# pascalPost/turbomesh

Hardware: AMD Instinct MI355X
Metric: nodes smoothed/sec (elliptic sweeps, 4096^2 blocks) + achieved HBM GB/s (higher is better)
Workload: dtype f64

## Files before the change

include/tm_hip.h:

```cpp
#ifndef TM_HIP_H
#define TM_HIP_H

#include <stdint.h>

#ifdef __cplusplus
extern "C" {
#endif

#define TM_HIP_ABI_VERSION 1

typedef enum tm_error {
    TM_OK = 0,
    TM_W_NOT_CONVERGED = 1,
    TM_E_SIZE = -1,
    TM_E_TOPOLOGY = -2,
    TM_E_MISMATCH = -3,
    TM_E_OVERFLOW = -4,
    TM_E_UNSUPPORTED = -5,
    TM_E_ARG = -6,
    TM_E_MEMORY = -7,
    TM_E_HIP = -8,
    TM_E_COMM = -9
} tm_error;

// ... 49 lines not shown
} tm_control_fn;

enum { TM_SOLVER_GMRES = 0, TM_SOLVER_BICGSTAB = 1, TM_SOLVER_UMFPACK = 2, TM_SOLVER_PETSC = 3, TM_SOLVER_HIP = 4 };
enum {
    TM_INNER_BICGSTAB = 0,
    TM_INNER_RELAX = 1,
    TM_INNER_MG_BICGSTAB = 2,
    TM_INNER_GMRES = 4,
    TM_INNER_REFERENCE_GMRES = 5,
    TM_INNER_AUTO = 3
};
enum {
    TM_OPT_SINGLE_SWEEP = 1,
    TM_OPT_EAGER_SCALARS = 2,
    TM_OPT_PRECOND_ILU0 = 8,
    TM_OPT_REFINE = 16,
    TM_OPT_RTOL_INITIAL = 4
};
typedef struct tm_solver_opt {
    int32_t tag;
    int32_t inner;
    double rtol;
    double atol;
    uint64_t max_inner;
    uint32_t check_every;
    uint32_t flags;
    double omega;
} tm_solver_opt;

typedef struct tm_stats {
    uint64_t outer_iterations;
    uint64_t inner_iterations;
    uint64_t operator_sweeps;
    double last_residual;
    double last_dx2, last_dy2;
    double scaled_residual_rms;
    double seconds;
    int32_t not_converged;
    int32_t _pad;
} tm_stats;

int tm_tfi_block(double* xy_out, uint64_t ni, uint64_t nj,
                 const double* x_i_min, const double* x_i_max,
                 const double* x_j_min, const double* x_j_max,
                 const double* s1, const double* s2, const double* t1, const double* t2);

int tm_tfi_linear2d(double* xy_out, uint64_t ni, uint64_t nj,
                    const double* e_i_min, const double* e_i_max, const double* e_j_min, const double* e_j_max);

int tm_smooth_mesh(const tm_mesh_desc* mesh, uint64_t iterations, const tm_solver_opt* opt,
                   const tm_control_fn* cf, tm_stats* stats );

int tm_csr_solve(uint64_t n, const int32_t* Ap, const int32_t* Ai, const double* Ax_x, const double* Ax_y ,
                 const double* bx, const double* by, double* x , double* y, const tm_solver_opt* opt ,
                 tm_stats* stats );

int tm_csr_residual(uint64_t n, const int32_t* Ap, const int32_t* Ai, const double* Ax_x, const double* Ax_y ,
                    const double* bx, const double* by, const double* x, const double* y, double* rx, double* ry);

typedef struct tm_smoother tm_smoother;

typedef struct tm_comm_hooks {
    void* ctx;
    int32_t rank, nranks;
    const int32_t* owner;
    int (*exchange)(void* ctx, const double* send_buf, double* recv_buf, void* stream);
    int (*allreduce_sum)(void* ctx, double* buf, int32_t n, void* stream);
    int (*exchange_wait)(void* ctx, void* stream);
    void* workspace;
    uint64_t workspace_bytes;
} tm_comm_hooks;
int tm_smoother_workspace_bytes(const tm_mesh_desc* mesh, const tm_solver_opt* opt, const tm_control_fn* cf,
                                const tm_comm_hooks* hooks, uint64_t* bytes);

int tm_smoother_create(const tm_mesh_desc* mesh, const tm_solver_opt* opt, const tm_control_fn* cf,
                       const tm_comm_hooks* hooks , void* stream ,
                       tm_smoother** out);
int tm_smoother_iterate(tm_smoother* s, uint64_t iterations, tm_stats* stats);
int tm_smoother_iterate_until(tm_smoother* s, uint64_t max_iterations, double scaled_residual_tol, tm_stats* stats);
int tm_smoother_iterate_until_update(tm_smoother* s, uint64_t max_iterations, double update_rms_tol, tm_stats* stats);
int tm_smoother_download(tm_smoother* s, const tm_mesh_desc* mesh);
int tm_smoother_upload(tm_smoother* s, const tm_mesh_desc* mesh);
void tm_smoother_destroy(tm_smoother* s);

typedef struct tm_rccl_comm tm_rccl_comm;
#define TM_RCCL_ID_BYTES 128
int tm_rccl_unique_id(const char* librccl_path, void* id_out );
int tm_rccl_comm_create(const char* librccl_path, const void* id, int32_t rank, int32_t nranks, tm_rccl_comm** out);
void tm_rccl_comm_destroy(tm_rccl_comm* comm);
int tm_rccl_hooks(tm_rccl_comm* comm, const tm_mesh_desc* mesh, const int32_t* owner , tm_comm_hooks* hooks);
int tm_rccl_hooks_for(tm_rccl_comm* comm, const tm_mesh_desc* mesh, const int32_t* owner, const tm_solver_opt* opt, const tm_control_fn* cf ,
                      tm_comm_hooks* hooks);

typedef struct tm_rccl_peer_table {
    int32_t npeers, direct_send;
    int64_t send_rows, recv_rows;
    int32_t* peer;
    int64_t *send_off, *send_cnt, *recv_off, *recv_cnt;
} tm_rccl_peer_table;
int tm_rccl_peer_table_build(const tm_mesh_desc* mesh, const int32_t* owner, int32_t rank, int32_t nranks, tm_rccl_peer_table* out);
void tm_rccl_peer_table_free(tm_rccl_peer_table* table);

int tm_smoother_exchange_plan(const tm_smoother* s, int32_t* npeers, const int32_t** peer_rank,
                              const int64_t** send_offset, const int64_t** send_count,
                              const int64_t** recv_offset, const int64_t** recv_count);

int tm_smoother_apply(tm_smoother* s, const double* in_xy, double* out_xy, int scaled);
int tm_smoother_assemble_csr(tm_smoother* s, int32_t* Ap, int32_t* Ai, double* Ax_x, double* Ax_y, uint64_t nnz_capacity, uint64_t* nnz);
int tm_smoother_apply_reference_order(tm_smoother* s, const double* in_xy, double* out_xy);
int tm_smoother_rhs(tm_smoother* s, double* rhs_xy);
int tm_smoother_residual(tm_smoother* s, const double* xy , double* r_xy);
int tm_smoother_refine_report(const tm_smoother* s, uint32_t* steps_x_y ,
                              double* last_update_rel ,
                              uint64_t* correction_iterations );
int tm_smoother_row_kinds(const tm_smoother* s, int32_t* kinds );
uint64_t tm_smoother_dof(const tm_smoother* s);
int tm_smoother_inner(const tm_smoother* s);
int tm_smoother_inner_counts(const tm_smoother* s, uint64_t* x_iterations, uint64_t* y_iterations);
int tm_smoother_control_function(tm_smoother* s, double* pq);

int tm_export_soa(const double* xy , uint64_t ni, uint64_t nj, double* x_out , double* y_out );
int tm_smoother_export_soa(tm_smoother* s, uint64_t block, double* x, double* y, double* p, double* q);

typedef struct tm_quality {
    uint64_t cells, inverted, degenerate;
    int32_t  orientation, _pad;
    double   min_scaled_jacobian;
    uint64_t worst_block, worst_i, worst_j;
    double   min_angle_deg, max_angle_deg;
    double   max_aspect, max_growth_i, max_growth_j;
    double   min_area, max_area, total_area;
    uint64_t hist[10];
} tm_quality;

int tm_mesh_quality(const tm_mesh_desc* mesh, tm_quality* per_block , tm_quality* total );
int tm_mesh_quality_host(const tm_mesh_desc* mesh, tm_quality* per_block, tm_quality* total);
int tm_smoother_quality(tm_smoother* s, tm_quality* per_block, tm_quality* total);
int tm_smoother_quality_field(tm_smoother* s, uint64_t block, double* min_scaled_jacobian );

typedef struct tm_plan_rows {
    uint64_t nrows;
    int64_t* row;
    int32_t* kind;
    int32_t* ncols;
    int64_t* cols;
    double* coef_x;
    double* coef_y;
    double* rhs;
    int32_t* slot;
} tm_plan_rows;
int tm_plan_build(const tm_mesh_desc* mesh, tm_plan_rows* out);
void tm_plan_free(tm_plan_rows* rows);

typedef struct tm_plan_local_info {
    int64_t n_owned, n_ghost, n_send;
    int32_t npeers, nowned_blocks;
    int64_t* owned_blocks;
    int64_t* local_start;
    int64_t* ghost_gid;
    int32_t* send_ids;
    int64_t* send_gid;
    int32_t* peer_rank;
    int64_t* send_offset;
    int64_t* send_count;
    int64_t* recv_offset;
    int64_t* recv_count;
    int64_t* send_first;
    int32_t direct_send;
    int32_t _pad;
    int64_t n_ghost_rows;
    int64_t* ghost_row_gid;
    int32_t* ghost_row_kind;
    int64_t* ghost_row_cols;
} tm_plan_local_info;
int tm_plan_local(const tm_mesh_desc* mesh, const int32_t* owner, int32_t rank, int32_t nranks, tm_plan_local_info* out);
void tm_plan_local_free(tm_plan_local_info* info);

int tm_dev_tfi_block(double* d_xy, uint64_t ni, uint64_t nj,
                     const double* d_x_i_min, const double* d_x_i_max, const double* d_x_j_min, const double* d_x_j_max,
                     const double* d_s1, const double* d_s2, const double* d_t1, const double* d_t2, void* stream);
int tm_dev_relax_sweep(const double* d_in, double* d_out, uint64_t ni, uint64_t nj, double omega,
                       double* d_partials, uint64_t partials_capacity, uint64_t* nwg, void* stream);
uint64_t tm_dev_relax_partials_needed(uint64_t ni, uint64_t nj);

#ifdef __cplusplus
}
#endif
#endif
```

turbomesh_amd/_capi.py:

```python
from __future__ import annotations

import ctypes as C
import os

import numpy as np

_HERE = os.path.dirname(os.path.abspath(__file__))
LIB_PATH = os.environ.get("TM_HIP_LIB") or os.path.join(_HERE, "libtm_hip.so")
DBG_LIB_PATH = os.path.join(_HERE, "libtm_hip_dbg.so")

TM_OK, TM_W_NOT_CONVERGED = 0, 1
TM_E_SIZE, TM_E_TOPOLOGY, TM_E_MISMATCH, TM_E_OVERFLOW, TM_E_UNSUPPORTED, TM_E_ARG, TM_E_MEMORY, TM_E_HIP, TM_E_COMM = -1, -2, -3, -4, -5, -6, -7, -8, -9
_ERR_NAMES = {-1: "InconsistentSize", -2: "Topology", -3: "Mismatch", -4: "Overflow", -5: "ExternalSolverNotEnabled", -6: "Argument",
              -7: "OutOfMemory", -8: "Hip", -9: "Comm"}
TM_SOLVER_GMRES, TM_SOLVER_BICGSTAB, TM_SOLVER_UMFPACK, TM_SOLVER_PETSC, TM_SOLVER_HIP = 0, 1, 2, 3, 4
TM_INNER_BICGSTAB, TM_INNER_RELAX, TM_INNER_MG_BICGSTAB, TM_INNER_AUTO, TM_INNER_GMRES, TM_INNER_REFERENCE_GMRES = 0, 1, 2, 3, 4, 5
TM_CF_LAPLACE, TM_CF_WHITE = 0, 1
TM_OPT_REFINE = 16


class TmError(RuntimeError):

    def __init__(self, code, msg):
        super().__init__(f"error.{_ERR_NAMES.get(code, 'Unknown')} ({code}): {msg}")
        self.code = code
        self.name = _ERR_NAMES.get(code, "Unknown")


class tm_range(C.Structure):
    _fields_ = [("block", C.c_uint64), ("side", C.c_uint32), ("_pad", C.c_uint32), ("start", C.c_uint64), ("end", C.c_uint64)]


class tm_connection(C.Structure):
    _fields_ = [("r", tm_range * 2), ("has_periodicity", C.c_int32), ("_pad", C.c_int32), ("periodicity", C.c_double * 2)]


class tm_condition(C.Structure):
    _fields_ = [("range", tm_range), ("kind", C.c_uint32), ("_pad", C.c_uint32)]


class tm_block(C.Structure):
    _fields_ = [("xy", C.POINTER(C.c_double)), ("ni", C.c_uint64), ("nj", C.c_uint64)]


class tm_mesh_desc(C.Structure):
    _fields_ = [("blocks", C.POINTER(tm_block)), ("nblocks", C.c_uint64), ("conns", C.POINTER(tm_connection)), ("nconns", C.c_uint64),
                ("bcs", C.POINTER(tm_condition)), ("nbcs", C.c_uint64)]


class tm_control_fn(C.Structure):
    _fields_ = [("kind", C.c_int32), ("_pad", C.c_int32), ("ds_target", C.c_double), ("theta_target", C.c_double)]


class tm_solver_opt(C.Structure):
    _fields_ = [("tag", C.c_int32), ("inner", C.c_int32), ("rtol", C.c_double), ("atol", C.c_double), ("max_inner", C.c_uint64),
                ("check_every", C.c_uint32), ("flags", C.c_uint32), ("omega", C.c_double)]


class tm_stats(C.Structure):
    _fields_ = [("outer_iterations", C.c_uint64), ("inner_iterations", C.c_uint64), ("operator_sweeps", C.c_uint64),
                ("last_residual", C.c_double), ("last_dx2", C.c_double), ("last_dy2", C.c_double), ("scaled_residual_rms", C.c_double),
                ("seconds", C.c_double), ("not_converged", C.c_int32), ("_pad", C.c_int32)]

    def as_dict(self):
        return {k: getattr(self, k) for k, _ in self._fields_ if not k.startswith("_")}


EXCHANGE_FN = C.CFUNCTYPE(C.c_int, C.c_void_p, C.c_void_p, C.c_void_p, C.c_void_p)
ALLREDUCE_FN = C.CFUNCTYPE(C.c_int, C.c_void_p, C.c_void_p, C.c_int32, C.c_void_p)
EXCHANGE_WAIT_FN = C.CFUNCTYPE(C.c_int, C.c_void_p, C.c_void_p)


LOG_FN = C.CFUNCTYPE(None, C.c_void_p, C.c_int32, C.c_uint64, C.c_double)


class tm_comm_hooks(C.Structure):
    _fields_ = [("ctx", C.c_void_p), ("rank", C.c_int32), ("nranks", C.c_int32), ("owner", C.POINTER(C.c_int32)),
                ("exchange", EXCHANGE_FN), ("allreduce_sum", ALLREDUCE_FN), ("exchange_wait", EXCHANGE_WAIT_FN), ("workspace", C.c_void_p),
                ("workspace_bytes", C.c_uint64)]


class tm_plan_rows(C.Structure):
    _fields_ = [("nrows", C.c_uint64), ("row", C.POINTER(C.c_int64)), ("kind", C.POINTER(C.c_int32)), ("ncols", C.POINTER(C.c_int32)),
                ("cols", C.POINTER(C.c_int64)), ("coef_x", C.POINTER(C.c_double)), ("coef_y", C.POINTER(C.c_double)),
                ("rhs", C.POINTER(C.c_double)), ("slot", C.POINTER(C.c_int32))]


class tm_plan_local_info(C.Structure):
    _fields_ = [("n_owned", C.c_int64), ("n_ghost", C.c_int64), ("n_send", C.c_int64), ("npeers", C.c_int32), ("nowned_blocks", C.c_int32),
                ("owned_blocks", C.POINTER(C.c_int64)), ("local_start", C.POINTER(C.c_int64)), ("ghost_gid", C.POINTER(C.c_int64)),
                ("send_ids", C.POINTER(C.c_int32)), ("send_gid", C.POINTER(C.c_int64)), ("peer_rank", C.POINTER(C.c_int32)),
                ("send_offset", C.POINTER(C.c_int64)), ("send_count", C.POINTER(C.c_int64)), ("recv_offset", C.POINTER(C.c_int64)),
                ("recv_count", C.POINTER(C.c_int64)), ("send_first", C.POINTER(C.c_int64)), ("direct_send", C.c_int32), ("_pad", C.c_int32),
                ("n_ghost_rows", C.c_int64), ("ghost_row_gid", C.POINTER(C.c_int64)), ("ghost_row_kind", C.POINTER(C.c_int32)),
                ("ghost_row_cols", C.POINTER(C.c_int64))]


class tm_rccl_peer_table(C.Structure):
    _fields_ = [("npeers", C.c_int32), ("direct_send", C.c_int32), ("send_rows", C.c_int64), ("recv_rows", C.c_int64),
                ("peer", C.POINTER(C.c_int32)), ("send_off", C.POINTER(C.c_int64)), ("send_cnt", C.POINTER(C.c_int64)),
                ("recv_off", C.POINTER(C.c_int64)), ("recv_cnt", C.POINTER(C.c_int64))]


_i32p = C.POINTER(C.c_int32)


class tm_edge_tables_info(C.Structure):
    _fields_ = ([("nrows", C.c_int64), ("nruns", C.c_int64), ("nwg", C.c_int64)] +
                [(k, _i32p) for k in ("first", "count", "row0", "row_stride", "col0", "col_stride", "met0", "met_stride", "kind", "ncols", "self", "flags",
                                     "wg_run", "wg_k0")] +
                [("gid", C.POINTER(C.c_int64)), ("nstrips", C.c_int64), ("ntasks", C.c_int64), ("strip_off", _i32p), ("task", _i32p)])


class tm_quality(C.Structure):
    _fields_ = [("cells", C.c_uint64), ("inverted", C.c_uint64), ("degenerate", C.c_uint64), ("orientation", C.c_int32), ("_pad", C.c_int32),
                ("min_scaled_jacobian", C.c_double), ("worst_block", C.c_uint64), ("worst_i", C.c_uint64), ("worst_j", C.c_uint64),
                ("min_angle_deg", C.c_double), ("max_angle_deg", C.c_double), ("max_aspect", C.c_double), ("max_growth_i", C.c_double),
                ("max_growth_j", C.c_double), ("min_area", C.c_double), ("max_area", C.c_double), ("total_area", C.c_double),
                ("hist", C.c_uint64 * 10)]


EXPORTS = [
    "tm_last_error", "tm_abi_version", "tm_set_log", "tm_csr_solve", "tm_tfi_block", "tm_tfi_linear2d", "tm_smooth_mesh", "tm_smoother_create",
    "tm_smoother_workspace_bytes", "tm_smoother_iterate", "tm_smoother_iterate_until", "tm_smoother_iterate_until_update", "tm_smoother_download", "tm_smoother_upload", "tm_smoother_destroy",
    "tm_smoother_exchange_plan", "tm_smoother_apply", "tm_smoother_rhs", "tm_smoother_row_kinds", "tm_smoother_dof",
    "tm_smoother_control_function", "tm_smoother_profile", "tm_smoother_profile_read", "tm_plan_build", "tm_plan_free", "tm_plan_local", "tm_plan_local_free", "tm_dev_tfi_block", "tm_dev_relax_sweep",
    "tm_dev_relax_partials_needed", "tm_export_soa", "tm_smoother_export_soa", "tm_rccl_unique_id", "tm_rccl_comm_create", "tm_rccl_comm_destroy", "tm_rccl_hooks",
    "tm_rccl_peer_table_build", "tm_rccl_peer_table_free", "tm_white_math_probe", "tm_stream_probe", "tm_smoother_queue_ordering", "tm_smoother_inner", "tm_csr_ilu0_probe", "tm_rccl_hooks_for", "tm_smoother_assemble_csr", "tm_smoother_apply_reference_order",
    "tm_smoother_inner_counts", "tm_mesh_quality", "tm_mesh_quality_host", "tm_smoother_quality", "tm_smoother_quality_field",
    "tm_csr_residual", "tm_smoother_residual", "tm_smoother_refine_report",
    "tm_mg_transfer_probe", "tm_smoother_mg_levels", "tm_smoother_precondition_probe", "tm_edge_tables_probe", "tm_edge_tables_free",
]

_lib = None
_dp = C.POINTER(C.c_double)


def _share_hip_runtime():
    import importlib.util
    import sys

    if "torch" in sys.modules:
        return
    try:
        spec = importlib.util.find_spec("torch")
    except (ImportError, ValueError):
        spec = None
    if spec is None or not spec.origin:
        return
    rt = os.path.join(os.path.dirname(spec.origin), "lib", "libamdhip64.so")
    if os.path.exists(rt):
        try:
            C.CDLL(rt, mode=C.RTLD_GLOBAL)
        except OSError:
            pass


def lib():
    global _lib
    if _lib is None:
        if not os.path.exists(LIB_PATH):
            raise OSError(f"{LIB_PATH} is missing: build it with `python -c 'import __graft_entry__ as g; g.build()'` "
                          "or `make -C turbomesh_amd/csrc`; turbomesh_amd has no CPU fallback")
        _share_hip_runtime()
        L = C.CDLL(LIB_PATH)
        L.tm_last_error.restype = C.c_char_p
        L.tm_csr_solve.argtypes = [C.c_uint64, C.POINTER(C.c_int32), C.POINTER(C.c_int32), _dp, _dp, _dp, _dp, _dp, _dp, C.POINTER(tm_solver_opt),
                                   C.POINTER(tm_stats)]
        L.tm_csr_residual.argtypes = [C.c_uint64, C.POINTER(C.c_int32), C.POINTER(C.c_int32)] + [_dp] * 8
        L.tm_set_log.argtypes = [LOG_FN, C.c_void_p]
        L.tm_set_log.restype = None
        L.tm_smoother_dof.restype = C.c_uint64
        L.tm_smoother_dof.argtypes = [C.c_void_p]
        L.tm_dev_relax_partials_needed.restype = C.c_uint64
        L.tm_dev_relax_partials_needed.argtypes = [C.c_uint64, C.c_uint64]
        L.tm_tfi_block.argtypes = [_dp, C.c_uint64, C.c_uint64] + [_dp] * 8
        L.tm_tfi_linear2d.argtypes = [_dp, C.c_uint64, C.c_uint64] + [_dp] * 4
        L.tm_smooth_mesh.argtypes = [C.POINTER(tm_mesh_desc), C.c_uint64, C.POINTER(tm_solver_opt), C.POINTER(tm_control_fn), C.POINTER(tm_stats)]
        L.tm_smoother_create.argtypes = [C.POINTER(tm_mesh_desc), C.POINTER(tm_solver_opt), C.POINTER(tm_control_fn), C.POINTER(tm_comm_hooks),
                                         C.c_void_p, C.POINTER(C.c_void_p)]
        L.tm_smoother_workspace_bytes.argtypes = [C.POINTER(tm_mesh_desc), C.POINTER(tm_solver_opt), C.POINTER(tm_control_fn),
                                                  C.POINTER(tm_comm_hooks), C.POINTER(C.c_uint64)]
        L.tm_smoother_iterate.argtypes = [C.c_void_p, C.c_uint64, C.POINTER(tm_stats)]
        L.tm_smoother_iterate_until.argtypes = [C.c_void_p, C.c_uint64, C.c_double, C.POINTER(tm_stats)]
        L.tm_smoother_iterate_until_update.argtypes = [C.c_void_p, C.c_uint64, C.c_double, C.POINTER(tm_stats)]
        L.tm_smoother_download.argtypes = [C.c_void_p, C.POINTER(tm_mesh_desc)]
        L.tm_smoother_upload.argtypes = [C.c_void_p, C.POINTER(tm_mesh_desc)]
        L.tm_smoother_destroy.argtypes = [C.c_void_p]
        L.tm_smoother_destroy.restype = None
        L.tm_smoother_exchange_plan.argtypes = [C.c_void_p, C.POINTER(C.c_int32), C.POINTER(C.POINTER(C.c_int32))] + [C.POINTER(C.POINTER(C.c_int64))] * 4
        L.tm_smoother_apply.argtypes = [C.c_void_p, _dp, _dp, C.c_int]
        L.tm_smoother_rhs.argtypes = [C.c_void_p, _dp]
        L.tm_smoother_residual.argtypes = [C.c_void_p, _dp, _dp]
        L.tm_smoother_refine_report.argtypes = [C.c_void_p, C.POINTER(C.c_uint32), _dp, C.POINTER(C.c_uint64)]
        L.tm_smoother_assemble_csr.argtypes = [C.c_void_p, C.POINTER(C.c_int32), C.POINTER(C.c_int32), _dp, _dp, C.c_uint64, C.POINTER(C.c_uint64)]
        L.tm_smoother_apply_reference_order.argtypes = [C.c_void_p, _dp, _dp]
        L.tm_smoother_row_kinds.argtypes = [C.c_void_p, C.POINTER(C.c_int32)]
        L.tm_smoother_control_function.argtypes = [C.c_void_p, _dp]
        L.tm_smoother_profile.argtypes = [C.c_void_p, C.c_int]
        L.tm_smoother_profile_read.argtypes = [C.c_void_p, _dp, C.POINTER(C.c_uint64), C.POINTER(C.c_uint64)]
        L.tm_smoother_queue_ordering.argtypes = [C.c_void_p]
        L.tm_smoother_inner.argtypes = [C.c_void_p]
        L.tm_smoother_inner_counts.argtypes = [C.c_void_p, C.POINTER(C.c_uint64), C.POINTER(C.c_uint64)]
        L.tm_csr_ilu0_probe.argtypes = [C.c_uint64, C.POINTER(C.c_int32), C.POINTER(C.c_int32), _dp, _dp, _dp, _dp]
        L.tm_plan_build.argtypes = [C.POINTER(tm_mesh_desc), C.POINTER(tm_plan_rows)]
        L.tm_plan_free.argtypes = [C.POINTER(tm_plan_rows)]
        L.tm_plan_free.restype = None
        L.tm_export_soa.argtypes = [_dp, C.c_uint64, C.c_uint64, _dp, _dp]
        L.tm_smoother_export_soa.argtypes = [C.c_void_p, C.c_uint64, _dp, _dp, _dp, _dp]
        L.tm_mesh_quality.argtypes = [C.POINTER(tm_mesh_desc), C.POINTER(tm_quality), C.POINTER(tm_quality)]
        L.tm_mesh_quality_host.argtypes = [C.POINTER(tm_mesh_desc), C.POINTER(tm_quality), C.POINTER(tm_quality)]
        L.tm_smoother_quality.argtypes = [C.c_void_p, C.POINTER(tm_quality), C.POINTER(tm_quality)]
        L.tm_smoother_quality_field.argtypes = [C.c_void_p, C.c_uint64, _dp]
        L.tm_rccl_unique_id.argtypes = [C.c_char_p, C.c_void_p]
        L.tm_rccl_comm_create.argtypes = [C.c_char_p, C.c_void_p, C.c_int32, C.c_int32, C.POINTER(C.c_void_p)]
        L.tm_rccl_comm_destroy.argtypes = [C.c_void_p]
        L.tm_rccl_comm_destroy.restype = None
        L.tm_rccl_hooks.argtypes = [C.c_void_p, C.POINTER(tm_mesh_desc), C.POINTER(C.c_int32), C.POINTER(tm_comm_hooks)]
        L.tm_rccl_hooks_for.argtypes = [C.c_void_p, C.POINTER(tm_mesh_desc), C.POINTER(C.c_int32), C.POINTER(tm_solver_opt), C.POINTER(tm_control_fn), C.POINTER(tm_comm_hooks)]
        L.tm_plan_local.argtypes = [C.POINTER(tm_mesh_desc), C.POINTER(C.c_int32), C.c_int32, C.c_int32, C.POINTER(tm_plan_local_info)]
        L.tm_plan_local_free.argtypes = [C.POINTER(tm_plan_local_info)]
        L.tm_plan_local_free.restype = None
        L.tm_dev_tfi_block.argtypes = [C.c_void_p, C.c_uint64, C.c_uint64] + [C.c_void_p] * 8 + [C.c_void_p]
        L.tm_dev_relax_sweep.argtypes = [C.c_void_p, C.c_void_p, C.c_uint64, C.c_uint64, C.c_double, C.c_void_p, C.c_uint64,
                                         C.POINTER(C.c_uint64), C.c_void_p]
        L.tm_rccl_peer_table_build.argtypes = [C.POINTER(tm_mesh_desc), C.POINTER(C.c_int32), C.c_int32, C.c_int32, C.POINTER(tm_rccl_peer_table)]
        L.tm_rccl_peer_table_free.argtypes = [C.POINTER(tm_rccl_peer_table)]
        L.tm_rccl_peer_table_free.restype = None
        L.tm_white_math_probe.argtypes = [_dp, _dp, C.c_uint64, _dp, _dp]
        L.tm_stream_probe.argtypes = [C.c_uint64, C.c_int32, _dp, _dp]
        L.tm_mg_transfer_probe.argtypes = [C.c_int32, C.c_uint64, C.c_uint64, C.c_int32, C.c_int32, _dp, _dp, C.c_double, C.c_double, _dp]
        L.tm_smoother_mg_levels.argtypes = [C.c_void_p, C.c_uint64, C.POINTER(C.c_int32), C.POINTER(C.c_int32), C.c_uint32, C.POINTER(C.c_int32), _dp]
        L.tm_smoother_precondition_probe.argtypes = [C.c_void_p, _dp, _dp, _dp]
        L.tm_edge_tables_probe.argtypes = [C.POINTER(tm_mesh_desc), C.POINTER(C.c_int32), C.c_int32, C.c_int32, C.c_int32, C.c_int32, C.POINTER(tm_edge_tables_info)]
        L.tm_edge_tables_free.argtypes = [C.POINTER(tm_edge_tables_info)]
        L.tm_edge_tables_free.restype = None
        if hasattr(L, "tm_tune_apply"):
            L.tm_debug_null_hooks.argtypes = [C.c_int32, C.c_int32, C.POINTER(C.c_int32), C.POINTER(tm_comm_hooks)]
            L.tm_diag_apply.argtypes = [C.c_void_p, C.c_void_p, C.c_uint64, C.c_uint64, C.c_int, C.c_void_p]
            L.tm_tune_fuse.argtypes = [C.c_int]
            L.tm_tune_apply.argtypes = [C.c_int, C.c_int, C.c_int, C.c_int]
        _lib = L
    return _lib


def check(rc):
    if rc < 0:
        raise TmError(rc, lib().tm_last_error().decode())
    return rc


def f64ptr(a):
    return a.ctypes.data_as(_dp)


class MeshDesc:

    def __init__(self, mesh, with_coordinates=True):
        blocks = mesh.blocks
        self._blocks = (tm_block * max(1, len(blocks)))()
        for k, b in enumerate(blocks):
            data = b.points.data
            if with_coordinates and data is not None:
                if data.dtype != np.float64 or not data.flags["C_CONTIGUOUS"]:
                    raise TmError(TM_E_ARG, "block coordinates must be C-contiguous float64")
                self._blocks[k] = tm_block(f64ptr(data), b.points.size[0], b.points.size[1])
            else:
                self._blocks[k] = tm_block(None, b.points.size[0], b.points.size[1])
        conns = mesh.connections
        self._conns = (tm_connection * max(1, len(conns)))()
        for k, c in enumerate(conns):
            tc = tm_connection()
            for s in range(2):
                r = c.ranges[s]
                tc.r[s] = tm_range(r.block, int(r.side), 0, r.start, r.end)
            tc.has_periodicity = 0 if c.periodicity is None else 1
            if c.periodicity is not None:
                tc.periodicity[0], tc.periodicity[1] = float(c.periodicity[0]), float(c.periodicity[1])
            self._conns[k] = tc
        bcs = mesh.boundary_conditions
        self._bcs = (tm_condition * max(1, len(bcs)))()
        for k, bc in enumerate(bcs):
            r = bc.range
            self._bcs[k] = tm_condition(tm_range(r.block, int(r.side), 0, r.start, r.end), int(bc.kind), 0)
        self.desc = tm_mesh_desc(self._blocks, len(blocks), self._conns, len(conns), self._bcs, len(bcs))

    def ref(self):
        return C.byref(self.desc)
```

turbomesh_amd/csrc/tm_api.cpp:

```cpp
#include "tm_smoother.hpp"
#include <cmath>
#include <cstdlib>
#include <cstring>
#include <limits>
#include <memory>

using namespace tmh;

#include "tm_api_util.hpp"
#include "tm_ilu.hpp"
#include "tm_refine.hpp"
#include "tm_quality_dev.hpp"

static void require_gfx950() {
    static int checked = 0;
    if (checked) return;
    int dev = 0;
    HIPCHK(hipGetDevice(&dev));
    hipDeviceProp_t prop;
    HIPCHK(hipGetDeviceProperties(&prop, dev));
    if (std::strncmp(prop.gcnArchName, "gfx950", 6) != 0)
        throw TmError(TM_E_HIP, std::string("libtm_hip is built for gfx950 (MI355X) only, found ") + prop.gcnArchName);
    checked = 1;
}
// ... 671 lines not shown
            gg.push_back(g.gid);
            gk.push_back(g.kind);
            for (int q = 0; q < 9; ++q) gc.push_back(q < g.ncols ? g.col[q] : -1);
        }
        out->n_ghost_rows = static_cast<int64_t>(gg.size());
        out->ghost_row_gid = dup(gg);
        out->ghost_row_kind = dup(gk);
        out->ghost_row_cols = dup(gc);
        return TM_OK;
    });
}
void tm_plan_local_free(tm_plan_local_info* i) {
    if (!i) return;
    std::free(i->owned_blocks);
    std::free(i->local_start);
    std::free(i->ghost_gid);
    std::free(i->send_ids);
    std::free(i->send_gid);
    std::free(i->peer_rank);
    std::free(i->send_first);
    std::free(i->send_offset);
    std::free(i->send_count);
    std::free(i->recv_offset);
    std::free(i->recv_count);
    std::free(i->ghost_row_gid);
    std::free(i->ghost_row_kind);
    std::free(i->ghost_row_cols);
    std::memset(i, 0, sizeof(*i));
}

int tm_edge_tables_probe(const tm_mesh_desc* mesh, const int32_t* owner, int32_t rank, int32_t nranks, int32_t table, int32_t level_strip,
                         tm_edge_tables_info* out) {
    return guarded([&]() {
        if (!mesh || !owner || !out) throw TmError(TM_E_ARG, "null argument");
        if (table < 0 || table > 5 || level_strip < 0) throw TmError(TM_E_ARG, "table outside 0..5 or negative strip length");
        std::memset(out, 0, sizeof(*out));
        const Topology t = topo_of(mesh);
        const std::vector<PlanRow> rows = build_rows(t);
        const LocalPlan lp = build_local_plan(t, rows, std::vector<int32_t>(owner, owner + t.nblocks()), rank, nranks);
        const MovingSides moving = moving_sides(t, lp);
        std::vector<PlanRow> zone[3];
        auto selection = [&](int tab) {
            std::vector<const PlanRow*> sel;
            auto add = [&](const std::vector<PlanRow>& more) {
                for (const PlanRow& r : more) sel.push_back(&r);
            };
            if (tab == 0) add(lp.rows);
            else for (size_t k : moving.nf_rows) sel.push_back(&lp.rows[k]);
            if (tab >= 3) add(zone[tab - 3] = zone_rows(t, lp, moving.dyn_mask, tab - 3));
            if (tab == 3) add(lp.ghost_rows2);
            if (tab == 2 || tab == 4) add(lp.ghost_rows);
            return sel;
        };
        RunTable level[3];
        for (int tab = 3; tab < 5 && table == 5; ++tab) level[tab - 3] = build_run_table(t, lp, selection(tab));
        const std::vector<const PlanRow*> sel = selection(table);
        const RunTable T = build_run_table(t, lp, sel);
        std::vector<int32_t> f[12], task;
        for (const EdgeRun& R : T.runs) {
            const int32_t scalars[8] = {R.first, R.count, R.row0, R.row_stride, R.kind, R.ncols, R.self, R.flags};
            for (int q = 0; q < 8; ++q) f[q].push_back(scalars[q]);
            f[8].insert(f[8].end(), R.col0, R.col0 + 9);
            f[9].insert(f[9].end(), R.col_stride, R.col_stride + 9);
            f[10].insert(f[10].end(), R.met0, R.met0 + 4);
            f[11].insert(f[11].end(), R.met_stride, R.met_stride + 4);
        }
        std::vector<int64_t> gid;
        for (int32_t k : T.order) gid.push_back(sel[k]->gid);
        StripPlan plan;
        if (table == 5) {
            const std::vector<EdgeRun>* const runs[3] = {&level[0].runs, &level[1].runs, &T.runs};
            plan = build_strip_plan(runs, T.where, level_strip ? level_strip : 60);
            for (int s = 0; s < plan.nstrips; ++s)
                for (int l = 0; l < 3; ++l)
                    for (int32_t k = plan.off[4 * s + l]; k < plan.off[4 * s + l + 1]; ++k)
                        task.insert(task.end(), {l + 1, plan.tasks[k].run, plan.tasks[k].k0, plan.tasks[k].count});
        }
        out->nrows = static_cast<int64_t>(sel.size());
        out->nruns = static_cast<int64_t>(T.runs.size());
        out->nwg = static_cast<int64_t>(T.wg_run.size());
        int32_t** const dst[12] = {&out->first, &out->count, &out->row0, &out->row_stride, &out->kind, &out->ncols, &out->self, &out->flags,
                                   &out->col0, &out->col_stride, &out->met0, &out->met_stride};
        for (int q = 0; q < 12; ++q) *dst[q] = dup(f[q]);
        out->wg_run = dup(T.wg_run);
        out->wg_k0 = dup(T.wg_k0);
        out->gid = dup(gid);
        out->nstrips = plan.nstrips;
        out->ntasks = static_cast<int64_t>(plan.tasks.size());
        out->strip_off = dup(plan.off);
        out->task = dup(task);
        return TM_OK;
    });
}
void tm_edge_tables_free(tm_edge_tables_info* i) {
    if (!i) return;
    int32_t* const arrays[] = {i->first, i->count, i->row0,   i->row_stride, i->col0,   i->col_stride, i->met0,      i->met_stride,
                               i->kind,  i->ncols, i->self,   i->flags,      i->wg_run, i->wg_k0,      i->strip_off, i->task};
    for (int32_t* p : arrays) std::free(p);
    std::free(i->gid);
    std::memset(i, 0, sizeof(*i));
}

int tm_plan_build(const tm_mesh_desc* mesh, tm_plan_rows* out) {
    return guarded([&]() {
        if (!mesh || !out) throw TmError(TM_E_ARG, "null argument");
        std::memset(out, 0, sizeof(*out));
        const Topology t = topo_of(mesh);
        const std::vector<PlanRow> rows = build_rows(t);
        const size_t n = rows.size();
        out->nrows = n;
        out->row = static_cast<int64_t*>(std::malloc(sizeof(int64_t) * (n ? n : 1)));
        out->kind = static_cast<int32_t*>(std::malloc(sizeof(int32_t) * (n ? n : 1)));
        out->ncols = static_cast<int32_t*>(std::malloc(sizeof(int32_t) * (n ? n : 1)));
        out->cols = static_cast<int64_t*>(std::malloc(sizeof(int64_t) * 9 * (n ? n : 1)));
        out->coef_x = static_cast<double*>(std::malloc(sizeof(double) * 9 * (n ? n : 1)));
        out->coef_y = static_cast<double*>(std::malloc(sizeof(double) * 9 * (n ? n : 1)));
        out->rhs = static_cast<double*>(std::malloc(sizeof(double) * 2 * (n ? n : 1)));
        out->slot = static_cast<int32_t*>(std::malloc(sizeof(int32_t) * 9 * (n ? n : 1)));
        if (!out->row || !out->kind || !out->ncols || !out->cols || !out->coef_x || !out->coef_y || !out->rhs || !out->slot) {
            tm_plan_free(out);
            throw TmError(TM_E_MEMORY, "out of host memory");
        }
        const double nan = std::numeric_limits<double>::quiet_NaN();
        for (size_t k = 0; k < n; ++k) {
            const PlanRow& r = rows[k];
            out->row[k] = r.gid;
            out->kind[k] = r.kind;
            out->ncols[k] = r.ncols;
            for (int q = 0; q < 9; ++q) {
                out->cols[k * 9 + q] = q < r.ncols ? r.col[q] : -1;
                out->coef_x[k * 9 + q] = (r.kind == KIND_SMOOTHED) ? nan : r.cx[q];
                out->coef_y[k * 9 + q] = (r.kind == KIND_SMOOTHED) ? nan : r.cy[q];
                out->slot[k * 9 + q] = r.slot[q];
            }
            out->rhs[2 * k] = (r.rhs_coord & 1) ? nan : r.rhs[0];
            out->rhs[2 * k + 1] = (r.rhs_coord & 2) ? nan : r.rhs[1];
        }
        return TM_OK;
    });
}
void tm_plan_free(tm_plan_rows* rows) {
    if (!rows) return;
    std::free(rows->row);
    std::free(rows->kind);
    std::free(rows->ncols);
    std::free(rows->cols);
    std::free(rows->coef_x);
    std::free(rows->coef_y);
    std::free(rows->rhs);
    std::free(rows->slot);
    std::memset(rows, 0, sizeof(*rows));
}

}
```

turbomesh_amd/csrc/tm_edge_types.h:

```cpp
#pragma once
#include <cstdint>

struct EdgeRun {
    int32_t first, count;
    int32_t row0, row_stride;
    int32_t col0[9], col_stride[9];
    int32_t met0[4], met_stride[4];
    int8_t kind, ncols, self;
    uint8_t flags;
    int8_t slot[9];
    int8_t _pad[3];
    double cx[9], cy[9];
    double per[2];
};
static_assert(sizeof(EdgeRun) == 296, "EdgeRun is read by the kernels through the scalar cache: its layout is fixed");
struct EdgeRowsDev {
    int nrows = 0;
    int nwg = 0;
    const EdgeRun* runs = nullptr;
    const int32_t* wg_run = nullptr;
    const int32_t* wg_k0 = nullptr;
    const double* rhs = nullptr;
};
constexpr int EDGE_BLOCK = 128;
struct LevelTask {
    int32_t run, k0, count;
};
struct FusedLevelsDev {
    int nstrips = 0;
    const LevelTask* tasks = nullptr;
    const int32_t* off = nullptr;
};
constexpr int LEVELS_BLOCK = 512;
```

turbomesh_amd/csrc/tm_kernels.h:

```cpp
#pragma once
#include <hip/hip_runtime.h>
#include <cstdint>
#include "tm_edge_types.h"
#include <vector>

namespace tmh {

enum ApplyMode : int {
    MODE_RAW = 0,
    MODE_SCALED = 1,
    MODE_RESID = 2,
    MODE_RELAX = 3,
    MODE_DIAG_COPY = 4,
    MODE_DIAG_SUM9 = 5,
    MODE_DIAG_NOSTORE = 6,
    MODE_DIAG_NOLOAD = 7,
    MODE_DIAG_MATH = 8,
    MODE_MG_RESID = 9,
    MODE_MG_SMOOTH = 10,
    MODE_MG_FIRST2 = 11
};
enum DotMode : int {
    DOT_NONE = 0,
    DOT_AUX = 1,
    DOT_IN = 2,
    DOT_OUT2 = 3,
    DOT_DELTA = 4,
    DOT_AUX2 = 5,
    DOT_IN_SS = 6,
    DOT_B2 = 7
};
constexpr int MAX_PARTIALS = 8;
struct KrylovScalars;
struct LazyScalars;

struct ApplyBlock {
    const double2* in2 = nullptr;
    const double2* in3 = nullptr;
    double2* pout = nullptr;
    const double2* in4 = nullptr;
    double2* rout = nullptr;
    double2* uio = nullptr;
    int rows = 0;
    int mg_nic = 0, mg_njc = 0, mg_ci = 0, mg_cj = 0;
    const double2* in;
    const double2* xk;
    const double2* pq;
    const double2* aux;
    double2* out;
    int ni, nj;
    double omega;
    double* partials;
};
int apply_block_nwg(int ni, int nj, int rows = 0);
int apply_block_nwg_overlap(int ni, int nj, int rows = 0);
void tune_apply(int rows_per_chunk, int unroll, int pipe, int nt);
hipError_t launch_apply_block(const ApplyBlock& a, int mode, int dot, hipStream_t stream);
constexpr int APPLY_BATCH_MAX = 8;
struct ApplyBatch {
    ApplyBlock b[APPLY_BATCH_MAX];
    int RI[APPLY_BATCH_MAX], nSG[APPLY_BATCH_MAX], nRC[APPLY_BATCH_MAX];
    int start[APPLY_BATCH_MAX];
    int n;
};
hipError_t launch_apply_blocks(const ApplyBlock* blocks, int n, int mode, int dot, hipStream_t stream);

struct Relax2Block {
    const double2* in;
    double2* mid;
    double2* out;
    int ni, nj;
    double omega;
    double* partials;
    const int32_t* border;
    int nborder;
    int store_nt = 1;
    int dyn;
};
bool relax2_supported(int ni, int nj);
int relax2_rows_per_chunk(int ni, int nj);
int relax2_block_nwg(int ni, int nj, int rows_per_chunk);
std::vector<int32_t> relax2_border_tiles(int ni, int nj, int rows_per_chunk, int dyn);
enum Relax2Subset { R2_ALL = 0, R2_BORDER = 1, R2_INSIDE_A = 2, R2_INSIDE_B = 3, R2_INSIDE = 4 };
constexpr long long QUEUE_WAIT_TICKS = 30LL * 100000000LL;
constexpr long long QUEUE_SELF_TEST_TICKS = 500000LL;
struct QueueWait {
    const uint32_t* counter = nullptr;
    uint32_t target = 0;
    uint32_t* error = nullptr;
    long long limit_ticks = QUEUE_WAIT_TICKS;
};
hipError_t launch_relax2_block(const Relax2Block& a, int rows_per_chunk, int dot, int subset, hipStream_t stream, size_t lds_bytes = 0,
                               const QueueWait* wait = nullptr);
struct Relax2Batch {
    Relax2Block b[8];
    int RI[8], nSG[8], nRC[8], start[8];
    int n;
};
hipError_t launch_relax2_blocks(const Relax2Block* blocks, const int* rows_per_chunk, int n, int dot, int subset, hipStream_t stream,
                                size_t lds_bytes = 0, const QueueWait* wait = nullptr);
void tune_fuse_rows(int rows);
bool relax3_supported(int ni, int nj);
int relax3_rows_per_chunk(int ni, int nj);
void relax3_rows_for_launch(const int* ni, const int* nj, int n, int* rows, bool beside_chain);
int relax3_block_nwg(int ni, int nj, int rows_per_chunk);
hipError_t launch_relax3_blocks(const Relax2Block* blocks, const int* rows_per_chunk, int n, int dot, hipStream_t stream);
bool relax4_supported(int ni, int nj);
void relax4_rows_for_launch(const int* ni, const int* nj, int n, int* rows);
int relax4_block_nwg(int ni, int nj, int rows_per_chunk);
hipError_t launch_relax4_blocks(const Relax2Block* blocks, const int* rows_per_chunk, int n, int dot, hipStream_t stream);

hipError_t launch_edge_levels3(const FusedLevelsDev& F, const EdgeRowsDev& e1, const EdgeRowsDev& e2, const EdgeRowsDev& e3, const double2* x, double2* m,
                               double2* m2, double2* out, const double2* pq, double omega, int dot, double* partials ,
                               hipStream_t stream);
hipError_t launch_edge_rows(const EdgeRowsDev& e, const double2* in, const double2* xk, const double2* pq, const double2* aux,
                            double2* out, double omega, int mode, int dot, double* partials, hipStream_t stream, uint32_t* signal = nullptr);
hipError_t launch_apply_edge_blocks(const ApplyBlock* blocks, int n, int mode, int dot, const EdgeRowsDev& e, const double2* in, const double2* xk,
                                    const double2* pq, const double2* aux, double2* out, double* edge_partials, hipStream_t stream);
constexpr int VK_NONE = 0, VK_S = 1, VK_P = 2, VK_R = 3, VK_S2 = 4, VK_PRO = 5;
struct VirtualIn {
    int kind;
    const double2 *in, *in2, *in3, *aux;
    double2* pout;
    const double2* in4 = nullptr;
    double2* rout = nullptr;
    double2* uio = nullptr;
};
hipError_t launch_apply_virtual(const ApplyBlock* blocks, int n, const EdgeRowsDev& e, const VirtualIn& V, const double2* xk, const double2* pq, double2* out,
                                double* edge_partials, const LazyScalars& scal, hipStream_t stream, bool overlap = false);
hipError_t launch_edge_rhs(const EdgeRowsDev& e, const double2* xk, const double2* pq, double2* rhs_out, int scaled,
                           double* partials , hipStream_t stream);

hipError_t launch_queue_signal(uint32_t* counter, hipStream_t stream);
hipError_t launch_queue_wait(const uint32_t* counter, uint32_t target, uint32_t* error, hipStream_t stream, long long limit_ticks = QUEUE_WAIT_TICKS);
hipError_t launch_queue_signal_wait(uint32_t* counter, const uint32_t* other, uint32_t target, uint32_t* error, hipStream_t stream,
                                    long long limit_ticks = QUEUE_WAIT_TICKS);

hipError_t launch_assemble_interior(const double2* xk, const double2* pq, int ni, int nj, const int32_t* row_ptr ,
                                    double* vx, double* vy, hipStream_t stream);
hipError_t launch_assemble_edge(const EdgeRowsDev& e, const double2* xk, const double2* pq, const int32_t* row_ptr, double* vx, double* vy, hipStream_t stream);
hipError_t launch_csr_product(int64_t n, const int32_t* row_ptr, const int32_t* col, const double* vx, const double* vy, const double2* in, double2* out,
                              hipStream_t stream);
hipError_t launch_delay_us(double us, hipStream_t stream);

hipError_t launch_finalize(const double* partials, int nwg, double* red, hipStream_t stream);

struct KrylovScalars {
    double rho[2], rho_old[2], alpha[2], omega[2], beta[2];
    double tol2[2];
    double rr[2];
    double rr0[2];
    int32_t done[2];
    int32_t early[2];
    int32_t iters;
    int32_t _pad;
};
constexpr int VEC_BLOCK = 256;
int vec_nwg(int64_t n);
enum ScalarStep : int { STEP_INIT = 0, STEP_SIGMA = 1, STEP_SS = 2, STEP_TSTT = 3, STEP_RHO = 4, STEP_TOL = 5, STEP_SS_TSTT = 6, STEP_INIT2 = 7, STEP_A2 = 8, STEP_B2 = 9 };
hipError_t launch_scalar_update(KrylovScalars* S, const double* red, int step, hipStream_t stream, double rtol = 0.0, double atol = 0.0);
hipError_t launch_finalize_scalar(const double* partials, int nwg, double* red, KrylovScalars* S, int step, hipStream_t stream, double rtol = 0.0,
                                  double atol = 0.0);
struct LazyStep {
    int step;
    const double* partials;
    int nwg;
};
struct LazyScalars {
    const KrylovScalars* S_in = nullptr;
    KrylovScalars* S_out = nullptr;
    int nsteps = 0;
    LazyStep st[2] = {{0, nullptr, 0}, {0, nullptr, 0}};
};
inline LazyScalars plain_scalars(const KrylovScalars* S) {
    LazyScalars L;
    L.S_in = S;
    return L;
}
hipError_t launch_p_update(const LazyScalars& S, const double2* r, double2* p, const double2* v, int64_t n, int nwg, hipStream_t stream);
hipError_t launch_s_update(const LazyScalars& S, const double2* r, const double2* v, double2* s, int64_t n, int nwg, double* partials,
                           hipStream_t stream);
hipError_t launch_xr_update(const LazyScalars& S, double2* u, const double2* p_hat, const double2* s_hat, const double2* s, const double2* t, double2* r,
                            const double2* r_hat, int64_t n, int nwg, double* partials, hipStream_t stream);
hipError_t launch_xr_update_vs(const LazyScalars& S, double2* u, const double2* p, const double2* v, const double2* t, double2* r, const double2* r_hat,
                               int64_t n, int nwg, double* partials, hipStream_t stream);
constexpr int GMRES_M = 30;
struct GmresScalars {
    double H[2][(GMRES_M + 1) * GMRES_M];
    double cs[2][GMRES_M], sn[2][GMRES_M];
    double g[2][GMRES_M + 1];
    double y[2][GMRES_M];
    double tol[2], beta[2], resid[2], rr0[2], scale[2];
    double rtol_initial;
    int32_t tol_initial[2];
    int32_t cols_used[2];
    int32_t done[2];
    int32_t scale_skip[2];
    int32_t j, cycle;
    int32_t sticky;
    int32_t iters[2];
};
hipError_t launch_gm_mgs(double2* w, const double2* v_prev, const double2* v_next, const double* red_prev, GmresScalars* G, int row_prev, int64_t n,
                         double* partials, hipStream_t stream);
hipError_t launch_gm_divide(double2* dst, const double2* src, const GmresScalars* G, int64_t n, hipStream_t stream);
hipError_t launch_gm_update(double2* u, const double2* V, int64_t ld, const GmresScalars* G, int64_t n, hipStream_t stream);
hipError_t launch_gm_tol(GmresScalars* G, const double* red, double rtol, double atol, hipStream_t stream, int sticky = 0);
hipError_t launch_gm_begin(GmresScalars* G, const double* red, hipStream_t stream);
hipError_t launch_gm_column(GmresScalars* G, const double* red, hipStream_t stream);
hipError_t launch_gm_backsub(GmresScalars* G, hipStream_t stream);

hipError_t launch_residual_copyback(double2* xk, const double2* u, int64_t n, int nwg, double* partials, hipStream_t stream);
hipError_t launch_stream(int kind, double2* a, const double2* b, const double2* c, double s, int64_t n, hipStream_t stream);
hipError_t launch_gather_rows(const double2* src, const int32_t* ids, int64_t n, double2* dst, hipStream_t stream);

hipError_t launch_copy_perimeter(const double2* in, double2* out, int ni, int nj, hipStream_t stream);
hipError_t launch_perimeter_sub(const double2* in, const double2* h, double2* out, int ni, int nj, hipStream_t stream);
hipError_t launch_ring_dirichlet(double2* f, const double2* X, const double2* PQ, double2* save, int ni, int nj, hipStream_t stream);
hipError_t launch_ring_restore(double2* f, const double2* save, int ni, int nj, hipStream_t stream);

hipError_t launch_tfi_block(double2* xy, int ni, int nj, const double2* x_i_min, const double2* x_i_max, const double2* x_j_min,
                            const double2* x_j_max, const double* s1, const double* s2, const double* t1, const double* t2,
                            hipStream_t stream);
hipError_t launch_tfi_linear2d(double2* xy, int ni, int nj, const double2* e_i_min, const double2* e_i_max, const double2* e_j_min,
                               const double2* e_j_max, hipStream_t stream);

struct WhiteArgs {
    const double2* x0;
    const double2* x1;
    double2* pq0;
    double2* pq1;
    int ni0, nj0, ni1, nj1;
    int le_p0, le_p1, le_fi0, le_fi1, le_dir0;
    double ds_target, theta_target;
};
hipError_t launch_white(const WhiteArgs& w, int update, hipStream_t stream);

struct MgPair {
    int nif, njf, nic, njc;
    int ci, cj;
};
hipError_t launch_mg_inject(const double2* fine, double2* coarse, const MgPair& g, double scale_x, double scale_y, hipStream_t stream);
hipError_t launch_mg_restrict(const double2* r_fine, const double2* X_coarse, double2* f_coarse, const MgPair& g, hipStream_t stream);
hipError_t launch_mg_prolong_smooth(const ApplyBlock& a, const MgPair& g, hipStream_t stream);
struct MgPairArgs {
    const double2* in = nullptr;
    const double2* xk = nullptr;
    const double2* pq = nullptr;
    const double2* f = nullptr;
    double2* out = nullptr;
    double2* out2 = nullptr;
    const double2* coarse = nullptr;
    const double2* xc = nullptr;
    double2* fc = nullptr;
    int nic = 0, njc = 0, ci = 0, cj = 0;
    int ni = 0, nj = 0;
    double omega = 1.0;
};
bool mg_pair_supported(int ni, int nj);
bool mg_pair_restrict_supported(int ni, int nj, int ci, int cj);
hipError_t launch_mg_pair(const MgPairArgs& a, int kind, hipStream_t stream);
hipError_t launch_mg_prolong_add(const double2* e_coarse, double2* e_fine, const MgPair& g, hipStream_t stream);
hipError_t launch_mg_scale(const double2* f, double2* out, int ni, int nj, double omega, hipStream_t stream);

// ... 6 lines not shown
```

turbomesh_amd/csrc/tm_kernels.hip:

```cpp
#include "tm_kernels.h"
#include "tm_devutil.hpp"
#include "tm_refmath.h"
#include <cstdlib>
#include <type_traits>

namespace tmh {

__device__ __forceinline__ double lane_prev(double edge, double v) {
    int2 o = __builtin_bit_cast(int2, edge), s = __builtin_bit_cast(int2, v), r;
    r.x = __builtin_amdgcn_update_dpp(o.x, s.x, 0x138 , 0xf, 0xf, false);
    r.y = __builtin_amdgcn_update_dpp(o.y, s.y, 0x138, 0xf, 0xf, false);
    return __builtin_bit_cast(double, r);
}
__device__ __forceinline__ double lane_next(double edge, double v) {
    int2 o = __builtin_bit_cast(int2, edge), s = __builtin_bit_cast(int2, v), r;
    r.x = __builtin_amdgcn_update_dpp(o.x, s.x, 0x130 , 0xf, 0xf, false);
    r.y = __builtin_amdgcn_update_dpp(o.y, s.y, 0x130, 0xf, 0xf, false);
    return __builtin_bit_cast(double, r);
}
__device__ __forceinline__ double2 lane_prev(double2 edge, double2 v) { return make_double2(lane_prev(edge.x, v.x), lane_prev(edge.y, v.y)); }
__device__ __forceinline__ double2 lane_next(double2 edge, double2 v) { return make_double2(lane_next(edge.x, v.x), lane_next(edge.y, v.y)); }

__device__ __forceinline__ double2 lane_prev0(double2 v) {
    int4 s = __builtin_bit_cast(int4, v), r;
// ... 739 lines not shown
        ++polls;
        if ((polls & 255u) != 0u) continue;
        if (__hip_atomic_load(error, __ATOMIC_RELAXED, __HIP_MEMORY_SCOPE_AGENT) != 0u) break;
        if (wall_clock64() - t0 > limit_ticks) {
            __hip_atomic_store(error, 1u, __ATOMIC_RELAXED, __HIP_MEMORY_SCOPE_AGENT);
            break;
        }
    }
}
__device__ __forceinline__ void queue_wait_in_kernel(const QueueWait& w) {
    if (threadIdx.x == 0) spin_until(w.counter, w.target, w.error, w.limit_ticks);
    __syncthreads();
    __builtin_amdgcn_fence(__ATOMIC_ACQUIRE, "agent");
}
__device__ __forceinline__ void queue_signal_in_kernel(uint32_t* counter) {
    if (counter && blockIdx.x == 0 && threadIdx.x == 0) __hip_atomic_fetch_add(counter, 1u, __ATOMIC_RELEASE, __HIP_MEMORY_SCOPE_AGENT);
}
template <int DOT, int U, int NT, bool W1>
__global__ __launch_bounds__(256) void k_relax2_waited(Relax2Block a, int RI, int nSG, int nRC, int subset, QueueWait w) {
    queue_wait_in_kernel(w);
    relax2_tile<DOT, U, NT, W1>(a, RI, nSG, nRC, subset, blockIdx.x);
}

template <int DOT, int U, int NT, bool W1>
__global__ __launch_bounds__(256) void k_relax2_batch_waited(Relax2Batch B, int subset, QueueWait w) {
    queue_wait_in_kernel(w);
    int k = 0;
#pragma unroll
    for (int q = 1; q < APPLY_BATCH_MAX; ++q)
        if (q < B.n && static_cast<int>(blockIdx.x) >= B.start[q]) k = q;
    relax2_tile<DOT, U, NT, W1>(B.b[k], B.RI[k], B.nSG[k], B.nRC[k], subset, static_cast<int>(blockIdx.x) - B.start[k]);
}
template <int DOT, int U, int NT, bool W1>
__global__ __launch_bounds__(256) void k_relax2_batch(Relax2Batch B, int subset) {
    int k = 0;
#pragma unroll
    for (int q = 1; q < APPLY_BATCH_MAX; ++q)
        if (q < B.n && static_cast<int>(blockIdx.x) >= B.start[q]) k = q;
    relax2_tile<DOT, U, NT, W1>(B.b[k], B.RI[k], B.nSG[k], B.nRC[k], subset, static_cast<int>(blockIdx.x) - B.start[k]);
}

#ifndef TM_R3_WAVES
#define TM_R3_WAVES 1
#endif
constexpr int R3_U = 3;
constexpr int R3_H = 3;
constexpr int R3_W = 64 - 2 * R3_H;
template <int DOT, int U, int NT, bool W1, bool INSIDE>
__device__ __forceinline__ void relax3_strip(const Relax2Block& a, const Relax2Tile& t, double (&acc)[MAX_PARTIALS]) {
    const int ni = a.ni, nj = a.nj;
    const int cc = INSIDE ? t.c : min(max(t.c, 0), nj - 1);
    const double2* in_col = a.in + cc;
    const int last_row = INSIDE ? t.i1 + 2 : ni - 1;
    auto load_in = [&](int row) { return in_col[static_cast<size_t>(INSIDE ? min(row, last_row) : min(max(row, 0), last_row)) * nj]; };
    const bool perim_col = !INSIDE && ((t.c <= 0) || (t.c >= nj - 1));
    const int nrows = t.i1 - t.i0;
    const __amdgpu_buffer_rsrc_t out_rsrc = __builtin_amdgcn_make_buffer_rsrc(a.out + static_cast<size_t>(t.i0) * nj, 0, nrows * nj * 16, 0x00020000);
    const bool skip_col = !INSIDE && (((a.dyn & 4) && t.c <= 2) || ((a.dyn & 8) && t.c >= nj - 3));
    const bool live_lane = t.out_lane && !skip_col;
    const unsigned lane_off = live_lane ? static_cast<unsigned>(cc) * 16u : OOB_VOFFSET;
    const double2 zero = make_double2(0.0, 0.0);

    Row3 A[3], S1[3], S2[3];
    double2 pc[U], pn[U];
    {
        const double2 a0 = load_in(t.i0 - 3), a1 = load_in(t.i0 - 2);
#pragma unroll
        for (int u = 0; u < U; ++u) pc[u] = load_in(t.i0 - 1 + u);
        A[0] = make_row(a0);
        A[1] = make_row(a1);
        A[2].c = A[2].e = A[2].h = zero;
        S1[0] = S1[1] = S1[2] = A[2];
        S2[0] = S2[1] = S2[2] = A[2];
    }
    const int nsteps = nrows + 4;
    auto group = [&](const int tb, const int phase) {
#pragma unroll
        for (int u = 0; u < U; ++u) pn[u] = load_in(t.i0 - 1 + tb + U + u);
#pragma unroll
        for (int u = 0; u < U; ++u) {
            const int A0 = u % 3, A1 = (u + 1) % 3, A2 = (u + 2) % 3;
            const int r = t.i0 - 1 + tb + u;
            A[A2] = make_row(pc[u]);
            double2 d = zero;
            double2 s1 = relax_row<W1>(A[A0], A[A1], A[A2], a.omega, d);
            if (!INSIDE && (perim_col || r - 1 <= 0 || r - 1 >= ni - 1)) s1 = A[A1].c;
            S1[A2] = make_row(s1);
            const bool do2 = phase > 0 || u >= 2, do3 = phase > 1 || (phase == 1 && u >= 1);
            double2 s2 = zero;
            if (do2) {
                s2 = relax_row<W1>(S1[A0], S1[A1], S1[A2], a.omega, d);
                if (!INSIDE && (perim_col || r - 2 <= 0 || r - 2 >= ni - 1)) s2 = S1[A1].c;
            }
            if (do2) S2[A2] = make_row(s2);
            double2 d3 = zero;
            double2 o = zero;
            if (do3) o = relax_row<W1>(S2[A0], S2[A1], S2[A2], a.omega, d3);
            const int i = r - 3;
            const bool row_live = (i >= t.i0) && (i < t.i1) && (INSIDE || !(((a.dyn & 1) && i <= 2) || ((a.dyn & 2) && i >= ni - 3)));
            __builtin_amdgcn_raw_buffer_store_b128(__builtin_bit_cast(v4i32, o), out_rsrc,
                                                   static_cast<int>(row_live ? lane_off + static_cast<unsigned>((i - t.i0) * nj * 16) : OOB_VOFFSET), 0,
                                                   (NT & 1) ? 2 : 0);
            if (DOT == DOT_DELTA) {
                if (!(live_lane && row_live)) d3 = zero;
                accumulate<DOT_DELTA>(acc, S2[A1].c, o, d3);
            }
        }
#pragma unroll
        for (int u = 0; u < U; ++u) pc[u] = pn[u];
    };
    static_assert(U == 3, "the phases below assume three steps per group");
    group(0, 0);
    group(U, 1);
    for (int tb = 2 * U; tb < nsteps; tb += U) group(tb, 2);
}

template <int DOT, int U, int NT, bool W1>
__device__ __forceinline__ void relax3_tile(const Relax2Block& a, int RI, int nSG, int nRC, int bid) {
    const int lane = threadIdx.x & 63;
    const int wave = threadIdx.x >> 6;
    const int total = nSG * nRC;
    const int q8 = total >> 3, rem = total & 7, xcd = bid & 7, k8 = bid >> 3;
    const int logical = (xcd < rem) ? xcd * (q8 + 1) + k8 : rem * (q8 + 1) + (xcd - rem) * q8 + k8;
    const int rc = logical / nSG;
    const int sg = logical - rc * nSG;
    const int ni = a.ni, nj = a.nj;
    Relax2Tile t;
    t.c0 = (sg * 4 + wave) * R3_W;
    t.c = t.c0 - R3_H + lane;
    t.out_lane = (lane >= R3_H) && (lane < 64 - R3_H) && (t.c >= 1) && (t.c <= nj - 2);
    t.i0 = 1 + rc * RI;
    t.i1 = min(t.i0 + RI, ni - 1);
    double acc[MAX_PARTIALS] = {0.0, 0.0, 0.0, 0.0};
    if (t.c0 <= nj - 2 && t.i0 < t.i1) {
        const bool inside = (t.c0 - R3_H >= 1) && (t.c0 - R3_H + 63 <= nj - 2) && (t.i0 - 3 >= 1) && (t.i1 + 2 <= ni - 2);
        if (inside) relax3_strip<DOT, U, NT, W1, true>(a, t, acc);
        else relax3_strip<DOT, U, NT, W1, false>(a, t, acc);
    }
    if (DOT != DOT_NONE) block_partials<256, dot_columns(DOT)>(acc, a.partials + static_cast<size_t>(logical) * MAX_PARTIALS);
}
template <int DOT, int U, int NT, bool W1>
__global__ __launch_bounds__(256, TM_R3_WAVES) void k_relax3(Relax2Block a, int RI, int nSG, int nRC) {
    relax3_tile<DOT, U, NT, W1>(a, RI, nSG, nRC, blockIdx.x);
}
template <int DOT, int U, int NT, bool W1>
__global__ __launch_bounds__(256) void k_relax3_batch(Relax2Batch B) {
    int k = 0;
#pragma unroll
    for (int q = 1; q < APPLY_BATCH_MAX; ++q)
        if (q < B.n && static_cast<int>(blockIdx.x) >= B.start[q]) k = q;
    relax3_tile<DOT, U, NT, W1>(B.b[k], B.RI[k], B.nSG[k], B.nRC[k], static_cast<int>(blockIdx.x) - B.start[k]);
}
constexpr int R4_L = 4;
constexpr int R4_W = 64 - 2 * R4_L;
template <int L, int DOT, int U, int NT, bool W1, bool INSIDE>
__device__ __forceinline__ void relaxn_strip(const Relax2Block& a, const Relax2Tile& t, double (&acc)[MAX_PARTIALS]) {
    static_assert(U == 3 && L >= 3, "three steps per group; the windows rotate by renaming");
    constexpr int STEADY = (2 * (L - 1) + 2) / 3;
    const int ni = a.ni, nj = a.nj;
    const int cc = INSIDE ? t.c : min(max(t.c, 0), nj - 1);
    const double2* in_col = a.in + cc;
    const int last_row = INSIDE ? t.i1 + L - 1 : ni - 1;
    auto load_in = [&](int row) { return in_col[static_cast<size_t>(INSIDE ? min(row, last_row) : min(max(row, 0), last_row)) * nj]; };
    const bool perim_col = !INSIDE && ((t.c <= 0) || (t.c >= nj - 1));
    const int nrows = t.i1 - t.i0;
    const __amdgpu_buffer_rsrc_t out_rsrc = __builtin_amdgcn_make_buffer_rsrc(a.out + static_cast<size_t>(t.i0) * nj, 0, nrows * nj * 16, 0x00020000);
    const unsigned lane_off = t.out_lane ? static_cast<unsigned>(cc) * 16u : OOB_VOFFSET;
    const double2 zero = make_double2(0.0, 0.0);
    const int r0 = t.i0 - (L - 2);

    Row3 A[3], S[L - 1][3];
    double2 pc[U], pn[U];
    {
        const double2 a0 = load_in(r0 - 2), a1 = load_in(r0 - 1);
#pragma unroll
        for (int u = 0; u < U; ++u) pc[u] = load_in(r0 + u);
        A[0] = make_row(a0);
        A[1] = make_row(a1);
        A[2].c = A[2].e = A[2].h = zero;
#pragma unroll
        for (int k = 0; k < L - 1; ++k) S[k][0] = S[k][1] = S[k][2] = A[2];
    }
    const int nsteps = nrows + 2 * (L - 1);
    auto group = [&](const int tb, const int phase) {
#pragma unroll
        for (int u = 0; u < U; ++u) pn[u] = load_in(r0 + tb + U + u);
#pragma unroll
        for (int u = 0; u < U; ++u) {
            const int A0 = u % 3, A1 = (u + 1) % 3, A2 = (u + 2) % 3;
            const int r = r0 + tb + u;
            const int s = U * phase + u;
            A[A2] = make_row(pc[u]);
            double2 d = zero;
            double2 v = relax_row<W1>(A[A0], A[A1], A[A2], a.omega, d);
            if (!INSIDE && (perim_col || r - 1 <= 0 || r - 1 >= ni - 1)) v = A[A1].c;
            S[0][A2] = make_row(v);
#pragma unroll
            for (int k = 2; k < L; ++k) {
                if (phase >= STEADY || s >= 2 * (k - 1)) {
                    v = relax_row<W1>(S[k - 2][A0], S[k - 2][A1], S[k - 2][A2], a.omega, d);
                    if (!INSIDE && (perim_col || r - k <= 0 || r - k >= ni - 1)) v = S[k - 2][A1].c;
                    S[k - 1][A2] = make_row(v);
                }
            }
            double2 dl = zero, o = zero;
            if (phase >= STEADY || s >= 2 * (L - 1)) o = relax_row<W1>(S[L - 2][A0], S[L - 2][A1], S[L - 2][A2], a.omega, dl);
            const int i = r - L;
            const bool row_live = (i >= t.i0) && (i < t.i1);
            __builtin_amdgcn_raw_buffer_store_b128(__builtin_bit_cast(v4i32, o), out_rsrc,
                                                   static_cast<int>(row_live ? lane_off + static_cast<unsigned>((i - t.i0) * nj * 16) : OOB_VOFFSET), 0,
                                                   (NT & 1) ? 2 : 0);
            if (DOT == DOT_DELTA) {
                if (!(t.out_lane && row_live)) dl = zero;
                accumulate<DOT_DELTA>(acc, S[L - 2][A1].c, o, dl);
            }
        }
#pragma unroll
        for (int u = 0; u < U; ++u) pc[u] = pn[u];
    };
    static_assert(STEADY == 2, "two warm-up groups are peeled below");
    group(0, 0);
    group(U, 1);
    for (int tb = 2 * U; tb < nsteps; tb += U) group(tb, STEADY);
}

template <int L, int DOT, int U, int NT, bool W1>
__device__ __forceinline__ void relaxn_tile(const Relax2Block& a, int RI, int nSG, int nRC, int bid) {
    constexpr int W = 64 - 2 * L;
    const int lane = threadIdx.x & 63;
    const int wave = threadIdx.x >> 6;
    const int total = nSG * nRC;
    const int q8 = total >> 3, rem = total & 7, xcd = bid & 7, k8 = bid >> 3;
    const int logical = (xcd < rem) ? xcd * (q8 + 1) + k8 : rem * (q8 + 1) + (xcd - rem) * q8 + k8;
    const int rc = logical / nSG;
    const int sg = logical - rc * nSG;
    const int ni = a.ni, nj = a.nj;
    Relax2Tile t;
    t.c0 = (sg * 4 + wave) * W;
    t.c = t.c0 - L + lane;
    t.out_lane = (lane >= L) && (lane < 64 - L) && (t.c >= 1) && (t.c <= nj - 2);
    t.i0 = 1 + rc * RI;
    t.i1 = min(t.i0 + RI, ni - 1);
    double acc[MAX_PARTIALS] = {0.0, 0.0, 0.0, 0.0};
    if (t.c0 <= nj - 2 && t.i0 < t.i1) {
        const bool inside = (t.c0 - L >= 1) && (t.c0 - L + 63 <= nj - 2) && (t.i0 - L >= 1) && (t.i1 + L - 1 <= ni - 2);
        if (inside) relaxn_strip<L, DOT, U, NT, W1, true>(a, t, acc);
        else relaxn_strip<L, DOT, U, NT, W1, false>(a, t, acc);
    }
    if (DOT != DOT_NONE) block_partials<256, dot_columns(DOT)>(acc, a.partials + static_cast<size_t>(logical) * MAX_PARTIALS);
}
template <int DOT, int U, int NT, bool W1>
__global__ __launch_bounds__(256) void k_relax4(Relax2Block a, int RI, int nSG, int nRC) {
    relaxn_tile<R4_L, DOT, U, NT, W1>(a, RI, nSG, nRC, blockIdx.x);
}
template <int DOT, int U, int NT, bool W1>
__global__ __launch_bounds__(256) void k_relax4_batch(Relax2Batch B) {
    int k = 0;
#pragma unroll
    for (int q = 1; q < APPLY_BATCH_MAX; ++q)
        if (q < B.n && static_cast<int>(blockIdx.x) >= B.start[q]) k = q;
    relaxn_tile<R4_L, DOT, U, NT, W1>(B.b[k], B.RI[k], B.nSG[k], B.nRC[k], static_cast<int>(blockIdx.x) - B.start[k]);
}
static int g_fuse3_rows = 0;
void relax3_rows_for_launch(const int* ni, const int* nj, int n, int* rows, bool beside_chain) {
    static const int forced = [] { const char* e = std::getenv("TM_FUSE3_ROWS"); return e ? std::atoi(e) : 0; }();
    if (forced > 0 || g_fuse3_rows > 0) {
        for (int k = 0; k < n; ++k) rows[k] = std::max(1, std::min(forced > 0 ? forced : g_fuse3_rows, ni[k] - 2));
        return;
    }
    static int slots = 0;
    if (slots == 0) {
        int dev = 0, cus = 0;
        if (hipGetDevice(&dev) != hipSuccess || hipDeviceGetAttribute(&cus, hipDeviceAttributeMultiprocessorCount, dev) != hipSuccess || cus <= 0) cus = 256;
        slots = 3 * cus;
    }
    static const int heights[] = {38, 26, 14, 8};
    const long need = static_cast<long>(slots) * (beside_chain ? 9 : 6);
    int RI = 8;
    for (const int h : heights) {
        long total = 0;
        for (int k = 0; k < n; ++k) {
            const int nstrips = (nj[k] - 1 + R3_W - 1) / R3_W, nSG = (nstrips + 3) / 4, interior = ni[k] - 2, r = std::max(1, std::min(h, interior));
            total += static_cast<long>(nSG) * ((interior + r - 1) / r);
        }
        RI = h;
        if (total * 10 >= need) break;
    }
    for (int k = 0; k < n; ++k) rows[k] = std::max(1, std::min(RI, ni[k] - 2));
}
int relax3_rows_per_chunk(int ni, int nj) {
    int r = 0;
    relax3_rows_for_launch(&ni, &nj, 1, &r, false);
    return r;
}
bool relax3_supported(int ni, int nj) { return ni >= 7 && nj >= 7 && nj <= (1 << 20); }
int relax3_block_nwg(int ni, int nj, int RI) {
    const int nstrips = (nj - 1 + R3_W - 1) / R3_W;
    return ((nstrips + 3) / 4) * ((ni - 2 + RI - 1) / RI);
}
static hipError_t launch_fixed_wall_blocks(int depth, const Relax2Block* blocks, const int* rows_per_chunk, int n, int dot, hipStream_t st) {
    const int W = 64 - 2 * depth;
    for (int first = 0; first < n; first += APPLY_BATCH_MAX) {
        Relax2Batch B;
        B.n = 0;
        int total = 0;
        bool w1 = true;
        const bool nts = blocks[first].store_nt != 0;
        for (int k = first; k < n && B.n < APPLY_BATCH_MAX; ++k) {
            const int q = B.n++;
            B.b[q] = blocks[k];
            B.RI[q] = rows_per_chunk[k];
            B.nSG[q] = ((blocks[k].nj - 1 + W - 1) / W + 3) / 4;
            B.nRC[q] = (blocks[k].ni - 2 + B.RI[q] - 1) / B.RI[q];
            B.start[q] = total;
            total += B.nSG[q] * B.nRC[q];
            w1 = w1 && blocks[k].omega == 1.0;
        }
        for (int q = B.n; q < APPLY_BATCH_MAX; ++q) B.start[q] = total;
        if (total == 0) continue;
        const dim3 grid(total), block(256);
#define TM_R3(KERNEL, ...)                                                                                                   \
    do {                                                                                                                     \
        if (dot == DOT_DELTA) {                                                                                              \
            if (w1 && nts) hipLaunchKernelGGL((KERNEL<DOT_DELTA, R3_U, 1, true>), grid, block, 0, st, __VA_ARGS__);          \
            else if (w1) hipLaunchKernelGGL((KERNEL<DOT_DELTA, R3_U, 0, true>), grid, block, 0, st, __VA_ARGS__);            \
            else hipLaunchKernelGGL((KERNEL<DOT_DELTA, R3_U, 1, false>), grid, block, 0, st, __VA_ARGS__);                   \
        } else {                                                                                                             \
            if (w1 && nts) hipLaunchKernelGGL((KERNEL<DOT_NONE, R3_U, 1, true>), grid, block, 0, st, __VA_ARGS__);           \
            else if (w1) hipLaunchKernelGGL((KERNEL<DOT_NONE, R3_U, 0, true>), grid, block, 0, st, __VA_ARGS__);             \
            else hipLaunchKernelGGL((KERNEL<DOT_NONE, R3_U, 1, false>), grid, block, 0, st, __VA_ARGS__);                    \
        }                                                                                                                    \
    } while (0)
        static const bool force_batch = [] { const char* e = std::getenv("TM_R3_FORCE_BATCH"); return e && std::atoi(e) != 0; }();
        const bool lone = B.n == 1 && !force_batch;
        if (depth == R4_L) {
            if (lone) TM_R3(k_relax4, B.b[0], B.RI[0], B.nSG[0], B.nRC[0]);
            else TM_R3(k_relax4_batch, B);
        } else {
            if (lone) TM_R3(k_relax3, B.b[0], B.RI[0], B.nSG[0], B.nRC[0]);
            else TM_R3(k_relax3_batch, B);
        }
#undef TM_R3
        const hipError_t rc = hipGetLastError();
        if (rc != hipSuccess) return rc;
    }
    return hipSuccess;
}
hipError_t launch_relax3_blocks(const Relax2Block* blocks, const int* rows_per_chunk, int n, int dot, hipStream_t st) {
    return launch_fixed_wall_blocks(3, blocks, rows_per_chunk, n, dot, st);
}

void relax4_rows_for_launch(const int* ni, const int* nj, int n, int* rows) {
    static const int forced = [] { const char* e = std::getenv("TM_FUSE4_ROWS"); return e ? std::atoi(e) : 0; }();
    if (forced > 0) {
        for (int k = 0; k < n; ++k) rows[k] = std::max(1, std::min(forced, ni[k] - 2));
        return;
    }
    static int slots = 0;
    if (slots == 0) {
        int dev = 0, cus = 0;
        if (hipGetDevice(&dev) != hipSuccess || hipDeviceGetAttribute(&cus, hipDeviceAttributeMultiprocessorCount, dev) != hipSuccess || cus <= 0) cus = 256;
        slots = 3 * cus;
    }
    static const int heights[] = {54, 42, 30, 18, 6};
    const long need = static_cast<long>(slots) * 6;
    int RI = 6;
    for (const int h : heights) {
        long total = 0;
        for (int k = 0; k < n; ++k) {
            const int nstrips = (nj[k] - 1 + R4_W - 1) / R4_W, nSG = (nstrips + 3) / 4, interior = ni[k] - 2, r = std::max(1, std::min(h, interior));
            total += static_cast<long>(nSG) * ((interior + r - 1) / r);
        }
        RI = h;
        if (total * 10 >= need) break;
    }
    for (int k = 0; k < n; ++k) rows[k] = std::max(1, std::min(RI, ni[k] - 2));
}
bool relax4_supported(int ni, int nj) { return ni >= 2 * R4_L + 1 && nj >= 2 * R4_L + 1 && nj <= (1 << 20); }
int relax4_block_nwg(int ni, int nj, int RI) {
    const int nstrips = (nj - 1 + R4_W - 1) / R4_W;
    return ((nstrips + 3) / 4) * ((ni - 2 + RI - 1) / RI);
}
hipError_t launch_relax4_blocks(const Relax2Block* blocks, const int* rows_per_chunk, int n, int dot, hipStream_t st) {
    for (int k = 0; k < n; ++k)
        if (blocks[k].dyn != 0) return hipErrorInvalidValue;
    return launch_fixed_wall_blocks(R4_L, blocks, rows_per_chunk, n, dot, st);
}

constexpr int MG_RST_W = 58;
struct MgMetric {
    double G11, G22, mhG12, m2D, D, rinv;
};
__device__ __forceinline__ MgMetric mg_metric(double2 dxi, double2 det) {
    MgMetric m;
    m.G11 = fma(dxi.x, dxi.x, dxi.y * dxi.y);
    m.G22 = fma(det.x, det.x, det.y * det.y);
    const double G12 = fma(dxi.x, det.x, dxi.y * det.y);
    m.D = m.G11 + m.G22;
    m.m2D = -2.0 * m.D;
    m.mhG12 = -0.5 * G12;
    m.rinv = recip_diag(m.D, m.m2D);
    return m;
}
template <bool HAS_PQ>
__device__ __forceinline__ double2 mg_scaled_row(const MgMetric& g, const Row3& m, const Row3& c, const Row3& p, double P, double Q) {
    double ax = p.c.x + m.c.x, ay = p.c.y + m.c.y;
    double bx = c.h.x, by = c.h.y;
    if (HAS_PQ) {
        const double hP = 0.5 * P, hQ = 0.5 * Q;
        ax = fma(hP, p.c.x - m.c.x, ax);
        ay = fma(hP, p.c.y - m.c.y, ay);
        bx = fma(hQ, c.e.x, bx);
        by = fma(hQ, c.e.y, by);
    }
    const double kx = p.e.x - m.e.x;
    const double ky = p.e.y - m.e.y;
    double sx = g.G22 * ax, sy = g.G22 * ay;
    sx = fma(g.G11, bx, sx);
    sy = fma(g.G11, by, sy);
    sx = fma(g.m2D, c.c.x, sx);
    sy = fma(g.m2D, c.c.y, sy);
    sx = fma(g.mhG12, kx, sx);
    sy = fma(g.mhG12, ky, sy);
    return make_double2(sx * g.rinv, sy * g.rinv);
}

template <int KIND, bool HAS_PQ, bool PRO, bool RST, int U>
__device__ __forceinline__ void mg_pair_strip(const MgPairArgs& a, const Relax2Tile& t) {
    static_assert(!RST || KIND == 1, "the restriction rides behind the residual");
    const int ni = a.ni, nj = a.nj;
    const int cc = min(max(t.c, 0), nj - 1);
    const double2 zero = make_double2(0.0, 0.0);
    auto at = [&](int row) { return static_cast<size_t>(min(max(row, 0), ni - 1)) * nj + cc; };
    const bool perim_col = (t.c <= 0) || (t.c >= nj - 1);
    const bool col_in = (t.c >= 1) && (t.c <= nj - 2);
    const int nrows = t.i1 - t.i0;
    const __amdgpu_buffer_rsrc_t out_rsrc = __builtin_amdgcn_make_buffer_rsrc(a.out + static_cast<size_t>(t.i0) * nj, 0, nrows * nj * 16, 0x00020000);
    const __amdgpu_buffer_rsrc_t out2_rsrc =
        __builtin_amdgcn_make_buffer_rsrc((KIND == 1 ? a.out2 : a.out) + static_cast<size_t>(t.i0) * nj, 0, nrows * nj * 16, 0x00020000);
    const unsigned lane_off = static_cast<unsigned>(cc) * 16u;
    const int cj1 = PRO ? min(a.cj ? ((cc + 1) >> 1) : cc, a.njc - 1) : 0;
    const bool midway = PRO && a.cj && (cc & 1);

    struct Ld {
        double2 in, x, f, pq, c0, c1;
    };
    auto load_step = [&](int i, Ld& L) {
        const size_t ar = at(i + 2), aq = at(i + 1);
        L.in = a.in[ar];
        L.x = a.xk[ar];
        if (KIND == 0) L.f = a.f[aq];
        if (HAS_PQ) L.pq = a.pq[aq];
        if (PRO) {
            const int r = min(max(i + 2, 0), ni - 1);
            const int ci0 = min(a.ci ? (r >> 1) : r, a.nic - 1), ci1 = min(a.ci ? ((r + 1) >> 1) : r, a.nic - 1);
            const double2* r0 = a.coarse + static_cast<size_t>(ci0) * a.njc;
            const double2* r1 = a.coarse + static_cast<size_t>(ci1) * a.njc;
            L.c0 = r0[cj1];
            L.c1 = r1[cj1];
        }
    };
    auto entering = [&](int row, const Ld& L) {
        if (KIND == 1) return (col_in && row >= 1 && row <= ni - 2) ? L.in : zero;
        if (!PRO) return L.in;
        const double2 l0 = lane_prev0(L.c0), l1 = lane_prev0(L.c1);
        const double2 a0 = midway ? l0 : L.c0, a1 = midway ? l1 : L.c1;
        const double2 v = make_double2(L.in.x + 0.25 * ((a0.x + L.c0.x) + (a1.x + L.c1.x)), L.in.y + 0.25 * ((a0.y + L.c0.y) + (a1.y + L.c1.y)));
        return (col_in && row >= 1 && row <= ni - 2) ? v : L.in;
    };
    auto det_of = [&](double2 x) { return sub2(lane_next0(x), lane_prev0(x)); };

    Row3 A[3], S[3];
    double2 Xc[3], Xe_cur;
    MgMetric Mp = {0.0, 0.0, 0.0, 0.0, 0.0, 0.0};
    double2 f_prev = zero, pq_prev = zero;
    double2 rm2 = zero, rm1 = zero;
    Ld cur[U], nxt[U];
    {
        Ld w0, w1;
        load_step(t.i0 - 4, w0);
        load_step(t.i0 - 3, w1);
#pragma unroll
        for (int u = 0; u < U; ++u) load_step(t.i0 - 2 + u, cur[u]);
        A[0] = make_row(entering(t.i0 - 2, w0));
        A[1] = make_row(entering(t.i0 - 1, w1));
        Xc[0] = w0.x;
        Xc[1] = w1.x;
        Xe_cur = det_of(w1.x);
        A[2].c = A[2].e = A[2].h = zero;
        S[0] = S[1] = S[2] = A[2];
        Xc[2] = zero;
    }
    const int nsteps = nrows + (RST ? 3 : 2);
    auto group = [&](const int tb) {
#pragma unroll
        for (int u = 0; u < U; ++u) load_step(t.i0 - 2 + tb + U + u, nxt[u]);
#pragma unroll
        for (int u = 0; u < U; ++u) {
            const int A0 = u % 3, A1 = (u + 1) % 3, A2 = (u + 2) % 3;
            const Ld& L = cur[u];
            const int i = t.i0 - 2 + tb + u;
            const int q = i + 1;
            A[A2] = make_row(entering(i + 2, L));
            Xc[A2] = L.x;
            const double2 Xe_next = det_of(L.x);
            const MgMetric M = mg_metric(sub2(Xc[A2], Xc[A0]), Xe_cur);
            const double2 t1 = mg_scaled_row<HAS_PQ>(M, A[A0], A[A1], A[A2], HAS_PQ ? L.pq.x : 0.0, HAS_PQ ? L.pq.y : 0.0);
            const double2 fq = (KIND == 0) ? L.f : A[A1].c;
            double2 s1;
            if (KIND == 0) {
                const double2 res = sub2(fq, t1);
                s1 = make_double2(fma(a.omega, res.x, A[A1].c.x), fma(a.omega, res.y, A[A1].c.y));
            } else {
                s1 = make_double2(a.omega * fma(-a.omega, t1.x, 2.0 * A[A1].c.x), a.omega * fma(-a.omega, t1.y, 2.0 * A[A1].c.y));
            }
            const bool perim_row = (q <= 0) || (q >= ni - 1);
            if (perim_row || perim_col) s1 = zero;
            if (KIND == 1) {
                const bool own = t.out_lane && !perim_row && (q >= t.i0) && (q < t.i1);
                __builtin_amdgcn_raw_buffer_store_b128(__builtin_bit_cast(v4i32, s1), out_rsrc,
                                                       static_cast<int>(own ? lane_off + static_cast<unsigned>((q - t.i0) * nj * 16) : OOB_VOFFSET), 0, 0);
            }
            S[A2] = make_row(s1);
            const double2 t2 = mg_scaled_row<HAS_PQ>(Mp, S[A0], S[A1], S[A2], HAS_PQ ? pq_prev.x : 0.0, HAS_PQ ? pq_prev.y : 0.0);
            const double2 res2 = sub2(f_prev, t2);
            double2 o;
            if (KIND == 0) {
                o = make_double2(fma(a.omega, res2.x, S[A1].c.x), fma(a.omega, res2.y, S[A1].c.y));
            } else {
                const double aii = -0.5 * Mp.D;
                o = make_double2(aii * res2.x, aii * res2.y);
            }
            if (!RST) {
                const bool live = t.out_lane && (i >= t.i0) && (i < t.i1);
                __builtin_amdgcn_raw_buffer_store_b128(__builtin_bit_cast(v4i32, o), out2_rsrc,
                                                       static_cast<int>(live ? lane_off + static_cast<unsigned>((i - t.i0) * nj * 16) : OOB_VOFFSET), 0, 2);
            } else {
                const double2 oz = (col_in && i >= 1 && i <= ni - 2) ? o : zero;
                if ((i & 1) && i > t.i0 && i <= t.i1) {
                    double2 acc = zero;
// ... 1703 lines not shown
```

turbomesh_amd/csrc/tm_plan.cpp:

```cpp
#include "tm_plan.hpp"
#include "../../include/tm_hip.h"
#include <cstdlib>
#include <algorithm>
#include <unordered_map>

namespace tmh {

namespace {

struct Junction {
    std::vector<int64_t> ids;
    std::vector<double> per;
    std::vector<int64_t> stencil;
    double rhs[2] = {0.0, 0.0};
};

enum { S_I_J = 0, S_IP1_J, S_IM1_J, S_I_JP1, S_I_JM1, S_IP1_JP1, S_IP1_JM1, S_IM1_JP1, S_IM1_JM1 };

struct Builder {
    const Topology& t;
    std::vector<int64_t> perim_start;
    std::vector<PlanRow> rows;

    explicit Builder(const Topology& topo) : t(topo) {}

    int64_t perim_count(int64_t b) const { return 2 * (t.nj[b] + t.ni[b] - 2); }
    void block_of(int64_t gid, int64_t& b, int64_t& local) const {
        int64_t k = t.nblocks() - 1;
        while (gid < t.start[k]) --k;
        b = k;
        local = gid - t.start[k];
    }
    int64_t perim_index(int64_t b, int64_t i, int64_t j) const {
        const int64_t ni = t.ni[b], nj = t.nj[b];
        if (i == 0) return j;
        if (i == ni - 1) return nj + 2 * (ni - 2) + j;
        if (j == 0) return nj + (i - 1) * 2;
        if (j == nj - 1) return nj - 1 + i * 2;
        throw PlanError(TM_E_TOPOLOGY, "NotBoundaryIndex: node is not on the block perimeter");
    }
    PlanRow& row_of(int64_t gid) {
        int64_t b, local;
        block_of(gid, b, local);
        const int64_t i = local / t.nj[b], j = local - i * t.nj[b];
        return rows[perim_start[b] + perim_index(b, i, j)];
    }
    std::vector<int64_t> range_points(const TopoRange& r) const {
        const int64_t ni = t.ni[r.block], nj = t.nj[r.block];
        int64_t idx = 0, inc = 0;
        switch (r.side) {
            case SIDE_I_MIN: idx = r.start * nj; inc = nj; break;
            case SIDE_I_MAX: idx = r.start * nj + nj - 1; inc = nj; break;
            case SIDE_J_MIN: idx = r.start; inc = 1; break;
            case SIDE_J_MAX: idx = (ni - 1) * nj + r.start; inc = 1; break;
        }
        const int64_t n = (r.start > r.end ? r.start - r.end : r.end - r.start) + 1;
        if (r.start > r.end) inc = -inc;
        std::vector<int64_t> out(n);
        for (int64_t k = 0; k < n; ++k) out[k] = idx + k * inc;
        return out;
    }
    int64_t first_internal_shift(const TopoRange& r) const {
        switch (r.side) {
            case SIDE_I_MIN: return 1;
            case SIDE_I_MAX: return -1;
            case SIDE_J_MIN: return t.nj[r.block];
            default: return -t.nj[r.block];
        }
    }

    std::vector<Junction> find_junctions() const;
    void build();
};

void append_unique(Junction& jn, int64_t id, const double per[2]) {
    for (int64_t v : jn.ids)
        if (v == id) return;
    if (jn.ids.size() >= 4) throw PlanError(TM_E_OVERFLOW, "junction point with more than 4 overlapping points");
    jn.ids.push_back(id);
    jn.per.push_back(per[0]);
    jn.per.push_back(per[1]);
}

std::vector<Junction> Builder::find_junctions() const {
    std::vector<Junction> out;
    const size_t nc = t.conns.size();
    if (nc == 0) return out;
    std::vector<int64_t> ep(nc * 4);
    for (size_t c = 0; c < nc; ++c) {
        const auto p0 = range_points(t.conns[c].r[0]);
        const auto p1 = range_points(t.conns[c].r[1]);
        ep[c * 4 + 0] = t.start[t.conns[c].r[0].block] + p0.front();
        ep[c * 4 + 1] = t.start[t.conns[c].r[1].block] + p1.front();
        ep[c * 4 + 2] = t.start[t.conns[c].r[0].block] + p0.back();
        ep[c * 4 + 3] = t.start[t.conns[c].r[1].block] + p1.back();
    }
    const double zero[2] = {0.0, 0.0};
    auto per_of = [&](size_t conn) -> const double* { return t.conns[conn].periodic ? t.conns[conn].per : zero; };
    for (size_t e = 0; e + 1 < ep.size(); ++e) {
        for (size_t chk = e + 1; chk < ep.size(); ++chk) {
            if (ep[chk] != ep[e]) continue;
            bool found = false;
            for (auto& jn : out) {
                const size_t n0 = jn.ids.size();
                for (size_t k = 0; k < n0; ++k)
                    if (jn.ids[k] == ep[e]) {
                        found = true;
                        const size_t add = (chk % 2 == 0) ? chk + 1 : chk - 1;
                        append_unique(jn, ep[add], per_of(add / 4));
                    }
            }
            if (found) continue;
            const size_t p0 = e / 2, p1 = chk / 2;
            if (p0 == p1) throw PlanError(TM_E_TOPOLOGY, "connection joins a point with itself");
            Junction jn;
            jn.ids.push_back(ep[p0 * 2]);
            jn.per.insert(jn.per.end(), {0.0, 0.0});
            append_unique(jn, ep[p0 * 2 + 1], per_of(p0 / 2));
            if (jn.ids.size() != 2) throw PlanError(TM_E_TOPOLOGY, "connection joins a point with itself");
            append_unique(jn, ep[p1 * 2], per_of(p1 / 2));
            append_unique(jn, ep[p1 * 2 + 1], per_of(p1 / 2));
            out.push_back(jn);
        }
    }
    for (auto& jn : out) {
        std::vector<size_t> order(jn.ids.size());
        for (size_t k = 0; k < order.size(); ++k) order[k] = k;
        std::stable_sort(order.begin(), order.end(), [&](size_t a, size_t b) { return jn.ids[a] < jn.ids[b]; });
        Junction s = jn;
        for (size_t k = 0; k < order.size(); ++k) {
            s.ids[k] = jn.ids[order[k]];
            s.per[2 * k] = jn.per[2 * order[k]];
            s.per[2 * k + 1] = jn.per[2 * order[k] + 1];
        }
        jn = s;
    }
    std::stable_sort(out.begin(), out.end(), [](const Junction& a, const Junction& b) { return a.ids[0] < b.ids[0]; });
    for (auto& jn : out) {
        jn.stencil.push_back(jn.ids[0]);
        for (size_t k = 0; k < jn.ids.size(); ++k) {
            int64_t b, local;
            block_of(jn.ids[k], b, local);
            const int64_t ni = t.ni[b], nj = t.nj[b];
            const int64_t i = local / nj, j = local - i * nj;
            int64_t nb[2][2];
            int n = 0;
            auto push = [&](int64_t a, int64_t c) { nb[n][0] = a; nb[n][1] = c; ++n; };
            if (i == 0) {
                if (j == 0) push(1, 1);
                else if (j == nj - 1) push(1, nj - 2);
                else { push(1, j - 1); push(1, j + 1); }
            } else if (i == ni - 1) {
                if (j == 0) push(ni - 2, 1);
                else if (j == nj - 1) push(ni - 2, nj - 2);
                else { push(ni - 2, j - 1); push(ni - 2, j + 1); }
            } else if (j == 0) {
// ... 291 lines not shown
    Builder b(t);
    b.build();
    return std::move(b.rows);
}

int64_t LocalPlan::to_local(int64_t gid) const {
    int64_t b = topo->nblocks() - 1;
    while (gid < topo->start[b]) --b;
    const auto it = std::lower_bound(owned_blocks.begin(), owned_blocks.end(), b);
    if (it != owned_blocks.end() && *it == b) return local_start[it - owned_blocks.begin()] + (gid - topo->start[b]);
    const auto g = ghost_index.find(gid);
    return g == ghost_index.end() ? -1 : n_owned + g->second;
}

bool triple_halo_for(const Topology& t, int nranks) {
    if (nranks < 2) return false;
    int64_t min_nodes = 0;
    if (const char* e = std::getenv("TM_TRIPLES_MIN_NODES")) min_nodes = std::atoll(e);
    if (min_nodes < 0) return false;
    for (int64_t b = 0; b < t.nblocks(); ++b)
        if (t.ni[b] < 16 || t.nj[b] < 16 || t.ni[b] * t.nj[b] < min_nodes) return false;
    return true;
}

LocalPlan build_local_plan(const Topology& t, const std::vector<PlanRow>& all_rows, const std::vector<int32_t>& owner, int rank,
                           int nranks, bool allow_triples) {
    LocalPlan lp;
    lp.rank = rank;
    lp.nranks = nranks;
    lp.topo = &t;
    const int64_t nb = t.nblocks();
    if (static_cast<int64_t>(owner.size()) != nb) throw PlanError(TM_E_ARG, "owner table must have one entry per block");
    for (int64_t b = 0; b < nb; ++b) {
        if (owner[b] < 0 || owner[b] >= nranks) throw PlanError(TM_E_ARG, "owner table names a missing rank");
        if (owner[b] == rank) {
            lp.owned_blocks.push_back(b);
            lp.local_start.push_back(lp.n_owned);
            lp.n_owned += t.ni[b] * t.nj[b];
        }
    }
    auto owner_of_gid = [&](int64_t gid) {
        int64_t b = nb - 1;
        while (gid < t.start[b]) --b;
        return owner[b];
    };
    std::vector<std::vector<std::pair<int32_t, int64_t>>> need(nranks);
    for (const PlanRow& r : all_rows) {
        const int32_t ro = owner_of_gid(r.gid);
        auto touch = [&](int64_t gid) {
            const int32_t o = owner_of_gid(gid);
            if (o != ro) need[ro].emplace_back(o, gid);
        };
        for (int k = 0; k < r.ncols; ++k) touch(r.col[k]);
        if (r.kind == KIND_SMOOTHED)
            for (int k = 0; k < 4; ++k) touch(r.metric[k]);
        if (ro == rank) lp.rows.push_back(r);
    }
    for (auto& v : need) {
        std::sort(v.begin(), v.end());
        v.erase(std::unique(v.begin(), v.end()), v.end());
    }
    auto row_def = [&](int64_t gid) {
        const auto it = std::lower_bound(all_rows.begin(), all_rows.end(), gid, [](const PlanRow& a, int64_t g) { return a.gid < g; });
        if (it != all_rows.end() && it->gid == gid) return *it;
        int64_t b = nb - 1;
        while (gid < t.start[b]) --b;
        const int64_t nj = t.nj[b];
        PlanRow r{};
        r.gid = gid;
        r.kind = KIND_INTERIOR;
        r.ncols = 9;
        r.self = 4;
        int q = 0;
        for (int64_t di = -1; di <= 1; ++di)
            for (int64_t dj = -1; dj <= 1; ++dj) r.col[q++] = gid + di * nj + dj;
        return r;
    };
    std::vector<std::vector<std::pair<int32_t, int64_t>>> need2 = need;
    for (int r = 0; r < nranks; ++r) {
        for (const auto& pr : need[r]) {
            const PlanRow def = row_def(pr.second);
            auto touch = [&](int64_t gid) {
                const int32_t o = owner_of_gid(gid);
                if (o != r) need2[r].emplace_back(o, gid);
            };
            for (int k = 0; k < def.ncols; ++k) touch(def.col[k]);
            if (def.kind == KIND_SMOOTHED)
                for (int k = 0; k < 4; ++k) touch(def.metric[k]);
            if (r == rank) lp.ghost_rows.push_back(def);
        }
        std::sort(need2[r].begin(), need2[r].end());
        need2[r].erase(std::unique(need2[r].begin(), need2[r].end()), need2[r].end());
    }
    need.swap(need2);
    lp.triple_halo = allow_triples && triple_halo_for(t, nranks);
    if (lp.triple_halo) {
        std::vector<std::vector<std::pair<int32_t, int64_t>>> need3 = need;
        for (int r = 0; r < nranks; ++r) {
            for (const auto& pr : need[r]) {
                const PlanRow def = row_def(pr.second);
                auto touch = [&](int64_t gid) {
                    const int32_t o = owner_of_gid(gid);
                    if (o != r) need3[r].emplace_back(o, gid);
                };
                for (int k = 0; k < def.ncols; ++k) touch(def.col[k]);
                if (def.kind == KIND_SMOOTHED)
                    for (int k = 0; k < 4; ++k) touch(def.metric[k]);
                if (r == rank) lp.ghost_rows2.push_back(def);
            }
            std::sort(need3[r].begin(), need3[r].end());
            need3[r].erase(std::unique(need3[r].begin(), need3[r].end()), need3[r].end());
        }
        need.swap(need3);
    }
    for (const auto& pr : need[rank]) {
        lp.ghost_index[pr.second] = static_cast<int64_t>(lp.ghost_gid.size());
        lp.ghost_gid.push_back(pr.second);
    }
    std::vector<std::vector<int64_t>> send_to(nranks), recv_from(nranks);
    for (const auto& pr : need[rank]) recv_from[pr.first].push_back(pr.second);
    for (int r = 0; r < nranks; ++r) {
        if (r == rank) continue;
        for (const auto& pr : need[r])
            if (pr.first == rank) send_to[r].push_back(pr.second);
    }
    int64_t soff = 0, roff = 0;
    for (int r = 0; r < nranks; ++r) {
        if (r == rank || (send_to[r].empty() && recv_from[r].empty())) continue;
        lp.peer_rank.push_back(r);
        lp.send_off.push_back(soff);
        lp.send_cnt.push_back(static_cast<int64_t>(send_to[r].size()));
        lp.recv_off.push_back(roff);
        lp.recv_cnt.push_back(static_cast<int64_t>(recv_from[r].size()));
        for (int64_t gid : send_to[r]) {
            int64_t b = nb - 1;
            while (gid < t.start[b]) --b;
            const auto it = std::lower_bound(lp.owned_blocks.begin(), lp.owned_blocks.end(), b);
            lp.send_ids.push_back(static_cast<int32_t>(lp.local_start[it - lp.owned_blocks.begin()] + (gid - t.start[b])));
        }
        soff += static_cast<int64_t>(send_to[r].size());
        roff += static_cast<int64_t>(recv_from[r].size());
    }
    lp.direct_send = !lp.peer_rank.empty();
    for (size_t k = 0; k < lp.peer_rank.size(); ++k) {
        const int64_t o = lp.send_off[k], c = lp.send_cnt[k];
        lp.send_first.push_back(c ? lp.send_ids[o] : 0);
        for (int64_t q = 1; q < c; ++q)
            if (lp.send_ids[o + q] != lp.send_ids[o] + q) lp.direct_send = false;
    }
    if (lp.n_owned + static_cast<int64_t>(lp.ghost_gid.size()) >= (int64_t{1} << 31)) throw PlanError(TM_E_SIZE, "rank-local vector exceeds 2^31 rows");
    return lp;
}

}
```

turbomesh_amd/csrc/tm_plan.hpp:

```cpp
#pragma once
#include <cstdint>
#include <stdexcept>
#include <string>
#include <unordered_map>
#include <vector>

namespace tmh {

struct PlanError : std::runtime_error {
    int code;
    PlanError(int c, const std::string& m) : std::runtime_error(m), code(c) {}
};

enum Side : uint32_t { SIDE_I_MIN = 0, SIDE_I_MAX = 1, SIDE_J_MIN = 2, SIDE_J_MAX = 3 };
enum RowKind : int8_t {
    KIND_FIXED = 0, KIND_SMOOTHED = 1, KIND_CONNECTED = 2, KIND_JUNCTION = 3, KIND_SLIDING = 4,
    KIND_INTERIOR = 5
};

struct TopoRange {
    int64_t block;
    uint32_t side;
    int64_t start, end;
};
struct TopoConn {
    TopoRange r[2];
    bool periodic;
    double per[2];
};
struct TopoCond {
    TopoRange range;
    uint32_t kind;
};
struct Topology {
    std::vector<int64_t> ni, nj;
    std::vector<TopoConn> conns;
    std::vector<TopoCond> bcs;
    std::vector<int64_t> start;
    int64_t dof = 0;
    void finalize();
    int64_t nblocks() const { return static_cast<int64_t>(ni.size()); }
};

struct PlanRow {
    int64_t gid;
    int8_t kind;
    int8_t ncols;
    int8_t self;
    int64_t col[9];
    double cx[9], cy[9];
    int8_t slot[9];
    int64_t metric[4];
    double per[2];
    uint8_t flags;
    double rhs[2];
    uint8_t rhs_coord;
};

struct ConnShifts {
    int64_t count;
    int64_t first_internal[2];
    int64_t direction[2];
    int64_t position[2];
};
ConnShifts conn_shifts(const Topology& t, const TopoConn& c);

std::vector<PlanRow> build_rows(const Topology& t);

struct LocalPlan {
    int rank = 0, nranks = 1;
    std::vector<int64_t> owned_blocks;
    std::vector<int64_t> local_start;
    int64_t n_owned = 0;
    std::vector<int64_t> ghost_gid;
    std::vector<PlanRow> rows;
    std::vector<PlanRow> ghost_rows;
    bool triple_halo = false;
    std::vector<PlanRow> ghost_rows2;
    std::vector<int32_t> peer_rank;
    std::vector<int64_t> send_off, send_cnt, recv_off, recv_cnt;
    std::vector<int32_t> send_ids;
    bool direct_send = false;
    std::vector<int64_t> send_first;
    std::unordered_map<int64_t, int64_t> ghost_index;
    int64_t to_local(int64_t gid) const;
    const Topology* topo = nullptr;
};
bool triple_halo_for(const Topology& t, int nranks);
LocalPlan build_local_plan(const Topology& t, const std::vector<PlanRow>& all_rows, const std::vector<int32_t>& owner, int rank,
                           int nranks, bool allow_triples = true);

}
```

turbomesh_amd/csrc/tm_smoother.cpp:

```cpp
#include "tm_smoother.hpp"
#include "tm_api_util.hpp"
#include "tm_ilu.hpp"
#include "tm_refine.hpp"
#include "tm_quality_dev.hpp"
#include <algorithm>
#include <atomic>
#include <chrono>
#include <cmath>
#include <cstdio>
#include <cstdlib>
#include <cstring>
#include <map>
#include <unordered_map>

namespace tmh {

void hip_check(hipError_t e, const char* what) {
    if (e != hipSuccess) throw TmError(TM_E_HIP, std::string(what) + ": " + hipGetErrorString(e));
}
#define HIPCHK(x) hip_check((x), #x)

std::atomic<int> g_multirank_handles{0};
tm_log_fn g_log_sink = nullptr;
void* g_log_ctx = nullptr;
// ... 320 lines not shown
    }
};

RunTable Smoother::make_table(const Selection& sel, EdgeRowsDev& e) {
    RunTable T = planned([&] { return build_run_table(topo, lp, sel.rows); });
    if (std::getenv("TM_DEBUG_RUNS")) {
        int singles = 0;
        for (const EdgeRun& R : T.runs) singles += R.count == 1;
        std::fprintf(stderr, "[tm] perimeter-row table: %zu rows -> %zu runs (%d of one row), %zu workgroups\n", sel.rows.size(), T.runs.size(), singles, T.wg_run.size());
    }
    e.nrows = static_cast<int>(sel.rows.size());
    e.nwg = static_cast<int>(T.wg_run.size());
    e.runs = static_cast<const EdgeRun*>(upload_table(T.runs.data(), T.runs.size() * sizeof(EdgeRun)));
    e.wg_run = static_cast<const int32_t*>(upload_table(T.wg_run.data(), T.wg_run.size() * 4));
    e.wg_k0 = static_cast<const int32_t*>(upload_table(T.wg_k0.data(), T.wg_k0.size() * 4));
    RhsTable rt;
    rt.dev = arena.alloc_n<double>(sel.rows.size() * 2);
    for (int32_t k : T.order) rt.src.push_back(sel.rhs[k]);
    e.rhs = rt.dev;
    rhs_tables.push_back(std::move(rt));
    return T;
}

void Smoother::build_row_tables() {
    const size_t nr = lp.rows.size();
    h_rhs.assign(nr * 2, 0.0);
    rhs_tables.clear();
    Selection all;
    for (size_t k = 0; k < nr; ++k) all.add(lp.rows[k], &h_rhs[2 * k]);
    make_table(all, edge);
    MovingSides moving = moving_sides(topo, lp);
    dyn_mask = std::move(moving.dyn_mask);
    if (opt.inner != TM_INNER_RELAX) return;
    Selection nf;
    for (size_t k : moving.nf_rows) nf.add(lp.rows[k], &h_rhs[2 * k]);
    make_table(nf, edge_nf);
    if (fuse_pairs && has_hooks && !lp.ghost_rows.empty()) {
        Selection sel = nf;
        sel.add_static(lp.ghost_rows);
        make_table(sel, edge_nf_g);
    }
    if (!triples_coupled) return;
    RunTable level[3];
    for (int lev = 0; lev < 3; ++lev) {
        const std::vector<PlanRow> zone = zone_rows(topo, lp, dyn_mask, lev);
        Selection sl = nf;
        for (const PlanRow& z : zone) sl.add(z, zero_rhs);
        if (lev == 0) sl.add_static(lp.ghost_rows2);
        if (lev == 1) sl.add_static(lp.ghost_rows);
        level[lev] = make_table(sl, edge_L[lev]);
    }
    levels_fused = true;
    if (const char* e = std::getenv("TM_LEVELS_FUSED")) levels_fused = std::atoi(e) != 0;
    if (!levels_fused) return;
    int LEVEL_STRIP = 60;
    if (const char* e = std::getenv("TM_LEVEL_STRIP")) LEVEL_STRIP = std::max(4, std::atoi(e));
    const std::vector<EdgeRun>* const runs[3] = {&level[0].runs, &level[1].runs, &level[2].runs};
    const StripPlan plan = build_strip_plan(runs, level[2].where, LEVEL_STRIP);
    fused_levels.nstrips = plan.nstrips;
    fused_levels.tasks = static_cast<const LevelTask*>(upload_table(plan.tasks.data(), plan.tasks.size() * sizeof(LevelTask)));
    fused_levels.off = static_cast<const int32_t*>(upload_table(plan.off.data(), plan.off.size() * 4));
    if (std::getenv("TM_DEBUG_RUNS"))
        std::fprintf(stderr, "[tm] fused level kernel: %d strips, %zu wave tasks (level tables: %d / %d / %d rows)\n", fused_levels.nstrips, plan.tasks.size(),
                     edge_L[0].nrows, edge_L[1].nrows, edge_L[2].nrows);
}

uint64_t Smoother::size_launches() {
    const int edge_wg = (opt.inner == TM_INNER_RELAX ? edge_nf.nwg : edge.nwg);
    apply_rows = 0;
    auto launch_wgs = [&](int rows, bool overlap) {
        int total = edge_wg;
        for (int64_t b : lp.owned_blocks)
            total += overlap ? apply_block_nwg_overlap(static_cast<int>(topo.ni[b]), static_cast<int>(topo.nj[b]), rows)
                             : apply_block_nwg(static_cast<int>(topo.ni[b]), static_cast<int>(topo.nj[b]), rows);
        return total;
    };
    const bool vk_able = !has_hooks && opt.inner == TM_INNER_BICGSTAB && !(opt.flags & TM_OPT_EAGER_SCALARS);
    auto shortest_rows = [&](bool overlap) {
        for (int r = 3; r <= (vk_able ? 36 : 15); r += 3)
            if (launch_wgs(r, overlap) <= 512) return r;
        return 0;
    };
    apply_rows = shortest_rows(false);
    vk_overlap = vk_able && lp.n_owned >= 50000 && lp.n_owned <= 12000000;
    if (vk_overlap && launch_wgs(apply_rows, false) <= 256 && launch_wgs(shortest_rows(true), true) > 256) vk_overlap = false;
    if (const char* e = std::getenv("TM_VK_OVERLAP")) vk_overlap = vk_able && std::atoi(e) != 0;
    if (vk_overlap) apply_rows = shortest_rows(true);
    if (vk_able && !apply_rows && lp.owned_blocks.size() > 1) apply_rows = 24;
    if (!apply_rows && opt.inner == TM_INNER_RELAX) apply_rows = 6;
    if (const char* e = std::getenv("TM_APPLY_ROWS")) apply_rows = std::max(0, std::atoi(e));
    poff.clear();
    int off = 0;
    for (int64_t b : lp.owned_blocks) {
        poff.push_back(off);
        off += apply_block_nwg(static_cast<int>(topo.ni[b]), static_cast<int>(topo.nj[b]), apply_rows);
    }
    poff_edge = off;
    off += edge_wg;
    nwg_apply = off;
    if (fuse_pairs) {
        poff2.clear();
        rows2.clear();
        int off2 = 0;
        for (int64_t b : lp.owned_blocks) {
            const int bi = static_cast<int>(topo.ni[b]), bj = static_cast<int>(topo.nj[b]);
            poff2.push_back(off2);
            rows2.push_back(relax2_rows_per_chunk(bi, bj));
            off2 += relax2_block_nwg(bi, bj, rows2.back());
            const std::vector<int32_t> ids = relax2_border_tiles(bi, bj, rows2.back(), dyn_mask[poff2.size() - 1]);
            border_n.push_back(static_cast<int>(ids.size()));
            border_ids.push_back(static_cast<const int32_t*>(upload_table(ids.data(), ids.size() * 4)));
        }
        poff2_edge = off2;
        nwg_apply2 = off2 + edge_nf.nwg;
    }
    pipelined_single = fuse_pairs && !(has_hooks && (lp.send_ids.size() > 0 || !lp.ghost_gid.empty())) && edge_nf.nrows > 0 && lp.n_owned >= (1 << 21);
    if (const char* e = std::getenv("TM_SINGLE_PIPELINED")) pipelined_single = pipelined_single && std::atoi(e) != 0;
    fuse_triples = fuse_pairs && edge_nf.nrows == 0 && !(has_hooks && (!lp.send_ids.empty() || !lp.ghost_gid.empty()));
    if (const char* e = std::getenv("TM_FUSE_3")) fuse_triples = fuse_triples && std::atoi(e) != 0;
    if (fuse_triples || triples_coupled) {
        poff3.clear();
        rows3.clear();
        int off3 = 0;
        rows3 = relax3_rows_of_owned_blocks();
        for (size_t k = 0; k < lp.owned_blocks.size(); ++k) {
            const int64_t b = lp.owned_blocks[k];
            const int bi = static_cast<int>(topo.ni[b]), bj = static_cast<int>(topo.nj[b]);
            if (!relax3_supported(bi, bj)) fuse_triples = false;
            poff3.push_back(off3);
            off3 += relax3_block_nwg(bi, bj, rows3[k]);
        }
        nwg_apply3 = off3;
    }
    fuse_quads = fuse_triples;
    bool quads_forced = false;
    if (const char* e = std::getenv("TM_FUSE_4")) {
        fuse_quads = fuse_quads && std::atoi(e) != 0;
        quads_forced = std::atoi(e) != 0;
    }
    nwg_apply4 = 0;
    if (fuse_quads) {
        std::vector<int> bi, bj;
        for (size_t first = 0; first < lp.owned_blocks.size(); first += APPLY_BATCH_MAX) {
            int64_t nodes = 0;
            for (size_t k = first; k < std::min<size_t>(first + APPLY_BATCH_MAX, lp.owned_blocks.size()); ++k) nodes += topo.ni[lp.owned_blocks[k]] * topo.nj[lp.owned_blocks[k]];
            if (nodes < QUAD_MIN_NODES && !quads_forced) fuse_quads = false;
        }
        for (int64_t b : lp.owned_blocks) {
            bi.push_back(static_cast<int>(topo.ni[b]));
            bj.push_back(static_cast<int>(topo.nj[b]));
            if (!relax4_supported(bi.back(), bj.back())) fuse_quads = false;
        }
        poff4.clear();
        rows4.assign(bi.size(), 1);
        for (size_t first = 0; first < rows4.size(); first += APPLY_BATCH_MAX)
            relax4_rows_for_launch(bi.data() + first, bj.data() + first, static_cast<int>(std::min<size_t>(APPLY_BATCH_MAX, rows4.size() - first)), rows4.data() + first);
        int off4 = 0;
        for (size_t k = 0; k < rows4.size(); ++k) {
            poff4.push_back(off4);
            off4 += relax4_block_nwg(bi[k], bj[k], rows4[k]);
        }
        nwg_apply4 = fuse_quads ? off4 : 0;
    }
    nwg_vec = vec_nwg(n_owned);
    const int nwg3_all = std::max(nwg_apply4, fuse_triples ? nwg_apply3 : (triples_coupled ? nwg_apply3 + std::max(edge_L[2].nwg, fused_levels.nstrips) : 0));
    if (vk_overlap) {
        int off_ov = 0;
        for (int64_t b : lp.owned_blocks) {
            poff_ov.push_back(off_ov);
            off_ov += apply_block_nwg_overlap(static_cast<int>(topo.ni[b]), static_cast<int>(topo.nj[b]), apply_rows);
        }
        poff_edge_ov = off_ov;
        nwg_apply_ov = off_ov + edge.nwg;
    }
    if (vk_able && std::max(nwg_apply, nwg_apply_ov) <= 512) nwg_vec = std::min(nwg_vec, 512);
    lazy = !has_hooks && opt.inner != TM_INNER_RELAX && std::max(std::max(nwg_apply, nwg_apply_ov), nwg_vec) <= 512 && !(opt.flags & TM_OPT_EAGER_SCALARS);
    const int nwg_refine = refine() ? csr_nwg(n_owned) : 0;
    const uint64_t npart = static_cast<uint64_t>(std::max(std::max(std::max(std::max(std::max(nwg_apply, nwg_apply_ov), nwg_apply2), nwg3_all), nwg_vec), nwg_refine)) * MAX_PARTIALS;
    fuse_s = !has_hooks && opt.inner == TM_INNER_BICGSTAB && !(opt.flags & TM_OPT_EAGER_SCALARS);
    fuse_p = fuse_s;
    if (const char* e = std::getenv("TM_FUSE_P")) fuse_p = fuse_p && std::atoi(e) != 0;
    fuse2 = fuse_p;
    if (const char* e = std::getenv("TM_FUSE_2")) fuse2 = fuse2 && std::atoi(e) != 0;
    if (fuse_p) {
        p_alt = vec();
        v_alt = vec();
    }
    if (fuse2) r_alt = vec();
    const int rows = static_cast<int>(npart / MAX_PARTIALS);
    const struct {
        const char* what;
        int nwg;
    } producers[] = {{"operator", nwg_apply},
                     {"operator (overlapping strips)", nwg_apply_ov},
                     {"sweep pairs", nwg_apply2},
                     {"sweep triples", nwg3_all},
                     {"vector kernels", nwg_vec},
                     {"GMRES Gram-Schmidt", (opt.inner == TM_INNER_GMRES || reference()) ? vec_nwg(n_owned) : 0},
                     {"perimeter-row right-hand side", opt.inner != TM_INNER_RELAX ? edge.nwg : 0},
                     {"refinement step", nwg_refine}};
    if (std::getenv("TM_DEBUG_RUNS"))
        std::fprintf(stderr, "[tm] partial-sum rows: %d allocated; operator %d, overlapping strips %d, pairs %d, triples %d, vector kernels %d (vec_nwg %d)\n", rows,
                     nwg_apply, nwg_apply_ov, nwg_apply2, nwg3_all, nwg_vec, vec_nwg(n_owned));
    for (const auto& q : producers)
        if (q.nwg > rows)
            throw TmError(TM_E_HIP, std::string("internal: the ") + q.what + " launch has " + std::to_string(q.nwg) + " workgroups, the partial-sum buffer " +
                                        std::to_string(rows) + " rows");
    return npart;
}

void Smoother::alloc_reductions(uint64_t npart) {
    partials_guard = false;
    if (const char* e = std::getenv("TM_PARTIALS_GUARD")) partials_guard = std::atoi(e) != 0;
    const uint64_t nguard = partials_guard ? GUARD_DOUBLES : 0;
    for (int k = 0; k < (lazy ? 3 : 1); ++k) part_buf[k] = arena.alloc_n<double>(npart + nguard);
    partials = part_buf[0];
    red = arena.alloc_n<double>(MAX_PARTIALS + nguard);
    if (partials_guard) {
        for (int k = 0; k < 3; ++k) guard[k] = part_buf[k] ? part_buf[k] + npart : nullptr;
        guard[3] = red ? red + MAX_PARTIALS : nullptr;
    }
    S_buf[0] = arena.alloc_n<KrylovScalars>(1);
    S_buf[1] = lazy ? arena.alloc_n<KrylovScalars>(1) : S_buf[0];
    S = S_buf[0];
    sync_flags = arena.alloc_n<uint32_t>(64);

    n_send = static_cast<int64_t>(lp.send_ids.size());
    if (n_send) {
        d_send_ids = static_cast<int32_t*>(upload_table(lp.send_ids.data(), static_cast<uint64_t>(n_send) * 4));
        d_send_buf = arena.alloc_n<double2>(static_cast<uint64_t>(n_send));
    }
}

void Smoother::finish_create(const tm_mesh_desc* mesh) {
    HIPCHK(hipHostMalloc(reinterpret_cast<void**>(&h_S), sizeof(KrylovScalars), hipHostMallocDefault));
    pipelined_poll = lazy;
    if (const char* e = std::getenv("TM_PIPELINED_POLL")) pipelined_poll = pipelined_poll && std::atoi(e) != 0;
    if (pipelined_poll)
        for (int k = 0; k < 2; ++k) {
            HIPCHK(hipHostMalloc(reinterpret_cast<void**>(&h_poll[k]), sizeof(KrylovScalars), hipHostMallocDefault));
            HIPCHK(hipEventCreateWithFlags(&ev_poll[k], hipEventDisableTiming));
        }
    HIPCHK(hipHostMalloc(reinterpret_cast<void**>(&h_red), sizeof(double) * MAX_PARTIALS, hipHostMallocDefault));
    if (gm_S) {
        HIPCHK(hipHostMalloc(reinterpret_cast<void**>(&h_gm), sizeof(GmresScalars), hipHostMallocDefault));
        HIPCHK(hipMemsetAsync(gm_S, 0, sizeof(GmresScalars), stream));
        HIPCHK(hipMemsetAsync(gm_V, 0, sizeof(double2) * static_cast<size_t>(n_local) * (GMRES_M + 1), stream));
        HIPCHK(hipMemsetAsync(r, 0, sizeof(double2) * n_local, stream));
    }
    HIPCHK(hipMemsetAsync(S_buf[0], 0, sizeof(KrylovScalars), stream));
    if (S_buf[1] != S_buf[0]) HIPCHK(hipMemsetAsync(S_buf[1], 0, sizeof(KrylovScalars), stream));
    HIPCHK(hipMemsetAsync(sync_flags, 0, sizeof(uint32_t) * 64, stream));
    for (double* g : guard)
        if (g) HIPCHK(hipMemsetAsync(g, GUARD_BYTE, sizeof(double) * GUARD_DOUBLES, stream));
    HIPCHK(hipHostMalloc(reinterpret_cast<void**>(&h_flags), sizeof(uint32_t) * 8, hipHostMallocDefault));
    std::memset(h_flags, 0, sizeof(uint32_t) * 8);
    for (double2* q : {p_hat, s_hat, mg_w0, mg_w1})
        if (q) HIPCHK(hipMemsetAsync(q, 0, sizeof(double2) * n_local, stream));
    if (PQ) HIPCHK(hipMemsetAsync(PQ, 0, sizeof(double2) * n_local, stream));
    upload(mesh);
    if (white) white_launch(0);
    if (refine()) csr_fill_values();
    if (reference()) reference_create();
    sync();
}

void Smoother::upload(const tm_mesh_desc* mesh) {
    check_desc_matches(topo, mesh);
    for (int64_t b : lp.owned_blocks)
        if (!mesh->blocks[b].xy) throw TmError(TM_E_ARG, "owned block without coordinates");
    connection_data_check(topo, mesh, owner, lp.rank);
    for (size_t k = 0; k < lp.owned_blocks.size(); ++k) {
        const int64_t b = lp.owned_blocks[k];
        HIPCHK(hipMemcpyAsync(X + lp.local_start[k], mesh->blocks[b].xy, sizeof(double2) * topo.ni[b] * topo.nj[b], hipMemcpyHostToDevice, stream));
    }
    for (size_t k = 0; k < lp.rows.size(); ++k) {
        const PlanRow& pr = lp.rows[k];
        h_rhs[2 * k] = pr.rhs[0];
        h_rhs[2 * k + 1] = pr.rhs[1];
        if (pr.rhs_coord) {
            const int64_t b = block_of(topo, pr.gid);
            const double* xy = mesh->blocks[b].xy + 2 * (pr.gid - topo.start[b]);
            if (pr.rhs_coord & 1) h_rhs[2 * k] = xy[0];
            if (pr.rhs_coord & 2) h_rhs[2 * k + 1] = xy[1];
        }
    }
    std::vector<double> staged;
    size_t total = 0;
    for (const RhsTable& t : rhs_tables) total += 2 * t.src.size();
    staged.reserve(total);
    for (const RhsTable& t : rhs_tables) {
        if (!t.dev || t.src.empty()) continue;
        const size_t base = staged.size();
        for (const double* v : t.src) {
            staged.push_back(v[0]);
            staged.push_back(v[1]);
        }
        HIPCHK(hipMemcpyAsync(t.dev, staged.data() + base, sizeof(double) * (staged.size() - base), hipMemcpyHostToDevice, stream));
    }
    if (opt.inner == TM_INNER_RELAX) prefill_fixed();
    sync();
}

void Smoother::prefill_fixed() {
    for (size_t k = 0; k < lp.owned_blocks.size(); ++k) {
        const int64_t b = lp.owned_blocks[k];
        const int64_t ls = lp.local_start[k];
        const int bi = static_cast<int>(topo.ni[b]), bj = static_cast<int>(topo.nj[b]);
        HIPCHK(launch_copy_perimeter(X + ls, U + ls, bi, bj, stream));
        if (M) HIPCHK(launch_copy_perimeter(X + ls, M + ls, bi, bj, stream));
        if (M2) HIPCHK(launch_copy_perimeter(X + ls, M2 + ls, bi, bj, stream));
    }
}

void Smoother::download(const tm_mesh_desc* mesh) {
// ... 757 lines not shown
        for (int j = 0; j < GMRES_M && it_total < opt.max_inner; ++j) {
            HIPCHK(launch_csr_product(n_owned, csr.p, csr.i, csr.vx, csr.vy, V(j), W, stream));
            precondition_W();
            st.operator_sweeps += 1;
            HIPCHK(launch_gm_mgs(W, nullptr, V(0), nullptr, gm_S, 0, n_owned, partials, stream));
            reduce(nwg_vec);
            for (int i = 1; i <= j; ++i) {
                HIPCHK(launch_gm_mgs(W, V(i - 1), V(i), red, gm_S, i - 1, n_owned, partials, stream));
                reduce(nwg_vec);
            }
            HIPCHK(launch_gm_mgs(W, V(j), nullptr, red, gm_S, j, n_owned, partials, stream));
            reduce(nwg_vec);
            HIPCHK(launch_gm_column(gm_S, red, stream));
            HIPCHK(launch_gm_divide(V(j + 1), W, gm_S, n_owned, stream));
            it_total += 1;
            if ((j + 1) % static_cast<int>(opt.check_every) == 0 || j + 1 == GMRES_M || it_total == opt.max_inner) {
                if (poll()) {
                    cycle_done = true;
                    break;
                }
            }
        }
        HIPCHK(launch_gm_backsub(gm_S, stream));
        HIPCHK(launch_gm_update(U, gm_V, ld, gm_S, n_owned, stream));
        if (cycle_done) {
            converged = true;
            break;
        }
    }
    HIPCHK(hipMemcpyAsync(h_gm, gm_S, sizeof(GmresScalars), hipMemcpyDeviceToHost, stream));
    sync();
    inner_counts[0] = static_cast<uint64_t>(h_gm->iters[0]);
    inner_counts[1] = static_cast<uint64_t>(h_gm->iters[1]);
    st.inner_iterations += inner_counts[0] + inner_counts[1];

    HIPCHK(launch_residual_copyback(X, U, n_owned, nwg_vec, partials, stream));
    reduce(nwg_vec);
    HIPCHK(hipMemcpyAsync(h_red, red, sizeof(double) * MAX_PARTIALS, hipMemcpyDeviceToHost, stream));
    sync();
    st.last_dx2 = h_red[0];
    st.last_dy2 = h_red[1];
    st.last_residual = (h_red[0] + h_red[1]) * (h_red[0] + h_red[1]);
    outer_done += 1;
    return converged ? 0 : 1;
}

void Smoother::relax2_launch(int subset, bool counts, int dot, hipStream_t on, const QueueWait* wait) {
    if (!on) on = stream;
    std::vector<Relax2Block> blocks(lp.owned_blocks.size());
    for (size_t k = 0; k < lp.owned_blocks.size(); ++k) {
        const int64_t b = lp.owned_blocks[k];
        const int64_t ls = lp.local_start[k];
        Relax2Block& a = blocks[k];
        a.in = X + ls;
        a.mid = M + ls;
        a.out = U + ls;
        a.ni = static_cast<int>(topo.ni[b]);
        a.nj = static_cast<int>(topo.nj[b]);
        a.omega = opt.omega;
        a.dyn = dyn_mask[k];
        a.store_nt = relax2_store_nt ? 1 : 0;
        a.border = border_ids[k];
        a.nborder = border_n[k];
        a.partials = partials + static_cast<size_t>(poff2[k]) * MAX_PARTIALS;
    }
    const size_t lds = (subset == R2_INSIDE) ? inside_lds : 0;
    profiled([&]() { HIPCHK(launch_relax2_blocks(blocks.data(), rows2.data(), static_cast<int>(blocks.size()), dot, subset, on, lds, wait)); }, counts, on);
}

std::vector<int> Smoother::relax3_rows_of_owned_blocks() const {
    std::vector<int> rows(lp.owned_blocks.size(), 1), bi, bj;
    for (int64_t b : lp.owned_blocks) {
        bi.push_back(static_cast<int>(topo.ni[b]));
        bj.push_back(static_cast<int>(topo.nj[b]));
    }
    for (size_t first = 0; first < rows.size(); first += APPLY_BATCH_MAX) {
        const int n = static_cast<int>(std::min<size_t>(APPLY_BATCH_MAX, rows.size() - first));
        relax3_rows_for_launch(bi.data() + first, bj.data() + first, n, rows.data() + first, triples_coupled);
    }
    return rows;
}

void Smoother::ensure_side() {
    if (side) return;
    int least = 0, greatest = 0;
    HIPCHK(hipDeviceGetStreamPriorityRange(&least, &greatest));
    HIPCHK(hipStreamCreateWithPriority(&side, hipStreamNonBlocking, greatest));
    HIPCHK(hipEventCreateWithFlags(&ev_to_side, hipEventDisableTiming));
    HIPCHK(hipEventCreateWithFlags(&ev_to_main, hipEventDisableTiming));
    HIPCHK(hipEventCreateWithFlags(&ev_inside[0], hipEventDisableTiming));
    HIPCHK(hipEventCreateWithFlags(&ev_inside[1], hipEventDisableTiming));
    if (pair_sync_events) queue_ordering = ORDER_EVENTS_REQUESTED;
    else queue_ordering = queue_self_test() ? ORDER_COUNTERS : ORDER_EVENTS_SELF_TEST;
}

bool Smoother::queue_self_test() {
    HIPCHK(hipStreamSynchronize(stream));
    HIPCHK(hipStreamSynchronize(side));
    uint32_t* a = sync_flags + 8;
    uint32_t* b = sync_flags + 9;
    uint32_t* err = sync_flags + 10;
    HIPCHK(hipMemsetAsync(sync_flags + 8, 0, sizeof(uint32_t) * 4, stream));
    HIPCHK(hipStreamSynchronize(stream));
    HIPCHK(launch_queue_signal_wait(a, b, 1u, err, stream, QUEUE_SELF_TEST_TICKS));
    HIPCHK(launch_queue_signal_wait(b, a, 1u, err, side, QUEUE_SELF_TEST_TICKS));
    HIPCHK(hipStreamSynchronize(stream));
    HIPCHK(hipStreamSynchronize(side));
    uint32_t h[4] = {0, 0, 0, 0};
    HIPCHK(hipMemcpy(h, sync_flags + 8, sizeof(h), hipMemcpyDeviceToHost));
    return h[2] == 0u && h[0] == 1u && h[1] == 1u;
}

bool Smoother::use_counters() {
    if (queue_ordering == ORDER_EVENTS_REQUESTED || queue_ordering == ORDER_EVENTS_SELF_TEST) return false;
    if (g_multirank_handles.load() > 1) {
        queue_ordering = ORDER_EVENTS_SHARED_PROCESS;
        return false;
    }
    queue_ordering = ORDER_COUNTERS;
    return true;
}

void Smoother::warm_transport() {
    if (transport_warm) return;
    transport_warm = true;
    if (!(has_hooks && (n_send > 0 || n_ghost > 0))) return;
    exchange(X, side);
    exchange_finish(side);
    HIPCHK(hipStreamSynchronize(side));
}

void Smoother::relax_triple(bool want_partials) { relax_fixed_walls(3, want_partials); }
void Smoother::relax_quad(bool want_partials) { relax_fixed_walls(4, want_partials); }
void Smoother::relax_fixed_walls(int depth, bool want_partials) {
    const int dot = want_partials ? DOT_DELTA : DOT_NONE;
    const std::vector<int>& poffd = depth == 4 ? poff4 : poff3;
    std::vector<Relax2Block> blocks(lp.owned_blocks.size());
    for (size_t k = 0; k < lp.owned_blocks.size(); ++k) {
        const int64_t b = lp.owned_blocks[k];
        const int64_t ls = lp.local_start[k];
        Relax2Block& a = blocks[k];
        a.in = X + ls;
        a.mid = nullptr;
        a.out = U + ls;
        a.ni = static_cast<int>(topo.ni[b]);
        a.nj = static_cast<int>(topo.nj[b]);
        a.omega = opt.omega;
        a.dyn = 0;
        a.store_nt = relax2_store_nt ? 1 : 0;
        a.border = nullptr;
        a.nborder = 0;
        a.partials = partials + static_cast<size_t>(poffd[k]) * MAX_PARTIALS;
    }
    if (depth == 4) profiled([&]() { HIPCHK(launch_relax4_blocks(blocks.data(), rows4.data(), static_cast<int>(blocks.size()), dot, stream)); }, true, stream);
    else profiled([&]() { HIPCHK(launch_relax3_blocks(blocks.data(), rows3.data(), static_cast<int>(blocks.size()), dot, stream)); }, true, stream);
    std::swap(X, U);
}

void Smoother::relax_triples_coupled(uint64_t ntriples, bool want_partials_last) {
    ensure_side();
    const bool use_flags = use_counters();
    uint32_t* chain_done = sync_flags;
    uint32_t* inside_done = sync_flags + 1;
    uint32_t* sync_err = sync_flags + 2;
    if (use_flags) HIPCHK(hipMemsetAsync(sync_flags, 0, sizeof(uint32_t) * 4, stream));
    fence(stream, side, ev_to_side);
    warm_transport();
    std::vector<Relax2Block> blocks(lp.owned_blocks.size());
    for (uint64_t q = 0; q < ntriples; ++q) {
        const int dot = (q + 1 == ntriples && want_partials_last) ? DOT_DELTA : DOT_NONE;
        for (size_t k = 0; k < lp.owned_blocks.size(); ++k) {
            const int64_t b = lp.owned_blocks[k];
            const int64_t ls = lp.local_start[k];
            Relax2Block& a = blocks[k];
            a.in = X + ls;
            a.mid = nullptr;
            a.out = U + ls;
            a.ni = static_cast<int>(topo.ni[b]);
            a.nj = static_cast<int>(topo.nj[b]);
            a.omega = opt.omega;
            a.dyn = dyn_mask[k];
            a.store_nt = relax2_store_nt ? 1 : 0;
            a.border = nullptr;
            a.nborder = 0;
            a.partials = partials + static_cast<size_t>(poff3[k]) * MAX_PARTIALS;
        }
        if (q > 0) {
            if (use_flags) HIPCHK(launch_queue_signal_wait(inside_done, chain_done, static_cast<uint32_t>(q), sync_err, stream));
            else HIPCHK(hipStreamWaitEvent(stream, ev_to_main, 0));
        }
        profiled([&]() { HIPCHK(launch_relax3_blocks(blocks.data(), rows3.data(), static_cast<int>(blocks.size()), dot, stream)); }, true, stream);
        if (!use_flags) HIPCHK(hipEventRecord(ev_inside[q & 1], stream));
        if (q > 0) {
            if (use_flags) HIPCHK(launch_queue_signal_wait(chain_done, inside_done, static_cast<uint32_t>(q), sync_err, side));
            else HIPCHK(hipStreamWaitEvent(side, ev_inside[(q - 1) & 1], 0));
        }
        exchange(X, side);
        exchange_finish(side);
        if (levels_fused) {
            HIPCHK(launch_edge_levels3(fused_levels, edge_L[0], edge_L[1], edge_L[2], X, M, M2, U, PQ, opt.omega, dot,
                                       partials + static_cast<size_t>(nwg_apply3) * MAX_PARTIALS, side));
        } else {
            HIPCHK(launch_edge_rows(edge_L[0], X, X, PQ, nullptr, M, opt.omega, MODE_RELAX, DOT_NONE, partials, side));
            HIPCHK(launch_edge_rows(edge_L[1], M, M, PQ, nullptr, M2, opt.omega, MODE_RELAX, DOT_NONE, partials, side));
            HIPCHK(launch_edge_rows(edge_L[2], M2, M2, PQ, nullptr, U, opt.omega, MODE_RELAX, dot, partials + static_cast<size_t>(nwg_apply3) * MAX_PARTIALS, side));
        }
        if (q + 1 < ntriples && !use_flags) HIPCHK(hipEventRecord(ev_to_main, side));
        std::swap(X, U);
    }
    fence(side, stream, ev_to_main);
    if (use_flags) {
        HIPCHK(hipMemcpyAsync(h_flags + 4, sync_flags, sizeof(uint32_t) * 4, hipMemcpyDeviceToHost, stream));
        flags_pending = true;
    }
}

void Smoother::relax_pair(bool want_partials) {
    const int dot = want_partials ? DOT_DELTA : DOT_NONE;
    HIPCHK(launch_edge_rows(edge_nf, X, X, PQ, nullptr, M, opt.omega, MODE_RELAX, DOT_NONE, partials, stream));
    relax2_launch(R2_ALL, true, dot);
    HIPCHK(launch_edge_rows(edge_nf, M, M, PQ, nullptr, U, opt.omega, MODE_RELAX, dot, partials + static_cast<size_t>(poff2_edge) * MAX_PARTIALS, stream));
    std::swap(X, U);
}

void Smoother::relax_pairs_pipelined(uint64_t npairs, bool want_partials_last) {
    ensure_side();
    const bool use_flags = use_counters();
    uint32_t* border_done = sync_flags;
    uint32_t* inside_done = sync_flags + 1;
    uint32_t* sync_err = sync_flags + 2;
    uint32_t n_border = 0, n_inside = 0;
    if (use_flags) HIPCHK(hipMemsetAsync(sync_flags, 0, sizeof(uint32_t) * 4, stream));
    auto signal_border = [&]() {
        if (use_flags) HIPCHK(launch_queue_signal(border_done, side));
        else HIPCHK(hipEventRecord(ev_to_main, side));
        n_border += 1;
    };
    auto wait_border = [&]() {
        if (use_flags) HIPCHK(launch_queue_wait(border_done, n_border, sync_err, stream));
        else HIPCHK(hipStreamWaitEvent(stream, ev_to_main, 0));
    };
    auto signal_inside = [&]() {
        if (use_flags) HIPCHK(launch_queue_signal(inside_done, stream));
        else HIPCHK(hipEventRecord(ev_inside[n_inside & 1], stream));
        n_inside += 1;
    };
    auto wait_inside = [&](uint32_t upto) {
        if (use_flags) HIPCHK(launch_queue_wait(inside_done, upto, sync_err, side));
        else HIPCHK(hipStreamWaitEvent(side, ev_inside[(upto - 1) & 1], 0));
    };
    const EdgeRowsDev& e1 = edge_nf_g.nrows ? edge_nf_g : edge_nf;
    auto edge_on_side = [&](const EdgeRowsDev& e, const double2* in, double2* out, int dot, uint32_t* signal = nullptr) {
        HIPCHK(launch_edge_rows(e, in, in, PQ, nullptr, out, opt.omega, MODE_RELAX, dot, partials + static_cast<size_t>(poff2_edge) * MAX_PARTIALS, side, signal));
    };
    auto exchange_on_side = [&](double2* vec) {
        exchange(vec, side);
        exchange_finish(side);
    };
    auto border_pass = [&](uint32_t inside_upto, int dot) {
        if (use_flags && inside_upto > 0) {
            QueueWait w;
            w.counter = inside_done;
            w.target = inside_upto;
            w.error = sync_err;
            relax2_launch(R2_BORDER, true, dot, side, &w);
        } else {
            if (inside_upto > 0) wait_inside(inside_upto);
            relax2_launch(R2_BORDER, true, dot, side);
        }
    };
    int dot = (npairs == 1 && want_partials_last) ? DOT_DELTA : DOT_NONE;
    fence(stream, side, ev_to_side);
    warm_transport();
    exchange_on_side(X);
    edge_on_side(e1, X, M, DOT_NONE);
    relax2_launch(R2_INSIDE, false, dot);
    if (!use_flags || npairs == 1) signal_inside();
    border_pass(0, dot);
    for (uint64_t k = 0; k < npairs; ++k) {
        const bool announce = k + 1 < npairs;
        if (use_flags && announce) {
            edge_on_side(edge_nf, M, U, dot, border_done);
            n_border += 1;
        } else {
            edge_on_side(edge_nf, M, U, dot);
            if (announce) signal_border();
        }
        std::swap(X, U);
        if (k + 1 == npairs) {
            fence(side, stream, ev_to_main);
            break;
        }
        dot = (k + 2 == npairs && want_partials_last) ? DOT_DELTA : DOT_NONE;
        if (use_flags) {
            HIPCHK(launch_queue_signal_wait(inside_done, border_done, n_border, sync_err, stream));
            n_inside += 1;
        } else {
            wait_border();
        }
        relax2_launch(R2_INSIDE, false, dot);
        if (!use_flags) signal_inside();
        exchange_on_side(X);
        edge_on_side(e1, X, M, DOT_NONE);
        border_pass(static_cast<uint32_t>(k + 1), dot);
    }
    if (use_flags) {
        HIPCHK(hipMemcpyAsync(h_flags, sync_flags, sizeof(uint32_t) * 4, hipMemcpyDeviceToHost, stream));
// ... 359 lines not shown
```

turbomesh_amd/csrc/tm_smoother.hpp:

```cpp
#pragma once
#include "../../include/tm_hip.h"
#include <cstdlib>
#include "tm_edge_tables.hpp"
#include "tm_kernels.h"
#include "tm_multigrid.hpp"
#include "tm_plan.hpp"
#include <cmath>
#include <atomic>
#include <memory>
#include <string>
#include <functional>
#include <vector>

namespace tmh {

struct TmError : std::runtime_error {
    int code;
    TmError(int c, const std::string& m) : std::runtime_error(m), code(c) {}
};
void hip_check(hipError_t e, const char* what);
extern std::atomic<int> g_multirank_handles;
extern tm_log_fn g_log_sink;
extern void* g_log_ctx;

class DeviceArena {
   public:
    DeviceArena() = default;
    ~DeviceArena();
    void use_workspace(void* base, uint64_t bytes);
    void measure_only();
    void* alloc(uint64_t bytes);
    template <class T>
    T* alloc_n(uint64_t n) { return static_cast<T*>(alloc(n * sizeof(T))); }
    uint64_t used() const { return used_; }
    bool measuring() const { return measure_; }

   private:
    std::vector<void*> owned_;
    char* base_ = nullptr;
    uint64_t cap_ = 0, used_ = 0;
    bool external_ = false, measure_ = false;
};

struct QualityDev;

struct Smoother {
    Smoother() = default;
    ~Smoother();
    Smoother(const Smoother&) = delete;
    Smoother& operator=(const Smoother&) = delete;
    Topology topo;
    std::vector<PlanRow> all_rows;
    LocalPlan lp;
    tm_solver_opt opt{};
    tm_control_fn cf{};
    tm_comm_hooks hooks{};
    bool has_hooks = false;
    std::vector<int32_t> owner;
    hipStream_t stream = nullptr;
    DeviceArena arena;

    int64_t n_owned = 0, n_local = 0, n_ghost = 0, dof_global = 0;
    double2 *X = nullptr, *U = nullptr, *r = nullptr, *r_hat = nullptr, *p = nullptr, *v = nullptr, *s = nullptr, *t = nullptr;
    double2 *PQ = nullptr, *tmpA = nullptr, *tmpB = nullptr;
    double2 *p_hat = nullptr, *s_hat = nullptr, *mg_w0 = nullptr, *mg_w1 = nullptr;
    std::vector<BlockMG> mg;
    bool use_mg = false;
    bool mg_perimeter_step = false;
    bool mg_dirichlet = false;
    std::vector<hipStream_t> mg_streams;
    std::vector<hipEvent_t> mg_join;
    hipEvent_t mg_fork = nullptr;
    int mg_perimeter_sweeps = 2;
    void precondition(const double2* in, double2* out);
    void precondition_probe_host(const double* f, double* z, double* f_after);
    double2* M = nullptr;
    double2* M2 = nullptr;
    bool fuse_pairs = false;
    bool relax2_store_nt = true;
    bool pair_sync_events = false;
    size_t inside_lds = 0;
    EdgeRowsDev edge;
    std::vector<double> h_rhs;
    struct RhsTable {
        double* dev = nullptr;
        std::vector<const double*> src;
    };
    std::vector<RhsTable> rhs_tables;
    EdgeRowsDev edge_nf;
    EdgeRowsDev edge_nf_g;
    std::vector<int> dyn_mask;
    std::vector<const int32_t*> border_ids;
    std::vector<int> border_n;
    void prefill_fixed();
    double* partials = nullptr;
    double* red = nullptr;
    KrylovScalars* S = nullptr;
    KrylovScalars* h_S = nullptr;
    bool pipelined_poll = false, poll_open = false;
    KrylovScalars* h_poll[2] = {nullptr, nullptr};
    hipEvent_t ev_poll[2] = {nullptr, nullptr};
    uint64_t poll_it[2] = {0, 0}, poll_iters = 0;
    int poll_slot = 0;
    int poll_done(uint64_t it, bool final);
    double stall_best[2] = {0.0, 0.0};
    uint64_t stall_since = 0, stall_window = 4000;
    bool stalled = false;
    double* h_red = nullptr;
    bool vk_overlap = false;
    std::vector<int> poff_ov;
    int poff_edge_ov = 0, nwg_apply_ov = 0;
    std::vector<int> poff;
    int poff_edge = 0, nwg_apply = 0, nwg_vec = 0;
    std::vector<int> poff2, rows2;
    int poff2_edge = 0, nwg_apply2 = 0;
    std::vector<int> poff3, rows3;
    int nwg_apply3 = 0;
    bool fuse_triples = false;
    std::vector<int> poff4, rows4;
    int nwg_apply4 = 0;
    bool fuse_quads = false;
    static constexpr int64_t QUAD_MIN_NODES = 8000000;
    bool triples_coupled = false;
    EdgeRowsDev edge_L[3];
    bool levels_fused = false;
    FusedLevelsDev fused_levels;
    bool pipelined_single = false;
    int32_t* d_send_ids = nullptr;
    double2* d_send_buf = nullptr;
    int64_t n_send = 0;
    bool white = false;
    ConnShifts white_le{};
    uint64_t outer_done = 0;
    int profile = 0;
    std::vector<hipEvent_t> ev_start, ev_stop;
    size_t ev_used = 0;
    uint64_t prof_launches = 0;
    uint64_t prof_timed = 0;
    uint64_t prof_open = 0;
    uint64_t prof_phase = 0;
    void profile_close(hipStream_t on);
    void profile_read(double* ms_total, uint64_t* launches, uint64_t* timed);

    void create(const tm_mesh_desc* mesh, const tm_solver_opt* o, const tm_control_fn* c, const tm_comm_hooks* h, void* strm,
                bool measure);
    void upload(const tm_mesh_desc* mesh);
    void download(const tm_mesh_desc* mesh);
    void iterate(uint64_t iterations, tm_stats* stats);
    bool iterate_until(uint64_t max_iterations, double tol, tm_stats* stats);
    bool iterate_until_update(uint64_t max_iterations, double tol, tm_stats* stats);
    double stop_tol = 0.0;
    void apply_host(const double* in_xy, double* out_xy, int scaled);
    uint64_t assemble_csr_host(int32_t* Ap, int32_t* Ai, double* Ax_x, double* Ax_y, uint64_t nnz_capacity);
    void apply_reference_host(const double* in_xy, double* out_xy);
    struct AssembledCsr {
        int32_t *p = nullptr, *i = nullptr;
        double *vx = nullptr, *vy = nullptr;
        uint64_t nnz = 0;
        std::vector<int32_t> h_p, h_i;
    } csr;
    void csr_build_pattern();
    void csr_fill_values();
    void csr_release();
    void csr_free();
    void rhs_host(double* rhs_xy);
    void residual_host(const double* xy, double* r_xy);
    void control_function_host(double* pq);
    void export_soa_host(int64_t block, double* x, double* y, double* p, double* q);
    void* export_buf = nullptr;
    size_t export_bytes = 0;
    QualityDev* qdev = nullptr;
    void quality_host(tm_quality* per_block, tm_quality* total);
    void quality_field_host(int64_t block, double* out);

    void exchange(double2* vec, hipStream_t on = nullptr);
    void exchange_finish(hipStream_t on = nullptr);
    hipStream_t side = nullptr;
    hipEvent_t ev_to_side = nullptr, ev_to_main = nullptr, ev_inside[2] = {nullptr, nullptr};
    void fence(hipStream_t from, hipStream_t to, hipEvent_t ev);
    enum { ORDER_UNDECIDED = -1, ORDER_COUNTERS = 0, ORDER_EVENTS_REQUESTED = 1, ORDER_EVENTS_SHARED_PROCESS = 2, ORDER_EVENTS_SELF_TEST = 3 };
    int queue_ordering = ORDER_UNDECIDED;
    void ensure_side();
    bool queue_self_test();
    bool use_counters();
    bool transport_warm = false;
    void warm_transport();
    void relax_pairs_pipelined(uint64_t npairs, bool want_partials_last);
    uint32_t* sync_flags = nullptr;
    uint32_t* h_flags = nullptr;
    bool flags_pending = false;
    bool counted = false;
    bool exchange_pending = false;
    void apply(const double2* in, double2* out, int mode, int dot, const double2* aux, const double2* xk, double omega, int step = -1);
    void reduce(int nwg);
    void reduce_update(int nwg, int step, double rtol = 0.0, double atol = 0.0);
    int apply_rows = 0;
    bool fuse_s = false;
    bool fuse_p = false;
    bool fuse2 = false;
    double2 *p_alt = nullptr, *v_alt = nullptr, *r_alt = nullptr;
    void apply_virtual(int kind, const double2* in, const double2* in2, const double2* in3, double2* pout, double2* out, const double2* in4 = nullptr,
                       double2* rout = nullptr, double2* uio = nullptr);
    bool lazy = false;
    double* part_buf[3] = {nullptr, nullptr, nullptr};
    static constexpr uint64_t GUARD_DOUBLES = 2048 * MAX_PARTIALS;
    static constexpr int GUARD_BYTE = 0xA5;
    bool partials_guard = false;
    double* guard[4] = {nullptr, nullptr, nullptr, nullptr};
    void check_guards();
    int part_rot = 0;
    KrylovScalars* S_buf[2] = {nullptr, nullptr};
    LazyStep pending[2];
    int npending = 0;
    void flush_pending();
    LazyScalars scalars_for();
    void white_launch(int update);
    void sync();
    void ensure_tmp();

    double2* gm_V = nullptr;
    GmresScalars* gm_S = nullptr;
    GmresScalars* h_gm = nullptr;

    struct ReferenceSolve;
    ReferenceSolve* ref = nullptr;
    void reference_create();
    double2* ref_b = nullptr;
    double2 *rf_r = nullptr, *rf_d = nullptr, *rf_dinv = nullptr;
    uint32_t refine_steps = 0;
    double refine_rel[2] = {0.0, 0.0};
    double refine_rtol = 0.0;
    uint64_t refine_iterations = 0;
    bool refine() const { return (opt.flags & TM_OPT_REFINE) != 0; }
    uint64_t inner_counts[2] = {0, 0};

   private:
    struct Selection;
    bool reference() const { return opt.inner == TM_INNER_REFERENCE_GMRES; }
    double2* vec() { return arena.alloc_n<double2>(static_cast<uint64_t>(n_local)); }
    void resolve_options(const tm_mesh_desc* mesh, const tm_solver_opt* o, const tm_control_fn* c, const tm_comm_hooks* h, bool measure);
    void plan_mesh(const tm_mesh_desc* mesh, const tm_comm_hooks* h, bool measure);
    void alloc_vectors(const tm_mesh_desc* mesh, bool measure);
    void decide_schedule();
    void* upload_table(const void* src, uint64_t bytes);
    RunTable make_table(const Selection& sel, EdgeRowsDev& e);
    void build_row_tables();
    uint64_t size_launches();
    void alloc_reductions(uint64_t npart);
    void finish_create(const tm_mesh_desc* mesh);
    int picard_bicgstab(tm_stats& st);
    int picard_gmres(tm_stats& st);
    int picard_reference(tm_stats& st);
    void refine_solution();
    uint64_t correct_bicgstab(const double2* rhs, double2* d);
    uint64_t correct_gmres(const double2* rhs, double2* d);
    int picard_solve(tm_stats& st) {
        const uint64_t before = st.inner_iterations;
        if (opt.inner == TM_INNER_REFERENCE_GMRES) return picard_reference(st);
        const int rc = opt.inner == TM_INNER_GMRES ? picard_gmres(st) : picard_bicgstab(st);
        inner_counts[0] = inner_counts[1] = st.inner_iterations - before;
        return rc;
    }
    void relax_sweeps(uint64_t n, tm_stats& st);
    void relax_pair(bool want_partials);
    std::vector<int> relax3_rows_of_owned_blocks() const;
    void relax_triple(bool want_partials);
    void relax_quad(bool want_partials);
    void relax_fixed_walls(int depth, bool want_partials);
    void relax_triples_coupled(uint64_t ntriples, bool want_partials_last);
    void profiled(const std::function<void()>& launch, bool counts = true, hipStream_t on = nullptr);
    void relax2_launch(int subset, bool counts, int dot, hipStream_t on = nullptr, const QueueWait* wait = nullptr);
};

// ... 26 lines not shown
```

turbomesh_amd/smoothing/smooth.py:

```python
from __future__ import annotations

import ctypes as C
import logging

import numpy as np

from .. import _capi
from . import solver as _solver
from . import wall_control_function as _wcf

log = logging.getLogger("smoothing")


def _log_sink(ctx, what, iteration, value):
    if what == 0:
        log.info("iteration: %d", iteration)
    elif what == 1:
        log.info("\tresidual: %r", value)
    elif what == 2:
        log.info("\trefinement steps: %d", int(value))
    elif what in (3, 4):
        log.info("\tlast refinement update |d|/|%s|: %r", "xy"[what - 3], value)
    elif what == 5:
        log.info("\tinner iterations in corrections: %d", int(value))
# ... 76 lines not shown
    def write(self, filename, with_control_function=True):
        from .. import output

        output.write_smoother(self, filename, with_control_function)

    def quality(self):
        from .. import quality

        n = len(self._mesh.blocks)
        per_block = (_capi.tm_quality * max(1, n))()
        total = _capi.tm_quality()
        _capi.check(_capi.lib().tm_smoother_quality(self._h, per_block, C.byref(total)))
        return quality.records(per_block[:n], total)

    def quality_field(self, block: int):
        ni, nj = self._mesh.blocks[block].points.size
        plane = np.empty((ni - 1) * (nj - 1), dtype=np.float64)
        _capi.check(_capi.lib().tm_smoother_quality_field(self._h, block, _capi.f64ptr(plane)))
        return plane.reshape(nj - 1, ni - 1).T

    def write_quality(self, filename):
        from .. import output

        sizes, fields = [], []
        for b, blk in enumerate(self._mesh.blocks):
            ni, nj = blk.points.size
            sizes.append((ni - 1, nj - 1))
            fields.append([np.ascontiguousarray(self.quality_field(b).T).reshape(-1)])
        output.write_plot3d_function(filename, sizes, fields)

    def iterate_until(self, scaled_residual_tol: float, max_iterations: int = 1000):
        st = _capi.tm_stats()
        rc = _capi.lib().tm_smoother_iterate_until(self._h, max_iterations, C.c_double(scaled_residual_tol), C.byref(st))
        if rc < 0:
            _capi.check(rc)
        return rc == 0, st.as_dict()

    def iterate_until_update(self, update_rms_tol: float, max_iterations: int = 1000):
        st = _capi.tm_stats()
        rc = _capi.lib().tm_smoother_iterate_until_update(self._h, max_iterations, C.c_double(update_rms_tol), C.byref(st))
        if rc < 0:
            _capi.check(rc)
        return rc == 0, st.as_dict()

    def download(self):
        _capi.check(_capi.lib().tm_smoother_download(self._h, self._md.ref()))

    def upload(self):
        _capi.check(_capi.lib().tm_smoother_upload(self._h, self._md.ref()))

    def apply(self, vec, scaled=False):
        vec = np.ascontiguousarray(vec, dtype=np.float64)
        assert vec.shape == (self.dof, 2)
        out = np.empty_like(vec)
        _capi.check(_capi.lib().tm_smoother_apply(self._h, _capi.f64ptr(vec), _capi.f64ptr(out), 1 if scaled else 0))
        return out

    def assemble_csr(self):
        n = C.c_uint64(0)
        _capi.check(_capi.lib().tm_smoother_assemble_csr(self._h, None, None, None, None, 0, C.byref(n)))
        nnz = int(n.value)
        Ap, Ai = np.empty(self.dof + 1, dtype=np.int32), np.empty(nnz, dtype=np.int32)
        Ax, Ay = np.empty(nnz), np.empty(nnz)
        ip = C.POINTER(C.c_int32)
        _capi.check(_capi.lib().tm_smoother_assemble_csr(self._h, Ap.ctypes.data_as(ip), Ai.ctypes.data_as(ip), _capi.f64ptr(Ax), _capi.f64ptr(Ay), nnz, C.byref(n)))
        return Ap, Ai, Ax, Ay

    def apply_reference_order(self, vec):
        vec = np.ascontiguousarray(vec, dtype=np.float64)
        assert vec.shape == (self.dof, 2)
        out = np.empty_like(vec)
        _capi.check(_capi.lib().tm_smoother_apply_reference_order(self._h, _capi.f64ptr(vec), _capi.f64ptr(out)))
        return out

    def rhs(self):
        out = np.empty((self.dof, 2))
        _capi.check(_capi.lib().tm_smoother_rhs(self._h, _capi.f64ptr(out)))
        return out

    def refine_report(self):
        steps, rel, its = (C.c_uint32 * 2)(), (C.c_double * 2)(), C.c_uint64(0)
        _capi.check(_capi.lib().tm_smoother_refine_report(self._h, steps, rel, C.byref(its)))
        return {"steps": (int(steps[0]), int(steps[1])), "last_update_rel": (float(rel[0]), float(rel[1])), "correction_iterations": int(its.value)}

    def residual(self, xy=None):
        out = np.empty((self.dof, 2))
        if xy is not None:
            xy = np.ascontiguousarray(xy, dtype=np.float64)
            assert xy.shape == (self.dof, 2)
        _capi.check(_capi.lib().tm_smoother_residual(self._h, None if xy is None else _capi.f64ptr(xy), _capi.f64ptr(out)))
        return out

    def row_kinds(self):
        out = np.empty(self.dof, dtype=np.int32)
        _capi.check(_capi.lib().tm_smoother_row_kinds(self._h, out.ctypes.data_as(C.POINTER(C.c_int32))))
        return out

    def profile(self, every=1):
        _capi.check(_capi.lib().tm_smoother_profile(self._h, int(every)))

    def profile_read(self):
        ms = C.c_double(0)
        timed = C.c_uint64(0)
        n = C.c_uint64(0)
        _capi.check(_capi.lib().tm_smoother_profile_read(self._h, C.byref(ms), C.byref(timed), C.byref(n)))
        return ms.value, int(timed.value), int(n.value)

    QUEUE_ORDERING = {-1: "none", 0: "counters", 1: "events (TM_PAIR_SYNC=events)", 2: "events (several multi-rank handles in this process)",
                      3: "events (self-test: both streams on one hardware queue)"}

    def queue_ordering(self):
        code = int(_capi.lib().tm_smoother_queue_ordering(self._h))
        return code, self.QUEUE_ORDERING.get(code, "?")

    def mg_levels(self, block: int = 0):
        i32 = C.POINTER(C.c_int32)
        n, omega = C.c_int32(0), C.c_double(0)
        shape, cycle = np.zeros(4 * 32, dtype=np.int32), np.zeros(6, dtype=np.int32)
        _capi.check(_capi.lib().tm_smoother_mg_levels(self._h, block, C.byref(n), shape.ctypes.data_as(i32), 32, cycle.ctypes.data_as(i32), C.byref(omega)))
        return {"levels": [tuple(int(v) for v in shape[4 * l:4 * l + 4]) for l in range(n.value)], "nu_pre": int(cycle[0]), "nu_post": int(cycle[1]),
                "nu_coarsest": int(cycle[2]), "omega": omega.value, "dirichlet": bool(cycle[3]), "perimeter_step": bool(cycle[4]),
                "perimeter_sweeps": int(cycle[5])}

    def precondition_probe(self, f, return_input=False):
        f = np.ascontiguousarray(f, dtype=np.float64)
        assert f.shape == (self.dof, 2)
        z = np.empty_like(f)
        after = np.empty_like(f) if return_input else None
        _capi.check(_capi.lib().tm_smoother_precondition_probe(self._h, _capi.f64ptr(f), _capi.f64ptr(z), _capi.f64ptr(after) if return_input else None))
        return (z, after) if return_input else z

    def control_function(self):
        out = np.empty((self.dof, 2))
        _capi.check(_capi.lib().tm_smoother_control_function(self._h, _capi.f64ptr(out)))
        return out


def plan_rows(mesh_data):
    md = _capi.MeshDesc(mesh_data, with_coordinates=False)
    rows = _capi.tm_plan_rows()
    _capi.check(_capi.lib().tm_plan_build(md.ref(), C.byref(rows)))
    try:
        n = int(rows.nrows)
        as_np = np.ctypeslib.as_array
        out = {
            "row": as_np(rows.row, (n,)).copy(), "kind": as_np(rows.kind, (n,)).copy(), "ncols": as_np(rows.ncols, (n,)).copy(),
            "cols": as_np(rows.cols, (n * 9,)).reshape(n, 9).copy(), "coef_x": as_np(rows.coef_x, (n * 9,)).reshape(n, 9).copy(),
            "coef_y": as_np(rows.coef_y, (n * 9,)).reshape(n, 9).copy(), "rhs": as_np(rows.rhs, (n * 2,)).reshape(n, 2).copy(),
            "slot": as_np(rows.slot, (n * 9,)).reshape(n, 9).copy(),
        }
    finally:
        _capi.lib().tm_plan_free(C.byref(rows))
    return out
```

Measured before the change: 475.1 billion.

## Drive depth-4 relax kernel from a host-built tile table with optional balanced plan

Replaces the in-kernel computation of tile coordinates (XCD-swizzled index arithmetic over uniform row chunks) with a precomputed per-workgroup TileRec table uploaded once, and adds a planner that can build either uniform or makespan-balanced tiles across XCDs. By default the plan mode is uniform, so the main runtime change is one 16-byte table load per workgroup instead of integer division and swizzle math, plus per-batch launches. The balanced planner, exposed through the C API and Python, is enabled only by environment variable and is meant to reduce tail imbalance, at the cost of extra host planning and a device table.

```diff
diff --git a/include/tm_hip.h b/include/tm_hip.h
--- a/include/tm_hip.h
+++ b/include/tm_hip.h
@@ -225,6 +225,30 @@
 int tm_plan_build(const tm_mesh_desc* mesh, tm_plan_rows* out);
 void tm_plan_free(tm_plan_rows* rows);
 
+typedef struct tm_tile_plan_opt {
+    int32_t depth;
+    int32_t cus;
+    int32_t wg_per_cu;
+    int32_t mode;
+    int32_t forced_rows;
+    int32_t pick;
+    double c0, lone_rate;
+} tm_tile_plan_opt;
+typedef struct tm_tile_plan {
+    int64_t ntiles;
+    int32_t* block;
+    int32_t* sg;
+    int32_t* i0;
+    int32_t* i1;
+    int32_t* slot;
+    int32_t mode;
+    int32_t uniform_rows;
+    double makespan;
+    double uniform_makespan;
+} tm_tile_plan;
+int tm_tile_plan_build(const int32_t* ni, const int32_t* nj, int32_t nblocks, const tm_tile_plan_opt* opt, tm_tile_plan* out);
+void tm_tile_plan_free(tm_tile_plan* plan);
+
 typedef struct tm_plan_local_info {
     int64_t n_owned, n_ghost, n_send;
     int32_t npeers, nowned_blocks;
diff --git a/turbomesh_amd/_capi.py b/turbomesh_amd/_capi.py
--- a/turbomesh_amd/_capi.py
+++ b/turbomesh_amd/_capi.py
@@ -84,6 +84,17 @@
     _fields_ = [("nrows", C.c_uint64), ("row", C.POINTER(C.c_int64)), ("kind", C.POINTER(C.c_int32)), ("ncols", C.POINTER(C.c_int32)),
                 ("cols", C.POINTER(C.c_int64)), ("coef_x", C.POINTER(C.c_double)), ("coef_y", C.POINTER(C.c_double)),
                 ("rhs", C.POINTER(C.c_double)), ("slot", C.POINTER(C.c_int32))]
+
+
+class tm_tile_plan_opt(C.Structure):
+    _fields_ = [("depth", C.c_int32), ("cus", C.c_int32), ("wg_per_cu", C.c_int32), ("mode", C.c_int32), ("forced_rows", C.c_int32),
+                ("pick", C.c_int32), ("c0", C.c_double), ("lone_rate", C.c_double)]
+
+
+class tm_tile_plan(C.Structure):
+    _fields_ = [("ntiles", C.c_int64), ("block", C.POINTER(C.c_int32)), ("sg", C.POINTER(C.c_int32)), ("i0", C.POINTER(C.c_int32)),
+                ("i1", C.POINTER(C.c_int32)), ("slot", C.POINTER(C.c_int32)), ("mode", C.c_int32), ("uniform_rows", C.c_int32),
+                ("makespan", C.c_double), ("uniform_makespan", C.c_double)]
 
 
 class tm_plan_local_info(C.Structure):
@@ -129,6 +140,7 @@
     "tm_rccl_peer_table_build", "tm_rccl_peer_table_free", "tm_white_math_probe", "tm_stream_probe", "tm_smoother_queue_ordering", "tm_smoother_inner", "tm_csr_ilu0_probe", "tm_rccl_hooks_for", "tm_smoother_assemble_csr", "tm_smoother_apply_reference_order",
     "tm_smoother_inner_counts", "tm_mesh_quality", "tm_mesh_quality_host", "tm_smoother_quality", "tm_smoother_quality_field",
     "tm_csr_residual", "tm_smoother_residual", "tm_smoother_refine_report",
+    "tm_tile_plan_build", "tm_tile_plan_free",
     "tm_mg_transfer_probe", "tm_smoother_mg_levels", "tm_smoother_precondition_probe", "tm_edge_tables_probe", "tm_edge_tables_free",
 ]
 
@@ -206,6 +218,9 @@
         L.tm_plan_build.argtypes = [C.POINTER(tm_mesh_desc), C.POINTER(tm_plan_rows)]
         L.tm_plan_free.argtypes = [C.POINTER(tm_plan_rows)]
         L.tm_plan_free.restype = None
+        L.tm_tile_plan_build.argtypes = [C.POINTER(C.c_int32), C.POINTER(C.c_int32), C.c_int32, C.POINTER(tm_tile_plan_opt), C.POINTER(tm_tile_plan)]
+        L.tm_tile_plan_free.argtypes = [C.POINTER(tm_tile_plan)]
+        L.tm_tile_plan_free.restype = None
         L.tm_export_soa.argtypes = [_dp, C.c_uint64, C.c_uint64, _dp, _dp]
         L.tm_smoother_export_soa.argtypes = [C.c_void_p, C.c_uint64, _dp, _dp, _dp, _dp]
         L.tm_mesh_quality.argtypes = [C.POINTER(tm_mesh_desc), C.POINTER(tm_quality), C.POINTER(tm_quality)]
diff --git a/turbomesh_amd/csrc/tm_api.cpp b/turbomesh_amd/csrc/tm_api.cpp
--- a/turbomesh_amd/csrc/tm_api.cpp
+++ b/turbomesh_amd/csrc/tm_api.cpp
@@ -847,4 +847,51 @@
     std::memset(rows, 0, sizeof(*rows));
 }
 
-}
+int tm_tile_plan_build(const int32_t* ni, const int32_t* nj, int32_t nblocks, const tm_tile_plan_opt* opt, tm_tile_plan* out) {
+    return guarded([&]() {
+        if (!ni || !nj || !opt || !out) throw TmError(TM_E_ARG, "null argument");
+        std::memset(out, 0, sizeof(*out));
+        TilePlanParams p;
+        p.L = opt->depth;
+        p.cus = opt->cus;
+        p.wg_per_cu = opt->wg_per_cu;
+        p.mode = opt->mode;
+        p.forced_rows = opt->forced_rows;
+        p.pick = opt->pick;
+        if (opt->c0 > 0.0) p.c0 = opt->c0;
+        if (opt->lone_rate > 0.0) p.lone_rate = opt->lone_rate;
+        const std::vector<int> bi(ni, ni + std::max(0, nblocks)), bj(nj, nj + std::max(0, nblocks));
+        const TilePlan plan = build_tile_plan(bi.data(), bj.data(), nblocks, p);
+        const size_t n = plan.tiles.size();
+        int32_t** const dst[5] = {&out->block, &out->sg, &out->i0, &out->i1, &out->slot};
+        for (int q = 0; q < 5; ++q) {
+            *dst[q] = static_cast<int32_t*>(std::malloc(sizeof(int32_t) * (n ? n : 1)));
+            if (!*dst[q]) {
+                tm_tile_plan_free(out);
+                throw TmError(TM_E_MEMORY, "out of host memory");
+            }
+        }
+        for (size_t k = 0; k < n; ++k) {
+            const TileRec& t = plan.tiles[k];
+            out->block[k] = t.bsg & 15;
+            out->sg[k] = t.bsg >> 4;
+            out->i0[k] = t.i0;
+            out->i1[k] = t.i1;
+            out->slot[k] = t.slot;
+        }
+        out->ntiles = static_cast<int64_t>(n);
+        out->mode = plan.mode;
+        out->uniform_rows = plan.uniform_rows;
+        out->makespan = plan.makespan;
+        out->uniform_makespan = plan.uniform_makespan;
+        return TM_OK;
+    });
+}
+void tm_tile_plan_free(tm_tile_plan* plan) {
+    if (!plan) return;
+    int32_t* const arrays[] = {plan->block, plan->sg, plan->i0, plan->i1, plan->slot};
+    for (int32_t* p : arrays) std::free(p);
+    std::memset(plan, 0, sizeof(*plan));
+}
+
+}
diff --git a/turbomesh_amd/csrc/tm_edge_types.h b/turbomesh_amd/csrc/tm_edge_types.h
--- a/turbomesh_amd/csrc/tm_edge_types.h
+++ b/turbomesh_amd/csrc/tm_edge_types.h
@@ -32,3 +32,10 @@
     const int32_t* off = nullptr;
 };
 constexpr int LEVELS_BLOCK = 512;
+
+struct TileRec {
+    int32_t bsg;
+    int32_t i0, i1;
+    int32_t slot;
+};
+static_assert(sizeof(TileRec) == 16, "one 16-byte uniform load per workgroup");
diff --git a/turbomesh_amd/csrc/tm_kernels.h b/turbomesh_amd/csrc/tm_kernels.h
--- a/turbomesh_amd/csrc/tm_kernels.h
+++ b/turbomesh_amd/csrc/tm_kernels.h
@@ -106,9 +106,8 @@
 int relax3_block_nwg(int ni, int nj, int rows_per_chunk);
 hipError_t launch_relax3_blocks(const Relax2Block* blocks, const int* rows_per_chunk, int n, int dot, hipStream_t stream);
 bool relax4_supported(int ni, int nj);
-void relax4_rows_for_launch(const int* ni, const int* nj, int n, int* rows);
-int relax4_block_nwg(int ni, int nj, int rows_per_chunk);
-hipError_t launch_relax4_blocks(const Relax2Block* blocks, const int* rows_per_chunk, int n, int dot, hipStream_t stream);
+int relax4_wg_per_cu(bool omega_is_one, bool store_nt);
+hipError_t launch_relax4_blocks(const Relax2Block* blocks, int n, const TileRec* tiles, int ntiles, int dot, hipStream_t stream);
 
 hipError_t launch_edge_levels3(const FusedLevelsDev& F, const EdgeRowsDev& e1, const EdgeRowsDev& e2, const EdgeRowsDev& e3, const double2* x, double2* m,
                                double2* m2, double2* out, const double2* pq, double omega, int dot, double* partials ,
diff --git a/turbomesh_amd/csrc/tm_kernels.hip b/turbomesh_amd/csrc/tm_kernels.hip
--- a/turbomesh_amd/csrc/tm_kernels.hip
+++ b/turbomesh_amd/csrc/tm_kernels.hip
@@ -915,7 +915,6 @@
     relax3_tile<DOT, U, NT, W1>(B.b[k], B.RI[k], B.nSG[k], B.nRC[k], static_cast<int>(blockIdx.x) - B.start[k]);
 }
 constexpr int R4_L = 4;
-constexpr int R4_W = 64 - 2 * R4_L;
 template <int L, int DOT, int U, int NT, bool W1, bool INSIDE>
 __device__ __forceinline__ void relaxn_strip(const Relax2Block& a, const Relax2Tile& t, double (&acc)[MAX_PARTIALS]) {
     static_assert(U == 3 && L >= 3, "three steps per group; the windows rotate by renaming");
@@ -988,41 +987,37 @@
 }
 
 template <int L, int DOT, int U, int NT, bool W1>
-__device__ __forceinline__ void relaxn_tile(const Relax2Block& a, int RI, int nSG, int nRC, int bid) {
+__device__ __forceinline__ void relaxn_tile(const Relax2Block& a, const TileRec& tt) {
     constexpr int W = 64 - 2 * L;
     const int lane = threadIdx.x & 63;
     const int wave = threadIdx.x >> 6;
-    const int total = nSG * nRC;
-    const int q8 = total >> 3, rem = total & 7, xcd = bid & 7, k8 = bid >> 3;
-    const int logical = (xcd < rem) ? xcd * (q8 + 1) + k8 : rem * (q8 + 1) + (xcd - rem) * q8 + k8;
-    const int rc = logical / nSG;
-    const int sg = logical - rc * nSG;
+    const int sg = tt.bsg >> 4;
     const int ni = a.ni, nj = a.nj;
     Relax2Tile t;
     t.c0 = (sg * 4 + wave) * W;
     t.c = t.c0 - L + lane;
     t.out_lane = (lane >= L) && (lane < 64 - L) && (t.c >= 1) && (t.c <= nj - 2);
-    t.i0 = 1 + rc * RI;
-    t.i1 = min(t.i0 + RI, ni - 1);
+    t.i0 = tt.i0;
+    t.i1 = tt.i1;
     double acc[MAX_PARTIALS] = {0.0, 0.0, 0.0, 0.0};
     if (t.c0 <= nj - 2 && t.i0 < t.i1) {
         const bool inside = (t.c0 - L >= 1) && (t.c0 - L + 63 <= nj - 2) && (t.i0 - L >= 1) && (t.i1 + L - 1 <= ni - 2);
         if (inside) relaxn_strip<L, DOT, U, NT, W1, true>(a, t, acc);
         else relaxn_strip<L, DOT, U, NT, W1, false>(a, t, acc);
     }
-    if (DOT != DOT_NONE) block_partials<256, dot_columns(DOT)>(acc, a.partials + static_cast<size_t>(logical) * MAX_PARTIALS);
+    if (DOT != DOT_NONE) block_partials<256, dot_columns(DOT)>(acc, a.partials + static_cast<size_t>(tt.slot) * MAX_PARTIALS);
 }
 template <int DOT, int U, int NT, bool W1>
-__global__ __launch_bounds__(256) void k_relax4(Relax2Block a, int RI, int nSG, int nRC) {
-    relaxn_tile<R4_L, DOT, U, NT, W1>(a, RI, nSG, nRC, blockIdx.x);
+__global__ __launch_bounds__(256) void k_relax4(Relax2Block a, const TileRec* __restrict__ tiles) {
+    const TileRec tt = tiles[blockIdx.x];
+    if (tt.slot < 0) return;
+    relaxn_tile<R4_L, DOT, U, NT, W1>(a, tt);
 }
 template <int DOT, int U, int NT, bool W1>
-__global__ __launch_bounds__(256) void k_relax4_batch(Relax2Batch B) {
-    int k = 0;
-#pragma unroll
-    for (int q = 1; q < APPLY_BATCH_MAX; ++q)
-        if (q < B.n && static_cast<int>(blockIdx.x) >= B.start[q]) k = q;
-    relaxn_tile<R4_L, DOT, U, NT, W1>(B.b[k], B.RI[k], B.nSG[k], B.nRC[k], static_cast<int>(blockIdx.x) - B.start[k]);
+__global__ __launch_bounds__(256) void k_relax4_batch(Relax2Batch B, const TileRec* __restrict__ tiles) {
+    const TileRec tt = tiles[blockIdx.x];
+    if (tt.slot < 0) return;
+    relaxn_tile<R4_L, DOT, U, NT, W1>(B.b[tt.bsg & 15], tt);
 }
 static int g_fuse3_rows = 0;
 void relax3_rows_for_launch(const int* ni, const int* nj, int n, int* rows, bool beside_chain) {
@@ -1061,27 +1056,6 @@
     const int nstrips = (nj - 1 + R3_W - 1) / R3_W;
     return ((nstrips + 3) / 4) * ((ni - 2 + RI - 1) / RI);
 }
-static hipError_t launch_fixed_wall_blocks(int depth, const Relax2Block* blocks, const int* rows_per_chunk, int n, int dot, hipStream_t st) {
-    const int W = 64 - 2 * depth;
-    for (int first = 0; first < n; first += APPLY_BATCH_MAX) {
-        Relax2Batch B;
-        B.n = 0;
-        int total = 0;
-        bool w1 = true;
-        const bool nts = blocks[first].store_nt != 0;
-        for (int k = first; k < n && B.n < APPLY_BATCH_MAX; ++k) {
-            const int q = B.n++;
-            B.b[q] = blocks[k];
-            B.RI[q] = rows_per_chunk[k];
-            B.nSG[q] = ((blocks[k].nj - 1 + W - 1) / W + 3) / 4;
-            B.nRC[q] = (blocks[k].ni - 2 + B.RI[q] - 1) / B.RI[q];
-            B.start[q] = total;
-            total += B.nSG[q] * B.nRC[q];
-            w1 = w1 && blocks[k].omega == 1.0;
-        }
-        for (int q = B.n; q < APPLY_BATCH_MAX; ++q) B.start[q] = total;
-        if (total == 0) continue;
-        const dim3 grid(total), block(256);
 #define TM_R3(KERNEL, ...)                                                                                                   \
     do {                                                                                                                     \
         if (dot == DOT_DELTA) {                                                                                              \
@@ -1094,61 +1068,66 @@
             else hipLaunchKernelGGL((KERNEL<DOT_NONE, R3_U, 1, false>), grid, block, 0, st, __VA_ARGS__);                    \
         }                                                                                                                    \
     } while (0)
-        static const bool force_batch = [] { const char* e = std::getenv("TM_R3_FORCE_BATCH"); return e && std::atoi(e) != 0; }();
-        const bool lone = B.n == 1 && !force_batch;
-        if (depth == R4_L) {
-            if (lone) TM_R3(k_relax4, B.b[0], B.RI[0], B.nSG[0], B.nRC[0]);
-            else TM_R3(k_relax4_batch, B);
-        } else {
-            if (lone) TM_R3(k_relax3, B.b[0], B.RI[0], B.nSG[0], B.nRC[0]);
-            else TM_R3(k_relax3_batch, B);
-        }
-#undef TM_R3
+static bool force_batch_launches() {
+    static const bool force_batch = [] { const char* e = std::getenv("TM_R3_FORCE_BATCH"); return e && std::atoi(e) != 0; }();
+    return force_batch;
+}
+hipError_t launch_relax3_blocks(const Relax2Block* blocks, const int* rows_per_chunk, int n, int dot, hipStream_t st) {
+    for (int first = 0; first < n; first += APPLY_BATCH_MAX) {
+        Relax2Batch B;
+        B.n = 0;
+        int total = 0;
+        bool w1 = true;
+        const bool nts = blocks[first].store_nt != 0;
+        for (int k = first; k < n && B.n < APPLY_BATCH_MAX; ++k) {
+            const int q = B.n++;
+            B.b[q] = blocks[k];
+            B.RI[q] = rows_per_chunk[k];
+            B.nSG[q] = ((blocks[k].nj - 1 + R3_W - 1) / R3_W + 3) / 4;
+            B.nRC[q] = (blocks[k].ni - 2 + B.RI[q] - 1) / B.RI[q];
+            B.start[q] = total;
+            total += B.nSG[q] * B.nRC[q];
+            w1 = w1 && blocks[k].omega == 1.0;
+        }
+        for (int q = B.n; q < APPLY_BATCH_MAX; ++q) B.start[q] = total;
+        if (total == 0) continue;
+        const dim3 grid(total), block(256);
+        if (B.n == 1 && !force_batch_launches()) TM_R3(k_relax3, B.b[0], B.RI[0], B.nSG[0], B.nRC[0]);
+        else TM_R3(k_relax3_batch, B);
         const hipError_t rc = hipGetLastError();
         if (rc != hipSuccess) return rc;
     }
     return hipSuccess;
 }
-hipError_t launch_relax3_blocks(const Relax2Block* blocks, const int* rows_per_chunk, int n, int dot, hipStream_t st) {
-    return launch_fixed_wall_blocks(3, blocks, rows_per_chunk, n, dot, st);
-}
-
-void relax4_rows_for_launch(const int* ni, const int* nj, int n, int* rows) {
-    static const int forced = [] { const char* e = std::getenv("TM_FUSE4_ROWS"); return e ? std::atoi(e) : 0; }();
-    if (forced > 0) {
-        for (int k = 0; k < n; ++k) rows[k] = std::max(1, std::min(forced, ni[k] - 2));
-        return;
-    }
-    static int slots = 0;
-    if (slots == 0) {
-        int dev = 0, cus = 0;
-        if (hipGetDevice(&dev) != hipSuccess || hipDeviceGetAttribute(&cus, hipDeviceAttributeMultiprocessorCount, dev) != hipSuccess || cus <= 0) cus = 256;
-        slots = 3 * cus;
-    }
-    static const int heights[] = {54, 42, 30, 18, 6};
-    const long need = static_cast<long>(slots) * 6;
-    int RI = 6;
-    for (const int h : heights) {
-        long total = 0;
-        for (int k = 0; k < n; ++k) {
-            const int nstrips = (nj[k] - 1 + R4_W - 1) / R4_W, nSG = (nstrips + 3) / 4, interior = ni[k] - 2, r = std::max(1, std::min(h, interior));
-            total += static_cast<long>(nSG) * ((interior + r - 1) / r);
-        }
-        RI = h;
-        if (total * 10 >= need) break;
-    }
-    for (int k = 0; k < n; ++k) rows[k] = std::max(1, std::min(RI, ni[k] - 2));
-}
+
 bool relax4_supported(int ni, int nj) { return ni >= 2 * R4_L + 1 && nj >= 2 * R4_L + 1 && nj <= (1 << 20); }
-int relax4_block_nwg(int ni, int nj, int RI) {
-    const int nstrips = (nj - 1 + R4_W - 1) / R4_W;
-    return ((nstrips + 3) / 4) * ((ni - 2 + RI - 1) / RI);
-}
-hipError_t launch_relax4_blocks(const Relax2Block* blocks, const int* rows_per_chunk, int n, int dot, hipStream_t st) {
-    for (int k = 0; k < n; ++k)
-        if (blocks[k].dyn != 0) return hipErrorInvalidValue;
-    return launch_fixed_wall_blocks(R4_L, blocks, rows_per_chunk, n, dot, st);
-}
+hipError_t launch_relax4_blocks(const Relax2Block* blocks, int n, const TileRec* tiles, int ntiles, int dot, hipStream_t st) {
+    if (n < 1 || n > APPLY_BATCH_MAX || ntiles < 1) return hipErrorInvalidValue;
+    Relax2Batch B;
+    B.n = n;
+    bool w1 = true;
+    const bool nts = blocks[0].store_nt != 0;
+    for (int q = 0; q < n; ++q) {
+        if (blocks[q].dyn != 0) return hipErrorInvalidValue;
+        B.b[q] = blocks[q];
+        B.RI[q] = B.nSG[q] = B.nRC[q] = B.start[q] = 0;
+        w1 = w1 && blocks[q].omega == 1.0;
+    }
+    for (int q = n; q < APPLY_BATCH_MAX; ++q) B.RI[q] = B.nSG[q] = B.nRC[q] = B.start[q] = 0;
+    const dim3 grid(ntiles), block(256);
+    if (n == 1 && !force_batch_launches()) TM_R3(k_relax4, B.b[0], tiles);
+    else TM_R3(k_relax4_batch, B, tiles);
+    return hipGetLastError();
+}
+int relax4_wg_per_cu(bool omega_is_one, bool store_nt) {
+    int n = 0;
+    hipError_t rc;
+    if (omega_is_one && store_nt) rc = hipOccupancyMaxActiveBlocksPerMultiprocessor(&n, k_relax4<DOT_NONE, R3_U, 1, true>, 256, 0);
+    else if (omega_is_one) rc = hipOccupancyMaxActiveBlocksPerMultiprocessor(&n, k_relax4<DOT_NONE, R3_U, 0, true>, 256, 0);
+    else rc = hipOccupancyMaxActiveBlocksPerMultiprocessor(&n, k_relax4<DOT_NONE, R3_U, 1, false>, 256, 0);
+    return (rc == hipSuccess && n > 0) ? n : 0;
+}
+#undef TM_R3
 
 constexpr int MG_RST_W = 58;
 struct MgMetric {
diff --git a/turbomesh_amd/csrc/tm_plan.cpp b/turbomesh_amd/csrc/tm_plan.cpp
--- a/turbomesh_amd/csrc/tm_plan.cpp
+++ b/turbomesh_amd/csrc/tm_plan.cpp
@@ -2,6 +2,8 @@
 #include "../../include/tm_hip.h"
 #include <cstdlib>
 #include <algorithm>
+#include <cmath>
+#include <functional>
 #include <unordered_map>
 
 namespace tmh {
@@ -599,4 +601,275 @@
     return lp;
 }
 
-}
+
+namespace {
+
+constexpr int TILE_QMAX = 40;
+
+int tile_nsg(int nj, int L) {
+    const int W = 64 - 2 * L;
+    return ((nj - 1 + W - 1) / W + 3) / 4;
+}
+
+double simulate_xcd(const std::vector<double>& cost, int ncu, int slots, double lone_rate) {
+    std::vector<std::vector<double>> cu(ncu);
+    size_t next = 0;
+    double now = 0.0;
+    for (;;) {
+        while (next < cost.size()) {
+            int best = -1;
+            for (int c = 0; c < ncu; ++c)
+                if (static_cast<int>(cu[c].size()) < slots && (best < 0 || cu[c].size() < cu[best].size())) best = c;
+            if (best < 0) break;
+            cu[best].push_back(cost[next++]);
+        }
+        double dt = -1.0;
+        for (int c = 0; c < ncu; ++c) {
+            const int n = static_cast<int>(cu[c].size());
+            if (n == 0) continue;
+            const double rate = std::min(1.0, n * lone_rate) / n;
+            for (double r : cu[c]) {
+                const double t = r / rate;
+                if (dt < 0.0 || t < dt) dt = t;
+            }
+        }
+        if (dt < 0.0) break;
+        now += dt;
+        for (int c = 0; c < ncu; ++c) {
+            const int n = static_cast<int>(cu[c].size());
+            if (n == 0) continue;
+            const double done = dt * std::min(1.0, n * lone_rate) / n;
+            std::vector<double> keep;
+            for (double r : cu[c])
+                if (r - done > 1e-9) keep.push_back(r - done);
+            cu[c].swap(keep);
+        }
+    }
+    return now;
+}
+
+double simulate_table(const std::vector<TileRec>& tiles, const TilePlanParams& p) {
+    const int ncu = std::max(1, p.cus / p.xcds);
+    double worst = 0.0;
+    for (int x = 0; x < p.xcds; ++x) {
+        std::vector<double> cost;
+        for (size_t w = x; w < tiles.size(); w += p.xcds)
+            if (tiles[w].i1 > tiles[w].i0) cost.push_back(tile_cost(tiles[w].i1 - tiles[w].i0, p));
+        worst = std::max(worst, simulate_xcd(cost, ncu, std::max(1, p.wg_per_cu), p.lone_rate));
+    }
+    return worst;
+}
+
+std::vector<TileRec> uniform_tiles(const int* ni, const int* nj, int n, int L, const int* rows, std::vector<int>& block_slots) {
+    std::vector<TileRec> out;
+    block_slots.assign(n, 0);
+    for (int b = 0; b < n; ++b) {
+        const int RI = rows[b], nSG = tile_nsg(nj[b], L), nRC = (ni[b] - 2 + RI - 1) / RI, total = nSG * nRC;
+        const int q8 = total >> 3, rem = total & 7;
+        for (int bid = 0; bid < total; ++bid) {
+            const int xcd = bid & 7, k8 = bid >> 3;
+            const int logical = (xcd < rem) ? xcd * (q8 + 1) + k8 : rem * (q8 + 1) + (xcd - rem) * q8 + k8;
+            const int rc = logical / nSG, sg = logical - rc * nSG;
+            TileRec t;
+            t.bsg = b | (sg << 4);
+            t.i0 = 1 + rc * RI;
+            t.i1 = std::min(t.i0 + RI, ni[b] - 1);
+            t.slot = logical;
+            out.push_back(t);
+        }
+        block_slots[b] = total;
+    }
+    return out;
+}
+
+struct ColumnSeg {
+    int block, sg, u0, u1;
+    bool takes_rest;
+};
+
+void equal_heights(int u, int n, std::vector<int>& q) {
+    q.clear();
+    for (int k = 0; k < n; ++k) q.push_back(u / n + (k < u % n ? 1 : 0));
+}
+void tapered_heights(int u, int qbulk, int qmin, double share, std::vector<int>& q) {
+    q.clear();
+    int left = u;
+    while (left > 0) {
+        int h = static_cast<int>((left + share - 1) / share);
+        h = std::max(qmin, std::min(qbulk, h));
+        if (h > left || left - h < qmin) h = left;
+        if (h > TILE_QMAX) h = TILE_QMAX;
+        q.push_back(h);
+        left -= h;
+    }
+    std::sort(q.begin(), q.end(), [](int a, int b) { return a > b; });
+}
+
+}
+
+double tile_cost(int h, const TilePlanParams& p) {
+    const int steps = h + 2 * (p.L - 1);
+    return p.c0 + p.L * ((steps + 2) / 3 * 3) - 3 * p.L;
+}
+
+int tile_uniform_rows(const int* ni, const int* nj, int n, int L, int cus) {
+    static const int heights[] = {54, 42, 30, 18, 6};
+    const long need = static_cast<long>(3 * cus) * 6;
+    int RI = 6;
+    for (const int h : heights) {
+        long total = 0;
+        for (int k = 0; k < n; ++k) {
+            const int interior = ni[k] - 2, r = std::max(1, std::min(h, interior));
+            total += static_cast<long>(tile_nsg(nj[k], L)) * ((interior + r - 1) / r);
+        }
+        RI = h;
+        if (total * 10 >= need) break;
+    }
+    return RI;
+}
+
+TilePlan build_tile_plan(const int* ni, const int* nj, int n, const TilePlanParams& p) {
+    if (n < 1 || n > 8) throw PlanError(TM_E_ARG, "a fixed-wall launch takes 1 to 8 blocks");
+    if (p.L < 3 || p.L > 8 || p.cus < 1 || p.wg_per_cu < 1 || p.xcds != 8) throw PlanError(TM_E_ARG, "tile plan: depth, CU count or residency out of range");
+    for (int b = 0; b < n; ++b)
+        if (ni[b] < 2 * p.L + 1 || nj[b] < 2 * p.L + 1 || nj[b] > (1 << 20)) throw PlanError(TM_E_SIZE, "tile plan: block too small for the pass, or wider than 2^20 nodes");
+    TilePlan plan;
+    std::vector<int> rows(n);
+    plan.uniform_rows = p.forced_rows > 0 ? p.forced_rows : tile_uniform_rows(ni, nj, n, p.L, p.cus);
+    for (int b = 0; b < n; ++b) rows[b] = std::max(1, std::min(plan.uniform_rows, ni[b] - 2));
+    plan.tiles = uniform_tiles(ni, nj, n, p.L, rows.data(), plan.block_slots);
+    plan.uniform_makespan = plan.makespan = simulate_table(plan.tiles, p);
+    plan.mode = TILE_UNIFORM;
+    if (p.mode != TILE_BALANCED || p.forced_rows > 0 || (2 * (p.L - 1)) % 3 != 0) return plan;
+
+    std::vector<int> U(n), nsg(n);
+    std::vector<long> wbefore(n + 1, 0);
+    for (int b = 0; b < n; ++b) {
+        U[b] = (ni[b] - 2) / 3;
+        nsg[b] = tile_nsg(nj[b], p.L);
+        wbefore[b + 1] = wbefore[b] + static_cast<long>(U[b]) * nsg[b];
+    }
+    const long wtotal = wbefore[n];
+    struct Cut {
+        int block, u;
+    };
+    auto cut_at = [&](double target) {
+        int b = 0;
+        while (b + 1 < n && static_cast<double>(wbefore[b + 1]) <= target) ++b;
+        long u = std::lround((target - static_cast<double>(wbefore[b])) / nsg[b]);
+        u = std::max(0L, std::min<long>(u, U[b]));
+        return Cut{b, static_cast<int>(u)};
+    };
+    std::vector<Cut> cuts;
+    cuts.push_back(Cut{0, 0});
+    for (int x = 1; x < p.xcds; ++x) cuts.push_back(cut_at(static_cast<double>(wtotal) * x / p.xcds));
+    cuts.push_back(Cut{n - 1, U[n - 1]});
+    std::vector<std::vector<ColumnSeg>> band(p.xcds);
+    for (int x = 0; x < p.xcds; ++x) {
+        const Cut a = cuts[x], e = cuts[x + 1];
+        for (int b = a.block; b <= e.block; ++b) {
+            const int u0 = b == a.block ? a.u : 0, u1 = b == e.block ? e.u : U[b];
+            if (u1 <= u0) continue;
+            for (int sg = 0; sg < nsg[b]; ++sg) band[x].push_back(ColumnSeg{b, sg, u0, u1, u1 == U[b]});
+        }
+    }
+    const int slots_x = std::max(1, p.cus / p.xcds) * p.wg_per_cu;
+
+    struct Candidate {
+        std::vector<std::vector<TileRec>> list;
+        double makespan = 0.0;
+    };
+    std::vector<Candidate> cands;
+    const int ncu = std::max(1, p.cus / p.xcds);
+    auto add_candidate = [&](const std::function<bool(int x, const ColumnSeg&, std::vector<int>&)>& heights_of) {
+        Candidate c;
+        c.list.resize(p.xcds);
+        std::vector<int> q;
+        for (int x = 0; x < p.xcds; ++x) {
+            std::vector<TileRec>& tl = c.list[x];
+            for (const ColumnSeg& s : band[x]) {
+                if (!heights_of(x, s, q)) return;
+                int u = s.u0, total = 0;
+                for (int h : q) total += h;
+                if (total != s.u1 - s.u0) return;
+                for (size_t k = 0; k < q.size(); ++k) {
+                    if (q[k] < 1 || q[k] > TILE_QMAX) return;
+                    TileRec t;
+                    t.bsg = s.block | (s.sg << 4);
+                    t.i0 = 1 + 3 * u;
+                    u += q[k];
+                    t.i1 = 1 + 3 * u;
+                    if (s.takes_rest && u == s.u1) t.i1 = ni[s.block] - 1;
+                    t.slot = 0;
+                    tl.push_back(t);
+                }
+            }
+            std::stable_sort(tl.begin(), tl.end(), [](const TileRec& a, const TileRec& b) {
+                const int ha = a.i1 - a.i0, hb = b.i1 - b.i0;
+                if (ha != hb) return ha > hb;
+                if ((a.bsg & 15) != (b.bsg & 15)) return (a.bsg & 15) < (b.bsg & 15);
+                if (a.i0 != b.i0) return a.i0 < b.i0;
+                return a.bsg < b.bsg;
+            });
+            std::vector<double> cost;
+            for (const TileRec& t : tl) cost.push_back(tile_cost(t.i1 - t.i0, p));
+            c.makespan = std::max(c.makespan, simulate_xcd(cost, ncu, std::max(1, p.wg_per_cu), p.lone_rate));
+        }
+        cands.push_back(std::move(c));
+    };
+    auto count_candidate = [&](int T, bool same_per_column) {
+        add_candidate([&](int x, const ColumnSeg& s, std::vector<int>& q) {
+            long utotal = 0;
+            for (const ColumnSeg& o : band[x]) utotal += o.u1 - o.u0;
+            const int u = s.u1 - s.u0;
+            const double ideal = static_cast<double>(T) * u / static_cast<double>(utotal);
+            int nt = static_cast<int>(ideal);
+            if (!same_per_column) {
+                int given = 0, ahead = 0;
+                for (const ColumnSeg& o : band[x]) {
+                    const double io = static_cast<double>(T) * (o.u1 - o.u0) / static_cast<double>(utotal);
+                    given += static_cast<int>(io);
+                    const double fo = io - static_cast<int>(io), fs = ideal - nt;
+                    if (&o != &s && (fo > fs || (fo == fs && &o < &s))) ++ahead;
+                }
+                if (ahead < T - given) ++nt;
+            }
+            nt = std::max(1, std::min(nt, u));
+            equal_heights(u, nt, q);
+            return true;
+        });
+    };
+    for (int k = 1; k <= 8; ++k) {
+        count_candidate(k * slots_x, false);
+        count_candidate(k * slots_x, true);
+    }
+    for (int qbulk = 4; qbulk <= 34; qbulk += 2)
+        for (int qmin = 2; qmin <= 4; qmin += 2)
+            for (int f = 1; f <= 2; ++f)
+                add_candidate([&](int x, const ColumnSeg& s, std::vector<int>& q) {
+                    const double share = f * std::max(1.0, static_cast<double>(slots_x) / std::max<size_t>(1, band[x].size()));
+                    tapered_heights(s.u1 - s.u0, qbulk, qmin, share, q);
+                    return true;
+                });
+    if (cands.empty()) return plan;
+    std::vector<size_t> order(cands.size());
+    for (size_t k = 0; k < order.size(); ++k) order[k] = k;
+    std::stable_sort(order.begin(), order.end(), [&](size_t a, size_t b) { return cands[a].makespan < cands[b].makespan; });
+    const Candidate& best = cands[order[std::min<size_t>(std::max(0, p.pick), order.size() - 1)]];
+    if (p.pick == 0 && best.makespan > plan.uniform_makespan) return plan;
+    size_t longest = 0;
+    for (const auto& l : best.list) longest = std::max(longest, l.size());
+    std::vector<TileRec> table(longest * p.xcds, TileRec{0, 0, 0, -1});
+    for (int x = 0; x < p.xcds; ++x)
+        for (size_t k = 0; k < best.list[x].size(); ++k) table[k * p.xcds + x] = best.list[x][k];
+    while (!table.empty() && table.back().slot < 0 && table.back().i1 == table.back().i0) table.pop_back();
+    plan.block_slots.assign(n, 0);
+    for (TileRec& t : table)
+        if (t.i1 > t.i0) t.slot = plan.block_slots[t.bsg & 15]++;
+    plan.tiles.swap(table);
+    plan.makespan = best.makespan;
+    plan.mode = TILE_BALANCED;
+    return plan;
+}
+
+}
diff --git a/turbomesh_amd/csrc/tm_plan.hpp b/turbomesh_amd/csrc/tm_plan.hpp
--- a/turbomesh_amd/csrc/tm_plan.hpp
+++ b/turbomesh_amd/csrc/tm_plan.hpp
@@ -1,5 +1,6 @@
 #pragma once
 #include <cstdint>
+#include "tm_edge_types.h"
 #include <stdexcept>
 #include <string>
 #include <unordered_map>
@@ -90,4 +91,27 @@
 LocalPlan build_local_plan(const Topology& t, const std::vector<PlanRow>& all_rows, const std::vector<int32_t>& owner, int rank,
                            int nranks, bool allow_triples = true);
 
+enum TilePlanMode : int { TILE_UNIFORM = 0, TILE_BALANCED = 1 };
+struct TilePlanParams {
+    int L = 4;
+    int cus = 256;
+    int wg_per_cu = 3;
+    int xcds = 8;
+    int mode = TILE_UNIFORM;
+    int forced_rows = 0;
+    int pick = 0;
+    double c0 = 6.0;
+    double lone_rate = 0.8;
+};
+struct TilePlan {
+    std::vector<TileRec> tiles;
+    std::vector<int> block_slots;
+    int mode = TILE_UNIFORM;
+    int uniform_rows = 0;
+    double makespan = 0.0, uniform_makespan = 0.0;
+};
+int tile_uniform_rows(const int* ni, const int* nj, int n, int L, int cus);
+double tile_cost(int h, const TilePlanParams& p);
+TilePlan build_tile_plan(const int* ni, const int* nj, int n, const TilePlanParams& p);
+
 }
diff --git a/turbomesh_amd/csrc/tm_smoother.cpp b/turbomesh_amd/csrc/tm_smoother.cpp
--- a/turbomesh_amd/csrc/tm_smoother.cpp
+++ b/turbomesh_amd/csrc/tm_smoother.cpp
@@ -496,15 +496,37 @@
             if (!relax4_supported(bi.back(), bj.back())) fuse_quads = false;
         }
         poff4.clear();
-        rows4.assign(bi.size(), 1);
-        for (size_t first = 0; first < rows4.size(); first += APPLY_BATCH_MAX)
-            relax4_rows_for_launch(bi.data() + first, bj.data() + first, static_cast<int>(std::min<size_t>(APPLY_BATCH_MAX, rows4.size() - first)), rows4.data() + first);
+        launches4.clear();
         int off4 = 0;
-        for (size_t k = 0; k < rows4.size(); ++k) {
-            poff4.push_back(off4);
-            off4 += relax4_block_nwg(bi[k], bj[k], rows4[k]);
-        }
-        nwg_apply4 = fuse_quads ? off4 : 0;
+        if (fuse_quads) {
+            TilePlanParams tp;
+            tp.L = 4;
+            int dev = 0, cus = 0;
+            if (hipGetDevice(&dev) != hipSuccess || hipDeviceGetAttribute(&cus, hipDeviceAttributeMultiprocessorCount, dev) != hipSuccess || cus <= 0) cus = 256;
+            tp.cus = cus;
+            if (const char* e = std::getenv("TM_TILE_CUS")) tp.cus = std::max(8, std::atoi(e));
+            const int resident = relax4_wg_per_cu(opt.omega == 1.0, relax2_store_nt);
+            tp.wg_per_cu = resident > 0 ? resident : 3;
+            tp.mode = TILE_PLAN_DEFAULT;
+            if (const char* e = std::getenv("TM_TILE_PLAN")) tp.mode = std::atoi(e) != 0 ? TILE_BALANCED : TILE_UNIFORM;
+            if (const char* e = std::getenv("TM_FUSE4_ROWS")) tp.forced_rows = std::max(0, std::atoi(e));
+            if (const char* e = std::getenv("TM_TILE_PICK")) tp.pick = std::max(0, std::atoi(e));
+            for (size_t first = 0; first < bi.size(); first += APPLY_BATCH_MAX) {
+                const int nb = static_cast<int>(std::min<size_t>(APPLY_BATCH_MAX, bi.size() - first));
+                const TilePlan plan = build_tile_plan(bi.data() + first, bj.data() + first, nb, tp);
+                Quad4Launch q;
+                q.first = static_cast<int>(first);
+                q.n = nb;
+                q.ntiles = static_cast<int>(plan.tiles.size());
+                q.tiles = static_cast<const TileRec*>(upload_table(plan.tiles.data(), plan.tiles.size() * sizeof(TileRec)));
+                launches4.push_back(q);
+                for (int k = 0; k < nb; ++k) {
+                    poff4.push_back(off4);
+                    off4 += plan.block_slots[k];
+                }
+            }
+        }
+        nwg_apply4 = off4;
     }
     nwg_vec = vec_nwg(n_owned);
     const int nwg3_all = std::max(nwg_apply4, fuse_triples ? nwg_apply3 : (triples_coupled ? nwg_apply3 + std::max(edge_L[2].nwg, fused_levels.nstrips) : 0));
@@ -1568,7 +1590,10 @@
         a.nborder = 0;
         a.partials = partials + static_cast<size_t>(poffd[k]) * MAX_PARTIALS;
     }
-    if (depth == 4) profiled([&]() { HIPCHK(launch_relax4_blocks(blocks.data(), rows4.data(), static_cast<int>(blocks.size()), dot, stream)); }, true, stream);
+    if (depth == 4)
+        profiled([&]() {
+            for (const Quad4Launch& q : launches4) HIPCHK(launch_relax4_blocks(blocks.data() + q.first, q.n, q.tiles, q.ntiles, dot, stream));
+        }, true, stream);
     else profiled([&]() { HIPCHK(launch_relax3_blocks(blocks.data(), rows3.data(), static_cast<int>(blocks.size()), dot, stream)); }, true, stream);
     std::swap(X, U);
 }
diff --git a/turbomesh_amd/csrc/tm_smoother.hpp b/turbomesh_amd/csrc/tm_smoother.hpp
--- a/turbomesh_amd/csrc/tm_smoother.hpp
+++ b/turbomesh_amd/csrc/tm_smoother.hpp
@@ -117,8 +117,14 @@
     std::vector<int> poff3, rows3;
     int nwg_apply3 = 0;
     bool fuse_triples = false;
-    std::vector<int> poff4, rows4;
+    std::vector<int> poff4;
+    struct Quad4Launch {
+        int first = 0, n = 0, ntiles = 0;
+        const TileRec* tiles = nullptr;
+    };
+    std::vector<Quad4Launch> launches4;
     int nwg_apply4 = 0;
+    static constexpr int TILE_PLAN_DEFAULT = TILE_UNIFORM;
     bool fuse_quads = false;
     static constexpr int64_t QUAD_MIN_NODES = 8000000;
     bool triples_coupled = false;
diff --git a/turbomesh_amd/smoothing/smooth.py b/turbomesh_amd/smoothing/smooth.py
--- a/turbomesh_amd/smoothing/smooth.py
+++ b/turbomesh_amd/smoothing/smooth.py
@@ -252,3 +252,20 @@
     finally:
         _capi.lib().tm_plan_free(C.byref(rows))
     return out
+
+
+def tile_plan(shapes, mode=1, depth=4, cus=256, wg_per_cu=3, forced_rows=0, pick=0, c0=0.0, lone_rate=0.0):
+    ni = np.ascontiguousarray([s[0] for s in shapes], dtype=np.int32)
+    nj = np.ascontiguousarray([s[1] for s in shapes], dtype=np.int32)
+    opt = _capi.tm_tile_plan_opt(depth, cus, wg_per_cu, mode, forced_rows, pick, c0, lone_rate)
+    plan = _capi.tm_tile_plan()
+    i32p = C.POINTER(C.c_int32)
+    _capi.check(_capi.lib().tm_tile_plan_build(ni.ctypes.data_as(i32p), nj.ctypes.data_as(i32p), len(shapes), C.byref(opt), C.byref(plan)))
+    try:
+        n = int(plan.ntiles)
+        as_np = np.ctypeslib.as_array
+        out = {k: (as_np(getattr(plan, k), (n,)).copy() if n else np.zeros(0, np.int32)) for k in ("block", "sg", "i0", "i1", "slot")}
+        out.update(mode=int(plan.mode), uniform_rows=int(plan.uniform_rows), makespan=float(plan.makespan), uniform_makespan=float(plan.uniform_makespan))
+    finally:
+        _capi.lib().tm_tile_plan_free(C.byref(plan))
+    return out
```

After: 468.6 billion. -1.4%, worse.
